# blue-yonder/tsfresh

Measured on AMD Instinct MI355X. Metric: series/sec (ComprehensiveFCParameters, len=1024), higher is better.
Workload: dtype f64

## Files before the change

tsfresh_amd/csrc/fam_ar.h:

```cpp
#ifndef TSFA_FAM_AR_H
#define TSFA_FAM_AR_H

#include "tsfa_common.h"

TSFA_DEV int adf_maxlag_for(int n) {
    int maxlag = (int)ceil(12.0 * pow((double)n / 100.0, 0.25));
    const int cap = n / 2 - 1 - 1;
    if (cap < maxlag) maxlag = cap;
    return maxlag;
}

TSFA_DEV bool chol_factor(double *G, int p, int ld) {
    for (int j = 0; j < p; ++j) {
        double d = G[j + j * ld];
        for (int k = 0; k < j; ++k) d -= G[j + k * ld] * G[j + k * ld];
        if (!(d > 0.0)) return false;
        d = sqrt(d);
        G[j + j * ld] = d;
        for (int i = j + 1; i < p; ++i) {
            double s = G[i + j * ld];
            for (int k = 0; k < j; ++k) s -= G[i + k * ld] * G[j + k * ld];
            G[i + j * ld] = s / d;
        }
    }
    return true;
}
TSFA_DEV void chol_solve(const double *L, int p, int ld, const double *rhs, double *x) {
    for (int i = 0; i < p; ++i) {
        double s = rhs[i];
        for (int k = 0; k < i; ++k) s -= L[i + k * ld] * x[k];
        x[i] = s * (1.0 / L[i + i * ld]);
    }
    for (int i = p - 1; i >= 0; --i) {
        double s = x[i];
        for (int k = i + 1; k < p; ++k) s -= L[k + i * ld] * x[k];
        x[i] = s * (1.0 / L[i + i * ld]);
    }
}

TSFA_DEV void blk_chol_solve(const Blk &b, const double *L, int p, int ld, const double *rhs, double *x) {
#if TSFA_GPU
    const int lane = b.tid & 63;
    const bool live = lane < p;
    double s = live ? rhs[lane] : 0.0;
    const double dg = live ? 1.0 / L[lane + lane * ld] : 1.0;
    for (int k = 0; k < p; ++k) {
        const double wk = readlane_f64(s, k) * readlane_f64(dg, k);
        if (lane == k) s = wk;
        else if (live && lane > k) s -= L[lane + k * ld] * wk;
    }
    for (int k = p - 1; k >= 0; --k) {
        const double xk = readlane_f64(s, k) * readlane_f64(dg, k);
        if (lane == k) s = xk;
        else if (live && lane < k) s -= L[k + lane * ld] * xk;
    }
    if (b.tid < p) x[b.tid] = s;
#else
    if (b.tid == 0) chol_solve(L, p, ld, rhs, x);
#endif
}

#define TSFA_AR_PIVOT_TOL 1e-6
TSFA_DEV bool blk_chol_factor(const Blk &b, double *G, int p, int ld, double *diag0, double *dmin = nullptr) {
    for (int a = b.tid; a < p; a += b.nt) diag0[a] = G[a + a * ld];
    double dm = TSFA_INF;
    for (int j = 0; j < p; ++j) {
        blk_sync();
        const double d = G[j + j * ld];
        if (!(d > TSFA_AR_PIVOT_TOL * diag0[j])) return false;
        dm = fmin(dm, d);
        if (dmin) *dmin = dm;
        const double sd = sqrt(d);
        blk_sync();
        const double rsd = 1.0 / sd;
        for (int i = j + b.tid; i < p; i += b.nt) G[i + j * ld] = (i == j) ? sd : G[i + j * ld] * rsd;
        blk_sync();
        const int rsh = (b.nt >= 32) ? 5 : 0;
        for (int i = j + 1 + (b.tid & ((1 << rsh) - 1)); i < p; i += (1 << rsh)) {
            const double lij = G[i + j * ld];
            for (int k = j + 1 + (b.tid >> rsh); k <= i; k += (b.nt >> rsh))
                G[i + k * ld] = G[i + k * ld] - lij * G[k + j * ld];
        }
    }
    blk_sync();
    return true;
}
TSFA_DEV void blk_chol_forward(const Blk &b, const double *L, int p, int ld, double *w) {
#if TSFA_GPU
    if (p <= 64) {
        const int lane = b.tid & 63;
        const bool live = lane < p;
        double s = live ? w[lane] : 0.0;
        const double dg = live ? 1.0 / L[lane + lane * ld] : 1.0;
        for (int k = 0; k < p; ++k) {
            const double wk = readlane_f64(s, k) * readlane_f64(dg, k);
            if (lane == k) s = wk;
            else if (live && lane > k) s = s - L[lane + k * ld] * wk;
        }
        blk_sync();
        if (b.tid < p) w[b.tid] = s;
        blk_sync();
        return;
    }
#endif
    for (int i = 0; i < p; ++i) {
        blk_sync();
        const double wi = w[i] * (1.0 / L[i + i * ld]);
        blk_sync();
        if (b.tid == 0) w[i] = wi;
        for (int k = i + 1 + b.tid; k < p; k += b.nt) w[k] = w[k] - L[k + i * ld] * wi;
    }
    blk_sync();
}


#define TSFA_AR_PADL 64
#define TSFA_AR_PADR 16

template <class ST>
TSFA_DEV void ar_load8(const ST *p, double (&r)[8]) {
#if TSFA_GPU
    p = (const ST *)__builtin_assume_aligned(p, 16);
#endif
#pragma unroll
    for (int q = 0; q < 8; ++q) r[q] = (double)p[q];
}

template <class ST>
struct ArBlocks {
    const ST *xs;
    double mean;
    TSFA_MEM void y8(int i0, double (&r)[8]) const {
        ar_load8(xs + i0, r);
#pragma unroll
        for (int q = 0; q < 8; ++q) r[q] -= mean;
    }
    TSFA_MEM void d8(int i0, double (&r)[8]) const {
        double v[8];
        ar_load8(xs + i0, v);
        const double nx = (double)xs[i0 + 8];
#pragma unroll
        for (int q = 0; q < 7; ++q) r[q] = v[q + 1] - v[q];
        r[7] = nx - v[7];
    }
};

TSFA_DEV void tile_mask_rows(double (&A)[8], int tb, int r0, int r1) {
#pragma unroll
    for (int u = 0; u < 8; ++u) A[u] = (tb + u >= r0 && tb + u < r1) ? A[u] : 0.0;
}

TSFA_DEV void tile_dots8(const double (&A)[8], const double (&lo)[8], const double (&hi)[8], double (&s)[8]) {
#pragma unroll
    for (int j = 0; j < 8; ++j) {
#pragma unroll
        for (int u = 0; u < 8; ++u) s[j] = fma(A[u], (u >= j) ? hi[u - j] : lo[u - j + 8], s[j]);
    }
}
TSFA_DEV void tile_axpy8(const double (&cf)[8], const double (&lo)[8], const double (&hi)[8], double (&r)[8]) {
#pragma unroll
    for (int j = 0; j < 8; ++j) {
#pragma unroll
        for (int u = 0; u < 8; ++u) r[u] = fma(-cf[j], (u >= j) ? hi[u - j] : lo[u - j + 8], r[u]);
    }
}

#define TSFA_AR_PART_STRIDE 72
template <class LA, class LB, class SF>
TSFA_DEV void blk_tile_lagdots(const Blk &b, int nrows, int nlags, LA loadA, LB loadB, SF store, double *sums = nullptr,
                               double *part = nullptr, int part_doubles = 0) {
    const int ntiles = (nrows + 7) >> 3;
    const bool single = ntiles <= b.nt;
#if TSFA_GPU
    const int nwv = (b.nt + 63) >> 6, wv = b.tid >> 6, lane = b.tid & 63;
#else
    const int nwv = 1, wv = 0;
#endif
    const bool deferred = (part != nullptr) && (nwv * TSFA_AR_PART_STRIDE <= part_doubles) && (nlags <= 64);
    if (deferred) blk_sync();
    double A[8], lo[8], hi[8];
    for (int j0 = 0; j0 < nlags; j0 += 8) {
        double s[8], sa[2] = {0.0, 0.0};
#pragma unroll
        for (int j = 0; j < 8; ++j) s[j] = 0.0;
        for (int tile = b.tid; tile < ntiles; tile += b.nt) {
            const int tb = tile << 3;
            if (single && j0 > 0) {
#pragma unroll
                for (int q = 0; q < 8; ++q) hi[q] = lo[q];
            } else {
                loadA(tb, A);
                loadB(tb - j0, hi);
            }
            loadB(tb - j0 - 8, lo);
            tile_dots8(A, lo, hi, s);
            if (sums != nullptr && j0 == 0) {
#pragma unroll
                for (int u = 0; u < 8; ++u) { sa[0] += A[u]; sa[1] = fma(A[u], A[u], sa[1]); }
            }
        }
        if (deferred) {
            double *slot = part + wv * TSFA_AR_PART_STRIDE;
#if TSFA_GPU
            const double held = wave_reduce_scatter<8>(s);
            if (lane < 8) slot[j0 + wave_reduce_scatter_index<8>(lane)] = held;
            if (sums != nullptr && j0 == 0) {
                sa[0] = wave_sum(sa[0]);
                sa[1] = wave_sum(sa[1]);
                if (lane == 0) { slot[64] = sa[0]; slot[65] = sa[1]; }
            }
#else
#pragma unroll
            for (int j = 0; j < 8; ++j) slot[j0 + j] = s[j];
            if (sums != nullptr && j0 == 0) { slot[64] = sa[0]; slot[65] = sa[1]; }
#endif
            continue;
        }
        blk_sum_multi<8>(b, s);
        if (b.tid == 0) {
#pragma unroll
            for (int j = 0; j < 8; ++j)
                if (j0 + j < nlags) store(j0 + j, s[j]);
        }
        if (sums != nullptr && j0 == 0) {
            blk_sum_multi<2>(b, sa);
            sums[0] = sa[0];
            sums[1] = sa[1];
        }
    }
    if (deferred) {
        blk_sync();
        for (int j = b.tid; j < nlags; j += b.nt) {
            double v = part[j];
            for (int w = 1; w < nwv; ++w) v += part[w * TSFA_AR_PART_STRIDE + j];
            store(j, v);
        }
        if (sums != nullptr) {
            double v0 = part[64], v1 = part[65];
            for (int w = 1; w < nwv; ++w) { v0 += part[w * TSFA_AR_PART_STRIDE + 64]; v1 += part[w * TSFA_AR_PART_STRIDE + 65]; }
            sums[0] = v0;
            sums[1] = v1;
        }
    }
}

template <class S>
TSFA_DEV void blk_lag_products_rest(const Blk &b, S s, int Lg, int t0, int t1, double *T, int ld, double *C) {
    if (b.tid == 0) {
        for (int j = 0; j < Lg; ++j) C[j + 1] = C[j] + s(t0 - 1 - j) - s(t1 - 1 - j);
    }
    blk_sync();
    for (int dg = b.tid; dg <= Lg; dg += b.nt) {
        double v = T[dg];
        for (int j = 0; dg + j + 1 <= Lg; ++j) {
            const int i = dg + j;
            v = v + s(t0 - 1 - i) * s(t0 - 1 - j) - s(t1 - 1 - i) * s(t1 - 1 - j);
            T[(i + 1) + (j + 1) * ld] = v;
        }
    }
    blk_sync();
}

TSFA_DEV double mackinnon_p_c1(double t) {
    if (t > 2.74) return 1.0;
    if (t < -18.83) return 0.0;
    double z;
    if (t <= -1.61) z = 2.1659 + t * (1.4412 + t * (3.8269 * 1e-2));
    else z = 1.7339 + t * (9.3202 * 1e-1 + t * (-1.2745 * 1e-1 + t * (-1.0368 * 1e-2)));
    return tsfa_norm_cdf(z);
}

TSFA_DEV int ar_scratch_doubles(int P) { return 2 * P * P + 7 * P + 64 + 16 + 48 + 40 + 128; }

#define TSFA_AR_REFINE_TOL 1e-8
TSFA_DEV bool ar_refinement_suspect(const Blk &b, const double *beta, const double *corr, const double *diag0, int p) {
    double mb = 0.0, mc = 0.0;
#if TSFA_GPU
    for (int a = b.tid & 63; a < p; a += 64) {
        const double w = sqrt(diag0[a]);
        mb = fmax(mb, fabs(beta[a]) * w);
        mc = fmax(mc, fabs(corr[a]) * w);
    }
    mb = wave_max(mb);
    mc = wave_max(mc);
#else
    (void)b;
    for (int a = 0; a < p; ++a) {
        const double w = sqrt(diag0[a]);
        mb = fmax(mb, fabs(beta[a]) * w);
        mc = fmax(mc, fabs(corr[a]) * w);
    }
#endif
    return mc > TSFA_AR_REFINE_TOL * mb;
}

#define TSFA_AR_COND_CHECK_K 10
#define TSFA_AR_RAW_RATIO 1e-12
TSFA_DEV bool ar_raw_design_suspect(double dmin, double mu_norm, double trace_raw) {
    return sqrt(dmin) < TSFA_AR_RAW_RATIO * (1.0 + mu_norm) * sqrt(trace_raw);
}

template <class ST>
struct ArCentred {
    const ST *p;
    double mean;
    TSFA_MEM double operator[](int i) const { return (double)p[i] - mean; }
};
template <class ST, class X>
TSFA_DEV int fam_ar_series(const Blk &b, X xv, int n, const TsfaSpec *specs, int nspecs, double *out_row, void *xc_raw,
                            double *aw, int P, int hint_acf, int hint_pacf, int hint_adf, int n_loop = -1,
                            const double *stats = nullptr) {
    const int nloop = (n_loop >= 0) ? n_loop : nspecs;
    const double dn = (double)n;
    TSFA_TICKER(tk, 0);
    const double mean = stats ? stats[TSFA_STATS_MEAN] : np_sum(b, n, [=](int i) { return xv(i); }) / dn;
    blk_sync();
    ST *xs_lds = (ST *)xc_raw + TSFA_AR_PADL;
    for (int i = b.tid; i < n + TSFA_AR_PADL + TSFA_AR_PADR; i += b.nt) {
        const int j = i - TSFA_AR_PADL;
        ((ST *)xc_raw)[i] = (j >= 0 && j < n) ? (ST)xv(j) : (ST)0;
    }
    const ArCentred<ST> xc{xs_lds, mean};
    const ArBlocks<ST> blk{xs_lds, mean};
    blk_sync();
    double v0 = 0.0;
    for (int i = b.tid; i < n; i += b.nt) v0 += xc[i] * xc[i];
    const double var = blk_sum(b, v0) / dn;

    double *T = aw;
    double *G = T + P * P;
    double *g = G + P * P;
    double *beta = g + P;
    double *tmp1 = beta + P;
    double *tmp2 = tmp1 + P;
    double *C = tmp2 + P;
    double *V = C + P;
    double *diag0 = V + P;
    double *acv = diag0 + P;
    double *res = acv + 64;
    double *pac = res + 16;
    double *arres = pac + 48;
    double *pacw = arres + 40;
    const ArCentred<ST> xcc = xc;
    int degenerate = 0;

    TSFA_TICK(tk, b, 120);
    int max_acf_lag = hint_acf, max_pacf_lag = hint_pacf;
    const bool need_adf = (hint_adf != 0);
    const int adf_mode = (hint_adf >> 1) & 3;
    if (max_acf_lag > 60) max_acf_lag = 60;
    if (max_pacf_lag > 40) max_pacf_lag = 40;

    int pacf_maxlag = 0;
    if (max_pacf_lag >= 0 && n > 1) pacf_maxlag = (max_pacf_lag >= n / 2) ? (n / 2 - 1) : max_pacf_lag;
    int nacv = -1;
    if (max_acf_lag >= 0) nacv = (max_acf_lag < n - 1) ? max_acf_lag : (n - 1);
    if (pacf_maxlag > nacv) nacv = pacf_maxlag;
    if (nacv >= 0) {
        blk_tile_lagdots(b, n, nacv + 1,
                         [=](int tb, double (&A)[8]) { blk.y8(tb, A); tile_mask_rows(A, tb, 0, n); },
                         [=](int i0, double (&B)[8]) {
                             blk.y8(i0, B);
#pragma unroll
                             for (int q = 0; q < 8; ++q) B[q] = (i0 >= 0) ? B[q] : 0.0;
                         },
                         [=](int k, double v) { acv[k] = v / (double)(n - k); }, nullptr, G, P * P);
    }
    blk_sync();

    TSFA_TICK(tk, b, 121);
    if (max_pacf_lag >= 0) {
#if TSFA_GPU
        {
            const int lane = b.tid & 63;
            for (int k = b.tid; k <= max_pacf_lag; k += b.nt) pac[k] = TSFA_NAN;
            blk_sync();
            if (n > 1 && pacf_maxlag > 0) {
                const int ord = pacf_maxlag;
                const double a0 = acv[0], a1 = acv[1];
                const double p1v = a1 / a0;
                double phi = (lane == 1) ? p1v : 0.0;
                double sig = a0 - p1v * a1;
                if (b.tid == 0) pac[1] = p1v;
                for (int k = 2; k <= ord; ++k) {
                    const int back = k - lane;
                    const double ak = acv[(back >= 0 && back <= ord) ? back : 0];
                    const double prod = phi * ak;
                    double dot = 0.0;
                    for (int j = 1; j < k; ++j) dot += readlane_f64(prod, j);
                    const double pkk = (acv[k] - dot) / sig;
                    const double rev = __shfl(phi, (back >= 0 && back < 64) ? back : 0);
                    phi = (lane >= 1 && lane < k) ? phi - pkk * rev : ((lane == k) ? pkk : phi);
                    sig = sig * (1.0 - pkk * pkk);
                    if (b.tid == 0) pac[k] = pkk;
                }
                if (b.tid == 0) pac[0] = 1.0;
            }
        }
#else
        if (b.tid == 0) {
            for (int k = 0; k <= max_pacf_lag; ++k) pac[k] = TSFA_NAN;
            if (n > 1 && pacf_maxlag > 0) {
                const int ord = pacf_maxlag;
                double *prev = pacw, *cur = pacw + 42, *sig = pacw + 84;
                prev[1] = acv[1] / acv[0];
                pac[1] = prev[1];
                sig[1] = acv[0] - prev[1] * acv[1];
                for (int k = 2; k <= ord; ++k) {
                    double dot = 0.0;
                    for (int j = 1; j < k; ++j) dot += prev[j] * acv[k - j];
                    const double pkk = (acv[k] - dot) / sig[k - 1];
                    for (int j = 1; j < k; ++j) cur[j] = prev[j] - pkk * prev[k - j];
                    cur[k] = pkk;
                    sig[k] = sig[k - 1] * (1.0 - pkk * pkk);
                    pac[k] = pkk;
                    for (int j = 1; j <= k; ++j) prev[j] = cur[j];
                }
                pac[0] = 1.0;
            }
        }
#endif
        blk_sync();
    }

    TSFA_TICK(tk, b, 122);
    double adf_stat = TSFA_NAN, adf_p = TSFA_NAN, adf_lag = TSFA_NAN;
    if (need_adf) {
        const int maxlag = adf_maxlag_for(n);
        if (maxlag + 2 > 64) degenerate |= 2;
        else if (maxlag >= 0 && maxlag + 3 <= P) {
            auto dif = [=](int t) { return (double)xs_lds[t + 1] - (double)xs_lds[t]; };
            const int t0 = maxlag, t1 = n - 1;
            const double nobs = (double)(t1 - t0);
            auto d_blocks = [=](int i0, double (&B)[8]) { blk.d8(i0, B); };
            double sd[2], sl[2];
            blk_tile_lagdots(b, n, maxlag + 1,
                             [=](int tb, double (&A)[8]) { blk.d8(tb, A); tile_mask_rows(A, tb, t0, t1); }, d_blocks,
                             [=](int j, double v) { T[j] = v; }, sd, G, P * P);
            blk_tile_lagdots(b, n, maxlag + 1,
                             [=](int tb, double (&A)[8]) { blk.y8(tb, A); tile_mask_rows(A, tb, t0, t1); }, d_blocks,
                             [=](int j, double v) { V[j] = v; }, sl, G, P * P);
            if (b.tid == 0) C[0] = sd[0];
            blk_lag_products_rest(b, dif, maxlag, t0, t1, T, P, C);
            const double sx = sl[0], sxx = sl[1];
            const int p1 = maxlag + 2;
            for (int e = b.tid; e < 64 * p1; e += b.nt) {
                const int a = e & 63, c = e >> 6;
                if (a >= p1 || c > a) continue;
                double v;
                if (a == 0) v = nobs;
                else if (a == 1) v = (c == 0) ? sx : sxx;
                else {
                    const int la = a - 1;
                    if (c == 0) v = C[la];
                    else if (c == 1) v = V[la];
                    else v = T[la + (c - 1) * P];
                }
                G[a + c * P] = v;
            }
            for (int a = b.tid; a < p1; a += b.nt) g[a] = (a == 0) ? C[0] : (a == 1 ? V[0] : T[a - 1]);
            blk_sync();
            const double yy = T[0];
            TSFA_TICK(tk, b, 123);
            {
                double dmin1 = 0.0;
                const bool okf = blk_chol_factor(b, G, p1, P, diag0, &dmin1);
                if (!okf) degenerate |= 2;
                else {
                    const double mu = xcc.mean;
                    const double tr = nobs + (sxx + 2.0 * mu * sx + nobs * mu * mu) + (double)maxlag * yy;
                    if (ar_raw_design_suspect(dmin1, fabs(mu), tr)) degenerate |= 2;
                }
                if (okf) {
                    for (int a = b.tid; a < p1; a += b.nt) tmp1[a] = g[a];
                    blk_chol_forward(b, G, p1, P, tmp1);
                    if (b.tid == 0) {
                        double acc = 0.0;
                        for (int i = 0; i < p1; ++i) { acc += tmp1[i] * tmp1[i]; tmp2[i] = acc; }
                    }
                    blk_sync();
                    for (int i = b.tid; i < p1; i += b.nt) {
                        const int pcols = i + 1;
                        const double ssr = yy - tmp2[i];
                        const double llf = -0.5 * nobs * log(2.0 * M_PI) - 0.5 * nobs * log(ssr / nobs) - 0.5 * nobs;
                        const double wi = tmp1[i];
                        double ic = -2.0 * llf + ((adf_mode == TSFA_AUTOLAG_BIC) ? log(nobs) : 2.0) * (double)pcols;
                        if (adf_mode == TSFA_AUTOLAG_TSTAT) ic = fabs(wi / sqrt(ssr / (nobs - (double)pcols)));
                        tmp1[i] = ic;
                    }
                    blk_sync();
                }
                if (b.tid == 0) {
                    int best = -1;
                    double best_aic = 0.0;
                    if (okf && adf_mode == TSFA_AUTOLAG_TSTAT) {
                        for (int i = p1 - 1; i >= 1; --i) {
                            best = i + 1;
                            if (tmp1[i] >= TSFA_AUTOLAG_TSTAT_STOP) break;
                        }
                    } else if (okf && adf_mode == TSFA_AUTOLAG_NONE) {
                        best = p1;
                    } else if (okf)
                        for (int i = 1; i < p1; ++i) {
                            const double aic = tmp1[i];
                            if (best < 0 || aic < best_aic) { best = i + 1; best_aic = aic; }
                        }
                    res[0] = (double)best;
                }
            }
            blk_sync();
            const int bestcols = (int)res[0];
            blk_sync();
            TSFA_TICK(tk, b, 124);
            if (bestcols >= 2) {
                const int usedlag = bestcols - 2;
                const int p2 = usedlag + 2;
                const int u0 = usedlag;
                const double nobs2 = (double)(t1 - u0);
                auto reg2 = [=](int a, int t) { return a == 0 ? xcc[t] : (a == p2 - 1 ? 1.0 : dif(t - a)); };
                for (int e = b.tid; e < p2 * p2 + p2; e += b.nt) {
                    const bool is_rhs = e >= p2 * p2;
                    const int a = is_rhs ? e - p2 * p2 : e % p2;
                    const int c = is_rhs ? 0 : e / p2;
                    if (!is_rhs && c > a) continue;
                    double v;
                    auto lagidx = [=](int q) { return q == 0 ? -2 : (q == p2 - 1 ? -1 : q); };
                    const int A = lagidx(a), Cc = is_rhs ? 0 : lagidx(c);
                    if (is_rhs) {
                        v = (A == -2) ? V[0] : (A == -1 ? C[0] : T[A]);
                    } else {
                        const int hi = a, lo = c;
                        (void)hi; (void)lo;
                        if (A == -1 && Cc == -1) v = nobs;
                        else if ((A == -1 && Cc == -2) || (A == -2 && Cc == -1)) v = sx;
                        else if (A == -2 && Cc == -2) v = sxx;
                        else if (A == -1) v = C[Cc];
                        else if (Cc == -1) v = C[A];
                        else if (A == -2) v = V[Cc];
                        else if (Cc == -2) v = V[A];
                        else v = (A >= Cc) ? T[A + Cc * P] : T[Cc + A * P];
                    }
                    for (int t = u0; t < t0; ++t) v += reg2(a, t) * (is_rhs ? dif(t) : reg2(c, t));
                    if (is_rhs) g[a] = v; else G[a + c * P] = v;
                }
                blk_sync();
                const bool ok2 = blk_chol_factor(b, G, p2, P, diag0);
                if (!ok2) degenerate |= 2;
                if (ok2) blk_chol_solve(b, G, p2, P, g, beta);
                blk_sync();
                if (ok2) {
                    auto resid2 = [=](int t) {
                        double r = dif(t);
                        for (int c = 0; c < p2; ++c) r -= reg2(c, t) * beta[c];
                        return r;
                    };
                    for (int a0 = 0; a0 < p2; a0 += 8) {
                        double s8[8];
#pragma unroll
                        for (int j = 0; j < 8; ++j) s8[j] = 0.0;
                        for (int t = u0 + b.tid; t < t1; t += b.nt) {
                            const double rt = resid2(t);
#pragma unroll
                            for (int j = 0; j < 8; ++j)
                                if (a0 + j < p2) s8[j] += reg2(a0 + j, t) * rt;
                        }
                        blk_sum_multi<8>(b, s8);
                        if (b.tid == 0) {
#pragma unroll
                            for (int j = 0; j < 8; ++j)
                                if (a0 + j < p2) tmp1[a0 + j] = s8[j];
                        }
                    }
                    blk_sync();
                    blk_chol_solve(b, G, p2, P, tmp1, tmp2);
                    blk_sync();
                    if (ar_refinement_suspect(b, beta, tmp2, diag0, p2)) degenerate |= 2;
                    blk_sync();
                    for (int a = b.tid; a < p2; a += b.nt) beta[a] += tmp2[a];
                    blk_sync();
                    double ssr = 0.0;
                    for (int t = u0 + b.tid; t < t1; t += b.nt) {
                        double r = dif(t);
                        for (int c = 0; c < p2; ++c) r -= reg2(c, t) * beta[c];
                        ssr += r * r;
                    }
                    ssr = blk_sum(b, ssr);
                    for (int i = b.tid; i < p2; i += b.nt) tmp1[i] = (i == 0) ? 1.0 : 0.0;
                    blk_sync();
                    blk_chol_solve(b, G, p2, P, tmp1, tmp2);
                    blk_sync();
                    if (b.tid == 0) {
                        const double sigma2 = ssr / (nobs2 - (double)p2);
                        const double tstat = beta[0] / sqrt(sigma2 * tmp2[0]);
                        res[2] = tstat;
                        res[3] = mackinnon_p_c1(tstat);
                        res[4] = (double)usedlag;
                    }
                    blk_sync();
                    adf_stat = res[2];
                    adf_p = res[3];
                    adf_lag = res[4];
                    if (adf_stat != adf_stat) adf_p = TSFA_NAN;
                    blk_sync();
                }
            }
        }
    }

    int ar_cached_k = -1;
    bool ar_ok = false;
    TSFA_TICK(tk, b, 125);
    for (int s = 0; s < nloop; ++s) {
        const TsfaSpec sp = specs[s];
        double v = TSFA_NAN;
        switch (sp.calc) {
        case TSFA_C_AGG_AUTOCORRELATION: {
            const int agg = (int)sp.p[0];
            const int ml = (int)sp.p[1];
            double r = TSFA_NAN;
#if TSFA_GPU
            {
                int len = (ml < n - 1) ? ml : (n - 1);
                if (len > 60) len = 60;
                const int lane = b.tid & 63;
                const bool live = lane < len;
                if (fabs(var) < 1e-10 || n == 1) {
                    r = 0.0;
                } else if (len > 0) {
                    const double a0 = acv[0];
                    const double ak = live ? acv[lane + 1] / a0 : 0.0;
                    if (agg == TSFA_AGG_MEAN) {
                        r = wave_sum(ak) / (double)len;
                    } else if (agg == TSFA_AGG_VAR) {
                        const double m = wave_sum(ak) / (double)len;
                        const double d = live ? ak - m : 0.0;
                        r = wave_sum(d * d) / (double)len;
                    } else {
                        int rank = 0;
                        for (int j = 0; j < len; ++j) {
                            const double aj = readlane_f64(ak, j);
                            rank += (aj < ak || (aj == ak && j < lane)) ? 1 : 0;
                        }
                        const unsigned long long mlo = __ballot(live && rank == (len - 1) / 2);
                        const unsigned long long mhi = __ballot(live && rank == len / 2);
                        const double lo = readlane_f64(ak, __ffsll((long long)mlo) - 1);
                        const double hi = readlane_f64(ak, __ffsll((long long)mhi) - 1);
                        r = (len & 1) ? lo : (0.0 + lo + hi) / 2.0;
                    }
                }
            }
            v = r;
            break;
#endif
            if (b.tid == 0) {
                if (fabs(var) < 1e-10 || n == 1) {
                    r = 0.0;
                } else {
                    int len = (ml < n - 1) ? ml : (n - 1);
                    if (len > 60) len = 60;
                    double abuf[64];
                    double *a = abuf;
                    for (int k = 0; k < len; ++k) a[k] = acv[k + 1] / acv[0];
                    if (len <= 0) {
                        r = TSFA_NAN;
                    } else if (agg == TSFA_AGG_MEAN) {
                        r = np_leaf_sum(0, len, [=](int i) { return a[i]; }) / (double)len;
                    } else if (agg == TSFA_AGG_VAR) {
                        const double m = np_leaf_sum(0, len, [=](int i) { return a[i]; }) / (double)len;
                        r = np_leaf_sum(0, len, [=](int i) { const double d = a[i] - m; return d * d; }) / (double)len;
                    } else {
                        for (int i = 1; i < len; ++i) {
                            const double key = a[i];
                            int j = i - 1;
                            while (j >= 0 && a[j] > key) { a[j + 1] = a[j]; --j; }
                            a[j + 1] = key;
                        }
                        r = (len & 1) ? a[(len - 1) / 2] : (0.0 + a[len / 2 - 1] + a[len / 2]) / 2.0;
                    }
                }
            }
            v = blk_bcast0(b, r);
        } break;
        case TSFA_C_PARTIAL_AUTOCORRELATION: {
            const int l = (int)sp.p[0];
            v = (l >= 0 && l <= max_pacf_lag) ? pac[l] : TSFA_NAN;
        } break;
        case TSFA_C_AUGMENTED_DICKEY_FULLER: {
            const int attr = (int)sp.p[0];
            v = (attr == TSFA_ADF_TESTSTAT) ? adf_stat : (attr == TSFA_ADF_PVALUE ? adf_p : (attr == TSFA_ADF_USEDLAG ? adf_lag : TSFA_NAN));
        } break;
        case TSFA_C_AR_COEFFICIENT: {
            const int coeff = (int)sp.p[0], k = (int)sp.p[1];
            if (coeff > k) { v = TSFA_NAN; break; }
            if (n < 2 * k + 2 || k < 1) {
                v = (coeff < k) ? TSFA_NAN : 0.0;
                break;
            }
            if (k > TSFA_AR_TABLE_K || k + 2 > P) {
                degenerate |= 1;
                v = TSFA_NAN;
                break;
            }
            if (ar_cached_k != k) {
                auto sx = [=](int u) { return xcc[u]; };
                auto y_blocks = [=](int i0, double (&B)[8]) { blk.y8(i0, B); };
                double sy[2];
                blk_tile_lagdots(b, n, k + 1,
                                 [=](int tb, double (&A)[8]) { blk.y8(tb, A); tile_mask_rows(A, tb, k, n); }, y_blocks,
                                 [=](int j, double v) { T[j] = v; }, sy, G, P * P);
                if (b.tid == 0) C[0] = sy[0];
                blk_lag_products_rest(b, sx, k, k, n, T, P, C);
                const int p = k + 1;
                for (int e = b.tid; e < p * p; e += b.nt) {
                    const int a = e % p, c = e / p;
                    if (c > a) continue;
                    G[a + c * P] = (a == 0) ? (double)(n - k) : (c == 0 ? C[a] : T[a + c * P]);
                }
                for (int a = b.tid; a < p; a += b.nt) g[a] = (a == 0) ? C[0] : T[a];
                blk_sync();
                double dmin_ar = 0.0;
                ar_ok = blk_chol_factor(b, G, p, P, diag0, &dmin_ar);
                if (!ar_ok) degenerate |= 1;
                else {
                    const double mu = xcc.mean, rows = (double)(n - k);
                    double tr = rows;
                    for (int a = 1; a < p; ++a) tr += diag0[a] + 2.0 * mu * C[a] + rows * mu * mu;
                    if (ar_raw_design_suspect(dmin_ar, sqrt((double)k) * fabs(mu), tr)) degenerate |= 1;
                }
                if (ar_ok && k > TSFA_AR_COND_CHECK_K) {
                    double tr0 = 0.0, s0 = 0.0;
                    for (int a = 0; a < p; ++a) { tr0 += diag0[a]; s0 += 1.0 / diag0[a]; }
                    for (int a = b.tid; a < p; a += b.nt) tmp1[a] = 1.0 / sqrt(diag0[a] * s0);
                    blk_sync();
                    double lmin = tr0;
                    for (int it = 0; it < 2; ++it) {
                        blk_chol_solve(b, G, p, P, tmp1, tmp2);
                        blk_sync();
                        double nrm2 = 0.0;
                        for (int a = 0; a < p; ++a) nrm2 += tmp2[a] * tmp2[a];
                        const double nrm = sqrt(nrm2);
                        if (!(nrm > 0.0) || isinf(nrm) || nrm != nrm) { lmin = 0.0; break; }
                        lmin = 1.0 / nrm;
                        blk_sync();
                        for (int a = b.tid; a < p; a += b.nt) tmp1[a] = tmp2[a] / nrm;
                        blk_sync();
                    }
                    if (!(lmin >= 1e-12 * tr0)) degenerate |= 1;
                }
                if (ar_ok) blk_chol_solve(b, G, p, P, g, beta);
                blk_sync();
                if (ar_ok) {
                    double sr[2];
                    blk_tile_lagdots(b, n, k + 1,
                                     [=](int tb, double (&A)[8]) {
                                         blk.y8(tb, A);
                                         const double b0 = beta[0];
#pragma unroll
                                         for (int u = 0; u < 8; ++u) A[u] -= b0;
                                         double lo[8], hi[8], cf[8];
                                         blk.y8(tb, hi);
                                         for (int c0 = 0; c0 <= k; c0 += 8) {
                                             blk.y8(tb - c0 - 8, lo);
#pragma unroll
                                             for (int j = 0; j < 8; ++j) {
                                                 const int c = c0 + j;
                                                 cf[j] = (c >= 1 && c <= k) ? beta[(c <= k) ? c : 0] : 0.0;
                                             }
                                             tile_axpy8(cf, lo, hi, A);
#pragma unroll
                                             for (int q = 0; q < 8; ++q) hi[q] = lo[q];
                                         }
                                         tile_mask_rows(A, tb, k, n);
                                     },
                                     y_blocks, [=](int a, double v) { if (a > 0) tmp1[a] = v; }, sr, T, P * P);
                    if (b.tid == 0) tmp1[0] = sr[0];
                    blk_sync();
                    blk_chol_solve(b, G, p, P, tmp1, tmp2);
                    blk_sync();
                    if (ar_refinement_suspect(b, beta, tmp2, diag0, p)) degenerate |= 1;
                    blk_sync();
                    if (b.tid == 0) {
                        double sphi = 0.0;
                        for (int a = 0; a < p; ++a) {
                            beta[a] += tmp2[a];
                            if (a > 0) sphi += beta[a];
                        }
                        arres[0] = beta[0] + mean * (1.0 - sphi);
                        for (int a = 1; a < p; ++a) arres[a] = beta[a];
                    }
                    blk_sync();
                }
                ar_cached_k = k;
            }
            v = ar_ok ? arres[coeff] : TSFA_NAN;
        } break;
        default: break;
        }
        if (b.tid == 0) out_row[sp.col] = v;
        TSFA_TICK(tk, b, sp.calc);
    }
    if (nloop < nspecs) {
        blk_sync();
        for (int s = nloop + b.tid; s < nspecs; s += b.nt) {
            const TsfaSpec sp = specs[s];
            double v = TSFA_NAN;
            if (sp.calc == TSFA_C_PARTIAL_AUTOCORRELATION) {
                const int l = (int)sp.p[0];
                v = (l >= 0 && l <= max_pacf_lag) ? pac[l] : TSFA_NAN;
            } else if (sp.calc == TSFA_C_AUGMENTED_DICKEY_FULLER) {
                const int attr = (int)sp.p[0];
                v = (attr == TSFA_ADF_TESTSTAT) ? adf_stat : (attr == TSFA_ADF_PVALUE ? adf_p : (attr == TSFA_ADF_USEDLAG ? adf_lag : TSFA_NAN));
            } else if (sp.calc == TSFA_C_AR_COEFFICIENT) {
                const int coeff = (int)sp.p[0], k = (int)sp.p[1];
                if (coeff > k) v = TSFA_NAN;
                else if (n < 2 * k + 2 || k < 1) v = (coeff < k) ? TSFA_NAN : 0.0;
                else v = (ar_cached_k == k && ar_ok && k <= TSFA_AR_TABLE_K) ? arres[coeff] : TSFA_NAN;
            }
            out_row[sp.col] = v;
        }
    }
    return degenerate;
}

#endif
```

tsfresh_amd/csrc/tsfa_api.cpp:

```cpp
#include <hip/hip_runtime.h>

#include <stdio.h>
#include <stdlib.h>

#include <algorithm>
#include <string>
#include <vector>

#include "../../include/tsfresh_amd.h"
#include "tsfa_host_tables.h"
#include "tsfa_launch.h"
#include "fam_seq.h"
#include "tsfa_layout.h"

static thread_local std::string g_last_error;

static int fail(int code, const std::string &msg) {
    g_last_error = msg;
    return code;
}

int tsfa_fail(int code, const char *msg) { return fail(code, std::string(msg ? msg : "")); }
#define HIP_TRY(expr)                                                                                    \
    do {                                                                                                 \
        hipError_t e_ = (expr);                                                                          \
        if (e_ != hipSuccess) return fail(TSFA_ERR_HIP, std::string(#expr) + ": " + hipGetErrorString(e_)); \
    } while (0)

struct DevBuf {
    void *p = nullptr;
    size_t cap = 0;
    int ensure(size_t bytes) {
        if (bytes <= cap) return 0;
        size_t want = bytes + bytes / 8 + 4096;
        void *q = nullptr;
        if (hipMalloc(&q, want) != hipSuccess) {
            (void)hipGetLastError();
            if (p) { (void)hipFree(p); p = nullptr; cap = 0; }
            if (hipMalloc(&q, want) != hipSuccess) {
                (void)hipGetLastError();
                return -1;
            }
        }
        if (p) (void)hipFree(p);
        p = q;
        cap = want;
        return 0;
    }
    void release() {
        if (p) (void)hipFree(p);
        p = nullptr;
        cap = 0;
    }
};

#define TSFA_MAX_AUX 3
#define TSFA_MAX_CHUNKS 16
#define TSFA_DEFAULT_STREAMS 1

struct Timing {
    std::string name;
    hipEvent_t e0 = nullptr, e1 = nullptr;
    float ms = 0.f;
};

struct PlanOptions {
    bool length_classes = true;
    bool stats_share = true;
    bool perm_share = true;
    bool select = true;
    bool bluestein = true;
    bool cwt_mfma = false;
    bool force_long = false;
    int entropy_route = 0;
    int bluestein_min = 0;
    int gscratch_slots = 0;
    int host_chunks = 0;
    int nt[TSFA_N_FAMILIES] = {0};
    bool trace = false;
    bool row_form = true;
    int seq_rows = -1;
};

#if defined(TSFA_LAB)
#define TSFA_LAB_ONLY(x) (x)
#else
#define TSFA_LAB_ONLY(x) (0)
#endif

static int64_t g_relevance_batch = 0;
int64_t tsfa_relevance_batch_override() { return g_relevance_batch; }

struct tsfa_plan {
    int device = 0;
    PlanOptions opt;
    hipStream_t stream = nullptr;
    int n_cols = 0;
    std::vector<TsfaSpec> fam_specs[TSFA_N_FAMILIES];
    TsfaSpec *d_specs[TSFA_N_FAMILIES] = {nullptr};
    TsfaFamHints hints[TSFA_N_FAMILIES];
    TsfaCwtBank bank;
    double *d_W = nullptr;
    int *d_cols = nullptr, *d_coeff = nullptr;
    double *d_dectab = nullptr, *d_twc = nullptr, *d_tws = nullptr, *d_consts = nullptr;
    long long *d_stats = nullptr;
    DevBuf values, offsets, out, gscratch, times, deg_list, sel, long_scratch, pf_buf, perm_buf, stats_buf, dd_scratch, gen_scratch, seq_rows;
    std::vector<TsfaSpec> gen_specs;
    TsfaSpec *d_gen_specs = nullptr;
    TsfaGenPlan gen_plan;
    double *d_pool = nullptr;
    int *d_deg_count = nullptr;
    int *d_cursor = nullptr;
    hipStream_t s_in = nullptr, s_out = nullptr;
    hipEvent_t ev_in[TSFA_MAX_CHUNKS] = {nullptr}, ev_k[TSFA_MAX_CHUNKS] = {nullptr};
    std::vector<int64_t> h_rel;
    bool needs_times = false;
    bool sort_only_order_stats = false;
    bool stream_ok = false;
    int n_streams = 1;
    hipStream_t aux[TSFA_MAX_AUX] = {nullptr};
    hipEvent_t ev_fork = nullptr, ev_join[TSFA_MAX_AUX] = {nullptr};
    bool profiling = false;
    std::vector<Timing> timings;
    long long hint_min_len = 0, hint_max_len = 0;
    bool fill_all = false;
    int *d_fill_cols = nullptr;
    int n_fill_cols = 0;
    int debug_skip_fam = -1;
    hipStream_t side = nullptr;
    hipEvent_t ev_side_fork = nullptr, ev_side_join = nullptr;
    unsigned side_mask = 0;
    double fill_value = __builtin_nan("");
};

static const char *fam_names[TSFA_N_FAMILIES] = {"k_basic", "k_sort", "k_spectral", "k_ar", "k_entropy", "k_cwtpeaks", "k_seq", "k_trend"};

template <class T>
static int upload(const std::vector<T> &h, T **d) {
    *d = nullptr;
    if (h.empty()) return 0;
    if (hipMalloc((void **)d, h.size() * sizeof(T)) != hipSuccess) return -1;
    if (hipMemcpy(*d, h.data(), h.size() * sizeof(T), hipMemcpyHostToDevice) != hipSuccess) return -1;
    return 0;
}

static int record(tsfa_plan *plan, hipStream_t st, size_t slot, const char *name, bool begin) {
    if (!plan->profiling) return 0;
    if (plan->timings.size() <= slot) plan->timings.resize(slot + 1);
    Timing &t = plan->timings[slot];
    if (!t.e0) {
        if (hipEventCreate(&t.e0) != hipSuccess || hipEventCreate(&t.e1) != hipSuccess) return -1;
    }
    t.name = name;
    return hipEventRecord(begin ? t.e0 : t.e1, st) == hipSuccess ? 0 : -1;
}

extern "C" {

int tsfa_version(void) { return TSFA_VERSION; }

int tsfa_device_count(void) {
    int n = 0;
    if (hipGetDeviceCount(&n) != hipSuccess) return 0;
    return n;
}

const char *tsfa_last_error(void) { return g_last_error.c_str(); }

int tsfa_calc_id(const char *name) {
    if (!name) return -1;
    for (int i = 0; i < TSFA_N_CALCS; ++i)
        if (strcmp(tsfa_calc_table[i].name, name) == 0) return i;
    return -1;
}
const char *tsfa_calc_name(int calc) { return (calc >= 0 && calc < TSFA_N_CALCS) ? tsfa_calc_table[calc].name : nullptr; }
int tsfa_calc_count(void) { return TSFA_N_CALCS; }

void tsfa_plan_destroy(tsfa_plan *plan) {
    if (!plan) return;
    (void)hipSetDevice(plan->device);
    for (int f = 0; f < TSFA_N_FAMILIES; ++f)
        if (plan->d_specs[f]) (void)hipFree(plan->d_specs[f]);
    if (plan->d_W) (void)hipFree(plan->d_W);
    if (plan->d_cols) (void)hipFree(plan->d_cols);
    if (plan->d_coeff) (void)hipFree(plan->d_coeff);
    if (plan->d_dectab) (void)hipFree(plan->d_dectab);
    if (plan->d_twc) (void)hipFree(plan->d_twc);
    if (plan->d_tws) (void)hipFree(plan->d_tws);
    if (plan->d_consts) (void)hipFree(plan->d_consts);
    if (plan->d_stats) (void)hipFree(plan->d_stats);
    if (plan->d_deg_count) (void)hipFree(plan->d_deg_count);
    if (plan->d_cursor) (void)hipFree(plan->d_cursor);
    plan->deg_list.release();
    plan->pf_buf.release();
    plan->stats_buf.release();
    plan->perm_buf.release();
    plan->sel.release();
    plan->long_scratch.release();
    for (int i = 0; i < TSFA_MAX_CHUNKS; ++i) {
        if (plan->ev_in[i]) (void)hipEventDestroy(plan->ev_in[i]);
        if (plan->ev_k[i]) (void)hipEventDestroy(plan->ev_k[i]);
    }
    if (plan->s_in) (void)hipStreamDestroy(plan->s_in);
    if (plan->s_out) (void)hipStreamDestroy(plan->s_out);
    plan->times.release();
    plan->values.release();
    plan->offsets.release();
    plan->out.release();
    plan->gscratch.release();
    plan->dd_scratch.release();
    plan->gen_scratch.release();
    if (plan->d_gen_specs) (void)hipFree(plan->d_gen_specs);
    if (plan->d_pool) (void)hipFree(plan->d_pool);
    for (auto &t : plan->timings) {
        if (t.e0) (void)hipEventDestroy(t.e0);
        if (t.e1) (void)hipEventDestroy(t.e1);
    }
    for (int i = 0; i < TSFA_MAX_AUX; ++i) {
        if (plan->aux[i]) (void)hipStreamDestroy(plan->aux[i]);
        if (plan->ev_join[i]) (void)hipEventDestroy(plan->ev_join[i]);
    }
    if (plan->ev_fork) (void)hipEventDestroy(plan->ev_fork);
    if (plan->side) (void)hipStreamDestroy(plan->side);
    if (plan->ev_side_fork) (void)hipEventDestroy(plan->ev_side_fork);
    if (plan->ev_side_join) (void)hipEventDestroy(plan->ev_side_join);
    if (plan->stream) (void)hipStreamDestroy(plan->stream);
    delete plan;
}

int tsfa_plan_create(const tsfa_feature_spec *specs, int32_t n_specs, int32_t device, tsfa_plan **out_plan) {
    return tsfa_plan_create_with_data(specs, n_specs, nullptr, 0, device, out_plan);
}

int tsfa_plan_create_with_data(const tsfa_feature_spec *specs, int32_t n_specs, const double *data, int64_t n_data, int32_t device,
                               tsfa_plan **out_plan) {
    if (!out_plan) return fail(TSFA_ERR_INVALID, "out_plan is NULL");
    *out_plan = nullptr;
    if (n_specs < 0 || (n_specs > 0 && !specs)) return fail(TSFA_ERR_INVALID, "bad specs");
    if (n_data < 0 || (n_data > 0 && !data)) return fail(TSFA_ERR_INVALID, "bad data pool");
    const int ndev = tsfa_device_count();
    if (ndev <= 0) return fail(TSFA_ERR_NO_DEVICE, "no HIP device visible: tsfresh_amd has no CPU fallback");
    if (device < 0 || device >= ndev) return fail(TSFA_ERR_INVALID, "device ordinal out of range");

    tsfa_plan *plan = new tsfa_plan();
    plan->device = device;
    plan->n_cols = n_specs;
    std::vector<TsfaSpec> cwt_coef;
    bool general[TSFA_N_CALCS];
    tsfa_general_calcs(specs, n_specs, general);
    for (int i = 0; i < n_specs; ++i) {
        TsfaSpec s;
        s.calc = specs[i].calc;
        s.col = i;
        for (int k = 0; k < 4; ++k) s.p[k] = specs[i].p[k];
        if (s.calc < 0 || s.calc >= TSFA_N_CALCS) {
            delete plan;
            return fail(TSFA_ERR_UNSUPPORTED, "spec " + std::to_string(i) + ": unknown calculator id " + std::to_string(s.calc));
        }
        const std::string why = tsfa_validate_spec(s);
        if (!why.empty()) {
            delete plan;
            return fail(TSFA_ERR_UNSUPPORTED, std::string("spec ") + std::to_string(i) + " (" + tsfa_calc_table[s.calc].name + "): " + why);
        }
        if (s.calc == TSFA_C_QUERY_SIMILARITY_COUNT && s.p[3] > 0 && !(s.p[2] + s.p[3] <= (double)n_data)) {
            delete plan;
            return fail(TSFA_ERR_INVALID, "spec " + std::to_string(i) + " (query_similarity_count): the query lies outside the data pool");
        }
        if (s.calc == TSFA_C_LINEAR_TREND_TIMEWISE) plan->needs_times = true;
        if (s.calc == TSFA_C_CWT_COEFFICIENTS) cwt_coef.push_back(s);
        else if (general[s.calc]) plan->gen_specs.push_back(s);
        else plan->fam_specs[tsfa_calc_table[s.calc].family].push_back(s);
    }
    plan->gen_plan = tsfa_prepare_general(plan->gen_specs);
    if (cwt_coef.size() > 128) {
        delete plan;
        return fail(TSFA_ERR_UNSUPPORTED, "more than 128 cwt_coefficients columns in one plan");
    }
    {
        std::vector<TsfaSpec> all;
        for (int f = 0; f < TSFA_N_FAMILIES; ++f) all.insert(all.end(), plan->fam_specs[f].begin(), plan->fam_specs[f].end());
        const std::string why = tsfa_validate_plan(all.data(), (int)all.size());
        if (!why.empty()) {
            delete plan;
            return fail(TSFA_ERR_UNSUPPORTED, why);
        }
    }
    if (!cwt_coef.empty()) {
        const std::string why = plan->bank.build(cwt_coef);
        if (!why.empty()) {
            delete plan;
            return fail(TSFA_ERR_UNSUPPORTED, why);
        }
    }
    if (hipSetDevice(device) != hipSuccess) {
        delete plan;
        return fail(TSFA_ERR_HIP, "hipSetDevice failed");
    }
    for (int f = 0; f < TSFA_N_FAMILIES; ++f) tsfa_prepare_family(f, plan->fam_specs[f], plan->hints[f]);
    plan->sort_only_order_stats = !plan->fam_specs[TSFA_FAM_SORT].empty();
    for (const auto &sp : plan->fam_specs[TSFA_FAM_SORT])
        if (sp.calc != TSFA_C_MEDIAN && sp.calc != TSFA_C_QUANTILE) plan->sort_only_order_stats = false;
    plan->stream_ok = !plan->fam_specs[TSFA_FAM_BASIC].empty() && plan->hints[TSFA_FAM_BASIC].c == 0;
    for (const auto &sp : plan->fam_specs[TSFA_FAM_BASIC])
        if (!tsfa_stream_calc_ok(sp.calc) || sp.calc == TSFA_C_MEDIAN) plan->stream_ok = false;
    for (const auto &sp : plan->fam_specs[TSFA_FAM_SORT])
        if (sp.calc != TSFA_C_MEDIAN) plan->stream_ok = false;
    bool ok = hipStreamCreateWithFlags(&plan->stream, hipStreamNonBlocking) == hipSuccess;
    for (int f = 0; ok && f < TSFA_N_FAMILIES; ++f) ok = upload(plan->fam_specs[f], &plan->d_specs[f]) == 0;
    if (ok) ok = upload(plan->gen_specs, &plan->d_gen_specs) == 0;
    if (ok && n_data > 0) ok = upload(std::vector<double>(data, data + n_data), &plan->d_pool) == 0;
    if (ok && !cwt_coef.empty()) {
        ok = upload(plan->bank.W, &plan->d_W) == 0 && upload(plan->bank.cols, &plan->d_cols) == 0 &&
             upload(plan->bank.coeff_idx, &plan->d_coeff) == 0;
    }
    if (ok) {
        std::vector<double> dt, twc, tws;
        tsfa_build_dectab(dt);
        tsfa_build_twiddles(twc, tws);
        ok = upload(dt, &plan->d_dectab) == 0 && upload(twc, &plan->d_twc) == 0 && upload(tws, &plan->d_tws) == 0;
        std::vector<double> consts;
        tsfa_build_consts(consts);
        ok = ok && upload(consts, &plan->d_consts) == 0;
    }
    if (ok) ok = hipMalloc((void **)&plan->d_stats, TSFA_LEN_STATS * sizeof(long long)) == hipSuccess;
    if (ok) ok = hipMalloc((void **)&plan->d_deg_count, 2 * sizeof(int)) == hipSuccess;
    if (ok) ok = hipMalloc((void **)&plan->d_cursor, TSFA_N_LEN_CLASSES * sizeof(int)) == hipSuccess;
    if (ok) ok = hipStreamCreateWithFlags(&plan->s_in, hipStreamNonBlocking) == hipSuccess &&
                 hipStreamCreateWithFlags(&plan->s_out, hipStreamNonBlocking) == hipSuccess;
    for (int i = 0; ok && i < TSFA_MAX_CHUNKS; ++i)
        ok = hipEventCreateWithFlags(&plan->ev_in[i], hipEventDisableTiming) == hipSuccess &&
             hipEventCreateWithFlags(&plan->ev_k[i], hipEventDisableTiming) == hipSuccess;
    {
        const char *e = getenv("TSFA_STREAMS");
        plan->n_streams = e ? std::min(std::max(atoi(e), 1), TSFA_MAX_AUX + 1) : TSFA_DEFAULT_STREAMS;
        for (int i = 0; ok && i + 1 < plan->n_streams; ++i)
            ok = hipStreamCreateWithFlags(&plan->aux[i], hipStreamNonBlocking) == hipSuccess &&
                 hipEventCreateWithFlags(&plan->ev_join[i], hipEventDisableTiming) == hipSuccess;
        if (ok && plan->n_streams > 1) ok = hipEventCreateWithFlags(&plan->ev_fork, hipEventDisableTiming) == hipSuccess;
    }
    if (const char *e = getenv("TSFA_PAIR")) {
        static const char *nm[TSFA_N_FAMILIES] = {"basic", "sort", "spectral", "ar", "entropy", "cwt", "seq", "trend"};
        for (int f = 0; f < TSFA_N_FAMILIES; ++f)
            if (f != TSFA_FAM_BASIC && f != TSFA_FAM_SORT && f != TSFA_FAM_ENTROPY && strstr(e, nm[f])) plan->side_mask |= 1u << f;
        if (plan->side_mask) {
            int least = 0, greatest = 0;
            (void)hipDeviceGetStreamPriorityRange(&least, &greatest);
            ok = ok && hipStreamCreateWithPriority(&plan->side, hipStreamNonBlocking, least) == hipSuccess &&
                 hipEventCreateWithFlags(&plan->ev_side_fork, hipEventDisableTiming) == hipSuccess &&
                 hipEventCreateWithFlags(&plan->ev_side_join, hipEventDisableTiming) == hipSuccess;
        }
    }
    if (const char *e = getenv("TSFA_HOST_CHUNKS")) plan->opt.host_chunks = std::max(atoi(e), 0);
    if (!ok) {
        tsfa_plan_destroy(plan);
        return fail(TSFA_ERR_HIP, "device allocation/upload failed while creating the plan");
    }
    *out_plan = plan;
    return TSFA_OK;
}

int32_t tsfa_plan_n_cols(const tsfa_plan *plan) { return plan ? plan->n_cols : -1; }

int tsfa_plan_set_length_hint(tsfa_plan *plan, int64_t min_len, int64_t max_len) {
    if (!plan) return fail(TSFA_ERR_INVALID, "null plan");
    if (max_len == 0 && min_len == 0) { plan->hint_min_len = plan->hint_max_len = 0; return TSFA_OK; }
    if (min_len < 1 || max_len < min_len || max_len > 2147483647LL / 64) return fail(TSFA_ERR_INVALID, "length hint must satisfy 1 <= min <= max <= 33554431");
    plan->hint_min_len = min_len;
    plan->hint_max_len = max_len;
    return TSFA_OK;
}

int tsfa_plan_set_option(tsfa_plan *plan, const char *name, double value) {
    if (!name) return fail(TSFA_ERR_INVALID, "option name is NULL");
    const std::string n(name);
    const bool on = value != 0.0;
    if (!plan) {
        if (n == "relevance_batch") { g_relevance_batch = value > 0.0 ? (int64_t)value : 0; return TSFA_OK; }
        return fail(TSFA_ERR_INVALID, "unknown library option '" + n + "'");
    }
    PlanOptions &o = plan->opt;
    if (n == "length_classes") o.length_classes = on;
    else if (n == "stats_share") o.stats_share = on;
    else if (n == "perm_share") o.perm_share = on;
    else if (n == "select") o.select = on;
    else if (n == "bluestein") o.bluestein = on;
    else if (n == "cwt_mfma") o.cwt_mfma = on;
    else if (n == "force_long") o.force_long = on;
    else if (n == "row_form") o.row_form = on;
    else if (n == "seq_rows") o.seq_rows = (value < 0.0) ? -1 : (on ? 1 : 0);
    else if (n == "entropy_route") { if (value != 0.0 && value != 1.0 && value != 2.0) return fail(TSFA_ERR_INVALID, "entropy_route: 0, 1 or 2"); o.entropy_route = (int)value; }
    else if (n == "bluestein_min") o.bluestein_min = value > 0.0 ? (int)std::min(value, 32767.0) : 0;
    else if (n == "gscratch_slots") o.gscratch_slots = value > 0.0 ? (int)std::min(value, 2147483647.0) : 0;
    else if (n == "host_chunks") o.host_chunks = value > 0.0 ? (int)std::min(value, (double)TSFA_MAX_CHUNKS) : 0;
    else if (n == "fused_minimal") { if (!on) plan->stream_ok = false; }
    else if (n == "perm_fused") { if (!on) plan->hints[TSFA_FAM_SORT].d = 0; }
    else if (n == "fill") { plan->fill_value = value; plan->fill_all = true; }
    else if (n == "fill_off") { plan->fill_all = false; }
#if defined(TSFA_LAB)
    else if (n == "skip_family") plan->debug_skip_fam = (int)value;
    else if (n == "trace") o.trace = on;
    else if (n.rfind("nt_", 0) == 0 && n.size() == 4 && n[3] >= '0' && n[3] < '0' + TSFA_N_FAMILIES) o.nt[n[3] - '0'] = (int)value;
#endif
    else return fail(TSFA_ERR_INVALID, "unknown plan option '" + n + "'");
    return TSFA_OK;
}

int tsfa_plan_set_profiling(tsfa_plan *plan, int32_t enable) {
    if (!plan) return fail(TSFA_ERR_INVALID, "plan is NULL");
    plan->profiling = enable != 0;
    return TSFA_OK;
}

int32_t tsfa_plan_last_timings(const tsfa_plan *plan, const char **names, float *ms, int32_t cap) {
    if (!plan) return 0;
    int32_t n = 0;
    for (const auto &t : plan->timings) {
        if (n >= cap) break;
        if (names) names[n] = t.name.c_str();
        if (ms) ms[n] = t.ms;
        ++n;
    }
    return n;
}

int tsfa_extract(tsfa_plan *plan, const void *values, int32_t dtype, const int64_t *offsets, int64_t n_series,
                 double *out, int64_t ld_out, int32_t space, void *stream) {
    return tsfa_extract_timed(plan, values, dtype, nullptr, offsets, n_series, out, ld_out, space, stream);
}

int tsfa_extract_timed(tsfa_plan *plan, const void *values, int32_t dtype, const double *times, const int64_t *offsets,
                       int64_t n_series, double *out, int64_t ld_out, int32_t space, void *stream) {
    return tsfa_extract_windows(plan, values, dtype, times, offsets, offsets ? offsets + 1 : nullptr, n_series, out,
                                ld_out, space, stream);
}

struct BatchShape {
    long long max_len = 0, min_len = 0, max_np2 = 0;
    int n_groups = 1;
    int g_maxn[TSFA_N_LEN_CLASSES] = {0};
    long long g_np2[TSFA_N_LEN_CLASSES] = {0};
    int64_t g_count[TSFA_N_LEN_CLASSES] = {0};
    bool g_has_short[TSFA_N_LEN_CLASSES] = {false};
    TsfaClassMap map;
};

static void shape_from_stats(const long long *st, int64_t n_series, BatchShape &sh, bool length_classes) {
    sh.max_len = st[0];
    sh.min_len = st[1];
    sh.max_np2 = st[2];
    memset(&sh.map, 0, sizeof sh.map);
    sh.n_groups = 1;
    sh.g_maxn[0] = (int)st[0];
    sh.g_np2[0] = st[2];
    sh.g_count[0] = n_series;
    sh.g_has_short[0] = st[1] <= TSFA_ROW_MAXN;
    if (!length_classes || n_series < 2048 || st[0] <= 2 * st[1] || st[0] <= 128) return;
    const int64_t min_group = 512;
    int ng = 0;
    int64_t pend_count = 0;
    long long pend_np2 = 0;
    int first_of_group = 0;
    for (int c = 0; c < TSFA_N_LEN_CLASSES; ++c) {
        const int64_t cnt = st[3 + c];
        pend_count += cnt;
        pend_np2 = std::max(pend_np2, st[3 + 2 * TSFA_N_LEN_CLASSES + c]);
        bool last = true;
        for (int d = c + 1; d < TSFA_N_LEN_CLASSES; ++d)
            if (st[3 + d] > 0) last = false;
        if (cnt > 0 && (pend_count >= min_group || last)) {
            sh.g_maxn[ng] = (int)st[3 + TSFA_N_LEN_CLASSES + c];
            sh.g_np2[ng] = pend_np2;
            sh.g_count[ng] = pend_count;
            sh.g_has_short[ng] = false;
            for (int d = first_of_group; d <= c; ++d) {
                sh.map.group_of[d] = ng;
                if ((64LL << d) <= TSFA_ROW_MAXN && st[3 + d] > 0) sh.g_has_short[ng] = true;
            }
            first_of_group = c + 1;
            pend_count = 0;
            pend_np2 = 0;
            ++ng;
        }
        if (last) {
            for (int d = first_of_group; d < TSFA_N_LEN_CLASSES; ++d) sh.map.group_of[d] = ng > 0 ? ng - 1 : 0;
            break;
        }
    }
    sh.n_groups = std::max(ng, 1);
    int b = 0;
    for (int g = 0; g < sh.n_groups; ++g) {
        sh.map.base[g] = b;
        b += (int)sh.g_count[g];
    }
}

static int host_len_stats(const int64_t *starts, const int64_t *ends, int64_t n, long long *st) {
    for (int i = 0; i < TSFA_LEN_STATS; ++i) st[i] = 0;
    st[1] = (1LL << 62);
    for (int64_t s = 0; s < n; ++s) {
        const long long l = ends[s] - starts[s];
        if (l < 0) return -1;
        const bool np2 = l > 0 && (l & (l - 1)) != 0;
        const int c = tsfa_len_class(l);
        st[0] = std::max(st[0], l);
        st[1] = std::min(st[1], l);
        if (np2) st[2] = std::max(st[2], l);
        st[3 + c] += 1;
        st[3 + TSFA_N_LEN_CLASSES + c] = std::max(st[3 + TSFA_N_LEN_CLASSES + c], l);
        if (np2) st[3 + 2 * TSFA_N_LEN_CLASSES + c] = std::max(st[3 + 2 * TSFA_N_LEN_CLASSES + c], l);
    }
    return 0;
}

static int run_batch(tsfa_plan *plan, const void *d_values, int dtype, const double *d_times, const int64_t *d_starts,
                     const int64_t *d_ends, int64_t n_series, double *d_out, int64_t ld, const BatchShape &sh,
                     const int *d_sel, hipStream_t st, bool with_overlap) {
    if ((plan->fill_all || plan->n_fill_cols > 0) &&
        tsfa_launch_fill_nan(d_out, n_series, plan->n_cols, ld, st, plan->fill_value, plan->fill_all ? nullptr : plan->d_fill_cols,
                             plan->n_fill_cols))
        return fail(TSFA_ERR_HIP, "fill launch failed");

    static const int order_long_first[TSFA_N_FAMILIES] = {TSFA_FAM_ENTROPY, TSFA_FAM_AR, TSFA_FAM_SORT, TSFA_FAM_CWT, TSFA_FAM_BASIC,
                                                          TSFA_FAM_SEQ, TSFA_FAM_SPECTRAL, TSFA_FAM_TREND};
    static const int order_basic_first[TSFA_N_FAMILIES] = {TSFA_FAM_BASIC, TSFA_FAM_ENTROPY, TSFA_FAM_AR, TSFA_FAM_SORT, TSFA_FAM_CWT,
                                                           TSFA_FAM_SEQ, TSFA_FAM_SPECTRAL, TSFA_FAM_TREND};
    const bool overlap = with_overlap && plan->n_streams > 1 && !plan->profiling;
    const bool share_stats = plan->stats_buf.p != nullptr && !overlap && !plan->stream_ok && plan->opt.stats_share;
    const int *order = share_stats ? order_basic_first : order_long_first;
    bool stats_valid[TSFA_N_LEN_CLASSES + 1];
    for (int g = 0; g <= TSFA_N_LEN_CLASSES; ++g) stats_valid[g] = false;
    if (overlap) {
        HIP_TRY(hipEventRecord(plan->ev_fork, st));
        for (int i = 0; i + 1 < plan->n_streams; ++i) HIP_TRY(hipStreamWaitEvent(plan->aux[i], plan->ev_fork, 0));
    }
    bool pair = plan->side != nullptr && plan->side_mask != 0 && !overlap && !plan->profiling && with_overlap;
    for (int g = 0; g < sh.n_groups; ++g) pair = pair && sh.g_maxn[g] <= 4096;
    bool side_forked = false, side_used = false;
    size_t slot = 0;
    int dealt = 0;
    bool perm_valid[TSFA_N_LEN_CLASSES + 1];
    for (int g = 0; g <= TSFA_N_LEN_CLASSES; ++g) perm_valid[g] = false;
    const bool perm_share = plan->perm_buf.p != nullptr && !overlap && plan->opt.perm_share;
    bool stream_done[TSFA_N_LEN_CLASSES + 1];
    for (int g = 0; g <= TSFA_N_LEN_CLASSES; ++g) stream_done[g] = false;
    for (int fi = 0; fi < TSFA_N_FAMILIES; ++fi) {
        const int f = order[fi];
        if (plan->fam_specs[f].empty()) continue;
        if (TSFA_LAB_ONLY(plan->debug_skip_fam == f)) continue;
        if (f == TSFA_FAM_BASIC && plan->stream_ok) {
            bool all = true;
            for (int g = 0; g < sh.n_groups; ++g) all = all && stream_done[g];
            if (all) continue;
        }
        hipStream_t fst = st;
        if (overlap) {
            const int k = dealt++ % plan->n_streams;
            if (k > 0) fst = plan->aux[k - 1];
        }
        if (pair && fi > 0 && ((plan->side_mask >> f) & 1u)) {
            if (!side_forked) {
                HIP_TRY(hipEventRecord(plan->ev_side_fork, st));
                HIP_TRY(hipStreamWaitEvent(plan->side, plan->ev_side_fork, 0));
                side_forked = true;
            }
            fst = plan->side;
            side_used = true;
        }
        const char *slot_name = (plan->stream_ok && (f == TSFA_FAM_SORT || (f == TSFA_FAM_BASIC && plan->fam_specs[TSFA_FAM_SORT].empty())))
                                    ? "k_stream" : fam_names[f];
        if (record(plan, fst, slot, slot_name, true)) return fail(TSFA_ERR_HIP, "event record failed");
        std::vector<TsfaLaunch> perm_launches;
        for (int g = sh.n_groups - 1; g >= 0; --g) {
            const int maxn = sh.g_maxn[g];
            const long long max_np2 = sh.g_np2[g];
            TsfaLaunch a;
            memset(&a, 0, sizeof a);
            a.fam = f;
            a.dtype = dtype;
            a.values = d_values;
            a.starts = d_starts;
            a.ends = d_ends;
            a.n_series = sh.g_count[g];
            a.sel = (sh.n_groups > 1) ? d_sel + sh.map.base[g] : nullptr;
            a.specs = plan->d_specs[f];
            a.nspecs = (int)plan->fam_specs[f].size();
            a.out = d_out;
            a.ld = ld;
            a.maxn = maxn;
            a.nt = (maxn <= 2048) ? 64 : 256;
            if (maxn > 2048) {
                static const int nt_8k[TSFA_N_FAMILIES] = {512, 512, 512, 512, 256, 1024, 256, 256};
                static const int nt_4k[TSFA_N_FAMILIES] = {256, 256, 256, 256, 256, 512, 256, 256};
                a.nt = (maxn > 4096) ? nt_8k[f] : nt_4k[f];
            }
            if (maxn <= 2048) {
                static const int pref[TSFA_N_FAMILIES] = {64, 128, 128, 128, 256, 256, 128, 64};
                const int cap = std::max(64, ((maxn / 4 + 63) / 64) * 64);
                a.nt = std::min(pref[f], cap);
            }
            if (TSFA_LAB_ONLY(plan->opt.nt[f] >= 64)) a.nt = plan->opt.nt[f];
            a.stream = fst;
            a.dectab = plan->d_dectab;
            a.times = d_times;
            a.twc = plan->d_twc;
            a.consts = plan->d_consts;
            a.tws = plan->d_tws;
            a.hint_a = plan->hints[f].a;
            a.hint_b = plan->hints[f].b;
            a.hint_c = plan->hints[f].c;
            a.hint_d = plan->hints[f].d;
            a.hint_e = plan->hints[f].e;
            a.alt = plan->hints[f].alt;
            a.cq = plan->hints[f].cq;
            if (f == TSFA_FAM_SPECTRAL && maxn > 2048 && !TSFA_LAB_ONLY(plan->opt.nt[f] >= 64)) a.nt = 512;
            int aux = 0;
            if (f == TSFA_FAM_TREND) aux = a.alt.small_w;
            if (f == TSFA_FAM_SPECTRAL) {
                a.dft_n = (int)std::min<long long>(max_np2, 256);
                aux = a.dft_n;
                int bl_odd = TSFA_BLUESTEIN_MIN, bl_even = TSFA_BLUESTEIN_MIN_EVEN;
                if (plan->opt.bluestein_min > 0) bl_odd = bl_even = std::min(std::max(plan->opt.bluestein_min, 17), 32767);
                a.bluestein_min = TSFA_BLUESTEIN_PACK(bl_odd, bl_even);
                if (max_np2 >= std::min(bl_odd, bl_even) && max_np2 <= 32768 && plan->opt.bluestein) {
                    long long M = 1;
                    while (M < 2 * max_np2 - 1) M <<= 1;
                    const size_t slot_bytes = (size_t)(4 * M) * sizeof(double);
                    int64_t slots = std::min<int64_t>(a.n_series, std::max<int64_t>((int64_t)((1ull << 30) / slot_bytes), 2048));
                    if (plan->opt.gscratch_slots > 0) slots = std::min<int64_t>(slots, plan->opt.gscratch_slots);
                    const size_t bytes = (size_t)slots * slot_bytes;
                    if (plan->gscratch.ensure(bytes) == 0) {
                        a.gscratch = (double *)plan->gscratch.p;
                        a.gscratch_n = (int)(4 * M);
                        a.gscratch_slots = slots;
                    }
                }
            } else if (f == TSFA_FAM_CWT) {
                a.cwt_rowv = tsfa_family_lds_bytes(f, maxn, a.nt, 1) <= 96 * 1024 ? 1 : 0;
                aux = a.cwt_rowv;
                if (plan->opt.cwt_mfma) a.cwt_rowv |= 2;
            } else if (f == TSFA_FAM_AR) {
                int P = 8, Pdd = 8;
                for (const auto &s : plan->fam_specs[f]) {
                    if (s.calc == TSFA_C_AUGMENTED_DICKEY_FULLER) {
                        int ml = (int)ceil(12.0 * pow((double)maxn / 100.0, 0.25));
                        if (maxn / 2 - 2 < ml) ml = maxn / 2 - 2;
                        P = std::max(P, ml + 3);
                    } else if (s.calc == TSFA_C_AR_COEFFICIENT) {
                        const int k = std::min((int)s.p[1], std::max(1, (maxn - 2) / 2));
                        if ((int)s.p[1] <= TSFA_AR_TABLE_K) P = std::max(P, (int)s.p[1] + 2);
                        Pdd = std::max(Pdd, k + 2);
                        a.ar_has_coef = 1;
                    }
                }
                Pdd = std::max(Pdd, P);
                a.ar_P = P;
                a.ar_P_dd = Pdd;
                aux = P;
                {
                    ArDdLds D;
                    if (D.carve(nullptr, Pdd) > TSFA_LDS_LIMIT - 2048) {
                        const size_t slot_bytes = (size_t)ArDdLds::scratch_doubles(Pdd) * sizeof(double);
                        const int slots = (int)std::min<int64_t>(a.n_series, std::min<int64_t>(256, std::max<int64_t>(8, (int64_t)(((size_t)2 << 30) / slot_bytes))));
                        if (plan->dd_scratch.ensure((size_t)slots * slot_bytes))
                            return fail(TSFA_ERR_HIP, "hipMalloc failed for the second AR pass");
                        a.dd_scratch = (double *)plan->dd_scratch.p;
                        a.dd_slots = slots;
                    }
                }
                a.deg_list = (long long *)plan->deg_list.p;
                a.deg_count = plan->d_deg_count;
                HIP_TRY(hipMemsetAsync(plan->d_deg_count, 0, sizeof(int), fst));
            } else if (f == TSFA_FAM_SORT && plan->hints[f].b > 0) {
                a.pf_slot = tsfa_pf_slot_doubles(plan->hints[f].b);
                a.pf_buf = (double *)plan->pf_buf.p;
                a.pf_count = plan->d_deg_count + 1;
                a.pf_cap = (int)std::min<long long>((long long)n_series * std::max(1, plan->hints[f].e), 2147483647LL);
                HIP_TRY(hipMemsetAsync(a.pf_count, 0, sizeof(int), fst));
            } else if (f == TSFA_FAM_ENTROPY) {
                const int waves = std::min(4, std::max(1, (maxn - 1 + 63) / 64));
                a.nt = std::max(a.nt, 64 * waves);
                a.ent_cnt = tsfa_entropy_lds_bytes(maxn, 1) <= TSFA_LDS_LIMIT ? 1 : 0;
                a.ent_fast = a.ent_cnt;
                for (const auto &s : plan->fam_specs[f])
                    if (s.calc == TSFA_C_APPROXIMATE_ENTROPY && (int)s.p[0] != 2) a.ent_fast = 0;
                if (plan->opt.entropy_route == 2) a.ent_fast = 0;
                const bool entb_wide = maxn > TSFA_ENTB_MAXN && maxn <= TSFA_ENTB_MAXN_WIDE &&
                                       tsfa_entropy_lds_bytes(maxn, 2) <= TSFA_LDS_LIMIT &&
                                       entb_kround(maxn, std::min(a.nspecs, TSFA_ENTB_MAXK), TSFA_ENTB_MAXWAVES) >= std::min(a.nspecs, TSFA_ENTB_MAXK);
                if (a.ent_fast && a.nspecs >= 2 && maxn >= 3 && plan->opt.entropy_route == 0 &&
                    ((maxn <= TSFA_ENTB_MAXN && tsfa_entropy_lds_bytes(maxn, 2) <= TSFA_LDS_LIMIT / 2) || entb_wide)) {
                    a.ent_cnt = 2;
                    a.nt = 64 * std::min(TSFA_ENTB_MAXWAVES, entb_waves_for(maxn, a.nspecs));
                    if (TSFA_LAB_ONLY(plan->opt.nt[f] >= 64)) a.nt = plan->opt.nt[f];
                } else if (a.ent_fast && a.nspecs >= 2 && maxn > TSFA_ENTB_MAXN && maxn <= TSFA_ENTB_MAXN_LONG &&
                           plan->opt.entropy_route == 0 &&
                           tsfa_entropy_lds_bytes(maxn, 3) <= TSFA_LDS_LIMIT) {
                    a.ent_cnt = 3;
                    a.nt = 64 * TSFA_ENTB_MAXWAVES;
                } else if (a.nspecs >= 2 && maxn > TSFA_ENTB_MAXN_LONG && maxn <= TSFA_ENTH_MAXN && plan->opt.entropy_route == 0) {
                    bool all_m2 = true;
                    for (const auto &s : plan->fam_specs[f])
                        if (s.calc == TSFA_C_APPROXIMATE_ENTROPY && (int)s.p[0] != 2) all_m2 = false;
                    if (all_m2) {
                        a.ent_cnt = 4;
                        a.ent_fast = 0;
                        a.nt = 64 * TSFA_ENTB_MAXWAVES;
                    }
                }
            }
            int seq_group = 0;
            if (f == TSFA_FAM_SEQ) {
                for (seq_group = std::min(a.nspecs, TSFA_LZ_MAX_GROUP); seq_group > 1; --seq_group) {
                    bool fits = true;
                    for (int s0 = 0; fits && s0 < a.nspecs; s0 += seq_group) {
                        lz_build_group(plan->fam_specs[f].data() + s0, std::min(seq_group, a.nspecs - s0), maxn, &a.seq);
                        fits = tsfa_seq_lds_bytes(a.seq) <= TSFA_LDS_LIMIT;
                    }
                    if (fits) break;
                }
                lz_build_group(plan->fam_specs[f].data(), std::min(seq_group, a.nspecs), maxn, &a.seq);
            }
            size_t seq_lds = 0;
            int seq_grows = 0;
            if (f == TSFA_FAM_SEQ) {
                TsfaSeqGroup g;
                for (int s0 = 0; s0 < a.nspecs; s0 += seq_group) {
                    lz_build_group(plan->fam_specs[f].data() + s0, std::min(seq_group, a.nspecs - s0), maxn, &g);
                    seq_lds = std::max(seq_lds, tsfa_seq_lds_bytes(g));
                }
                if (plan->opt.seq_rows != 0 && !plan->opt.force_long) {
                    const int group_g = std::min(a.nspecs, TSFA_LZ_MAX_GROUP);
                    size_t lds_g = 0, stride_g = 0;
                    for (int s0 = 0; s0 < a.nspecs; s0 += group_g) {
                        lz_build_group(plan->fam_specs[f].data() + s0, std::min(group_g, a.nspecs - s0), maxn, &g, 1);
                        lds_g = std::max(lds_g, tsfa_seq_lds_bytes(g));
                        stride_g = std::max(stride_g, (size_t)g.stride);
                    }
                    auto resident = [&](size_t lds) {
                        if (lds > TSFA_LDS_LIMIT) return (size_t)0;
                        return std::min<size_t>((size_t)(163840 / std::max<size_t>(lds, 1)), (size_t)(32 * 64 / a.nt));
                    };
                    const bool more = resident(lds_g) > resident(seq_lds);
                    if (lds_g <= TSFA_LDS_LIMIT && (plan->opt.seq_rows == 1 || more) &&
                        (size_t)a.n_series * stride_g <= ((size_t)2 << 30) &&
                        plan->seq_rows.ensure((size_t)a.n_series * stride_g) == 0) {
                        seq_grows = 1;
                        seq_group = group_g;
                        seq_lds = lds_g;
                        a.seq_rows = (unsigned char *)plan->seq_rows.p;
                    }
                }
            }
            size_t lds = (f == TSFA_FAM_SEQ) ? seq_lds
                         : (f == TSFA_FAM_ENTROPY) ? tsfa_entropy_lds_bytes(maxn, a.ent_cnt)
                                                   : tsfa_family_lds_bytes(f, maxn, a.nt, aux);
            const bool use_long = lds > TSFA_LDS_LIMIT || plan->opt.force_long || (f == TSFA_FAM_ENTROPY && a.ent_cnt == 4);
            if (TSFA_LAB_ONLY(f == TSFA_FAM_SPECTRAL && plan->opt.trace))
                fprintf(stderr, "[tsfa] spectral group %d: n_series %lld maxn %d max_np2 %lld lds %zu long %d chirp-z %d slots %lld nt %d\n", g,
                        (long long)a.n_series, maxn, max_np2, lds, (int)use_long, (int)(a.gscratch != nullptr), (long long)a.gscratch_slots, a.nt);
            if (use_long) {
                if (!(f == TSFA_FAM_ENTROPY && a.ent_cnt == 4)) a.nt = 256;
                if (a.gscratch != nullptr && a.gscratch_slots < std::min<int64_t>(a.n_series, 2048)) a.gscratch = nullptr;
                if (f == TSFA_FAM_ENTROPY && a.ent_cnt != 4) { a.ent_cnt = 0; a.ent_fast = 0; lds = tsfa_entropy_lds_bytes(maxn, 5); }
                if (f == TSFA_FAM_CWT) { a.cwt_rowv &= 2; lds = tsfa_family_lds_bytes(f, maxn, a.nt, 0); }
                if (f == TSFA_FAM_SEQ) {
                    seq_group = std::min(a.nspecs, TSFA_LZ_MAX_GROUP);
                    seq_grows = 0;
                    lds = 0;
                    for (int s0 = 0; s0 < a.nspecs; s0 += seq_group) {
                        lz_build_group(plan->fam_specs[f].data() + s0, std::min(seq_group, a.nspecs - s0), maxn, &a.seq);
                        lds = std::max(lds, tsfa_seq_lds_bytes(a.seq));
                    }
                } else if (f != TSFA_FAM_ENTROPY && f != TSFA_FAM_CWT) {
                    lds = tsfa_family_lds_bytes(f, maxn, a.nt, aux);
                }
                const size_t slot_bytes = (lds + 255) & ~(size_t)255;
                const int64_t n_slots = std::max<int64_t>(1, std::min<int64_t>(std::min<int64_t>(a.n_series, 512),
                                                                               (int64_t)((4ull << 30) / slot_bytes)));
                if (plan->long_scratch.ensure((size_t)n_slots * slot_bytes))
                    return fail(TSFA_ERR_HIP, "hipMalloc failed for the long-series scratch");
                a.long_scratch = (unsigned char *)plan->long_scratch.p;
                a.long_bytes = (size_t)n_slots * slot_bytes;
            }
            if (share_stats && g <= TSFA_N_LEN_CLASSES) {
                if (f == TSFA_FAM_BASIC && !(plan->hints[f].c == 0 && a.nt <= 256)) {
                    a.stats_out = (double *)plan->stats_buf.p;
                    stats_valid[g] = true;
                } else if ((f == TSFA_FAM_ENTROPY || f == TSFA_FAM_AR || f == TSFA_FAM_SEQ || f == TSFA_FAM_SORT) && stats_valid[g]) {
                    a.stats_in = (const double *)plan->stats_buf.p;
                }
            }
            if (perm_share && !use_long && g <= TSFA_N_LEN_CLASSES) {
                if (f == TSFA_FAM_ENTROPY && a.ent_cnt == 2 && maxn <= TSFA_ENTB_MAXN) {
                    a.perm_buf = (unsigned short *)plan->perm_buf.p;
                    a.perm_stride = TSFA_ENTB_MAXN;
                    perm_valid[g] = true;
                } else if (f == TSFA_FAM_SORT && perm_valid[g]) {
                    a.perm_buf = (unsigned short *)plan->perm_buf.p;
                    a.perm_stride = TSFA_ENTB_MAXN;
                }
            }
            if (f == TSFA_FAM_SORT) {
                a.hint_d = 0;
                if (plan->hints[f].d != 0) {
                    const int pnt = (maxn <= 2048) ? std::min(256, std::max(64, ((maxn / 4 + 63) / 64) * 64))
                                                   : std::min(1024, ((maxn / 8 + 63) / 64) * 64);
                    if (maxn <= 65535 && tsfa_perm_lds_bytes(maxn, pnt, dtype == TSFA_F32 ? 4 : 8) <= TSFA_LDS_LIMIT) {
                        a.hint_d = plan->hints[f].d;
                        TsfaLaunch pa = a;
                        pa.nt = pnt;
                        pa.long_scratch = nullptr;
                        perm_launches.push_back(pa);
                    }
                }
            }
            int rc = 0;
            if (plan->stream_ok && (f == TSFA_FAM_SORT || f == TSFA_FAM_BASIC) && maxn <= 2048 && g <= TSFA_N_LEN_CLASSES) {
                if (stream_done[g]) continue;
                TsfaLaunch sa = a;
                sa.specs = plan->d_specs[TSFA_FAM_SORT];
                sa.nspecs = (int)plan->fam_specs[TSFA_FAM_SORT].size();
                sa.bspecs = plan->d_specs[TSFA_FAM_BASIC];
                sa.nbspecs = (int)plan->fam_specs[TSFA_FAM_BASIC].size();
                rc = tsfa_launch_stream(sa);
                stream_done[g] = true;
            } else
            if (f == TSFA_FAM_SORT && plan->sort_only_order_stats && maxn <= 2048 && !use_long &&
                plan->opt.select) {
                rc = tsfa_launch_order_stats(a);
            } else if (f == TSFA_FAM_SEQ) {
                for (int s0 = 0; rc == 0 && s0 < a.nspecs; s0 += seq_group) {
                    lz_build_group(plan->fam_specs[f].data() + s0, std::min(seq_group, a.nspecs - s0), maxn, &a.seq, seq_grows);
                    if (!use_long && tsfa_seq_lds_bytes(a.seq) > TSFA_LDS_LIMIT)
                        return fail(TSFA_ERR_TOO_LONG, "k_seq: a series of " + std::to_string(maxn) + " samples does not fit LDS");
                    rc = use_long ? tsfa_launch_family_long(a) : tsfa_launch_family(a);
                }
            } else {
                bool rows_any = false, rows_all = false;
                const bool lite = (f == TSFA_FAM_BASIC && plan->hints[f].c == 0 && a.nt <= 256);
                if ((f == TSFA_FAM_BASIC || f == TSFA_FAM_TREND) && plan->opt.row_form && !lite && g <= TSFA_N_LEN_CLASSES) {
                    rows_any = sh.g_has_short[g];
                    rows_all = maxn <= TSFA_ROW_MAXN;
                }
                if (rows_any) {
                    a.skip_le = TSFA_ROW_MAXN;
                    rc = tsfa_launch_rows(a);
                }
                if (rc == 0 && !rows_all) rc = use_long ? tsfa_launch_family_long(a) : tsfa_launch_family(a);
            }
            if (rc == 0 && f == TSFA_FAM_AR) rc = tsfa_launch_ar_degenerate(a);
            if (rc == 0 && f == TSFA_FAM_SORT && a.pf_buf) rc = tsfa_launch_langevin_dd(a);
            if (rc) return fail(TSFA_ERR_HIP, std::string(fam_names[f]) + " launch failed: " +
                                                  (rc == -2 ? "no scratch slot" : hipGetErrorString((hipError_t)rc)));
        }
        if (record(plan, fst, slot, slot_name, false)) return fail(TSFA_ERR_HIP, "event record failed");
        ++slot;
        if (!perm_launches.empty()) {
            if (record(plan, fst, slot, "k_perm", true)) return fail(TSFA_ERR_HIP, "event record failed");
            for (const auto &pa : perm_launches) {
                const int rc = tsfa_launch_perm(pa);
                if (rc) return fail(TSFA_ERR_HIP, std::string("k_perm launch failed: ") + hipGetErrorString((hipError_t)rc));
            }
            if (record(plan, fst, slot, "k_perm", false)) return fail(TSFA_ERR_HIP, "event record failed");
            ++slot;
        }
    }
    if (overlap) {
        for (int i = 0; i + 1 < plan->n_streams; ++i) {
            HIP_TRY(hipEventRecord(plan->ev_join[i], plan->aux[i]));
            HIP_TRY(hipStreamWaitEvent(st, plan->ev_join[i], 0));
        }
    }
    if (side_used) {
        HIP_TRY(hipEventRecord(plan->ev_side_join, plan->side));
        HIP_TRY(hipStreamWaitEvent(st, plan->ev_side_join, 0));
    }
    if (plan->bank.C > 0) {
        TsfaCwtLaunch c;
        memset(&c, 0, sizeof c);
        c.dtype = dtype;
        c.values = d_values;
        c.starts = d_starts;
        c.ends = d_ends;
        c.n_series = n_series;
        c.W = plan->d_W;
        c.S4 = plan->bank.S4;
        c.C = plan->bank.C;
        c.cols = plan->d_cols;
        c.coeff_idx = plan->d_coeff;
        c.out = d_out;
        c.ld = ld;
        c.stream = st;
        if (record(plan, st, slot, "k_cwt_gemm", true)) return fail(TSFA_ERR_HIP, "event record failed");
        const int rc = tsfa_launch_cwt(c);
        if (rc) return fail(TSFA_ERR_HIP, "k_cwt_gemm launch failed");
        if (record(plan, st, slot, "k_cwt_gemm", false)) return fail(TSFA_ERR_HIP, "event record failed");
        ++slot;
    }
    if (!plan->gen_specs.empty()) {
        const int maxn = (int)sh.max_len;
        const size_t slot_doubles = tsfa_general_slot_doubles(maxn, plan->gen_plan) + 8;
        int slots = (int)std::min<int64_t>(n_series, 2048);
        const size_t budget = (size_t)1 << 30;
        if ((size_t)slots * slot_doubles * sizeof(double) > budget)
            slots = (int)std::max<size_t>(16, budget / (slot_doubles * sizeof(double)));
        slots = (int)std::min<int64_t>(slots, n_series);
        if (plan->gen_scratch.ensure((size_t)slots * slot_doubles * sizeof(double)))
            return fail(TSFA_ERR_HIP, "hipMalloc failed for the scratch of k_general");
        TsfaLaunch a;
        memset(&a, 0, sizeof a);
        a.dtype = dtype;
        a.values = d_values;
        a.starts = d_starts;
        a.ends = d_ends;
        a.n_series = n_series;
        a.specs = plan->d_gen_specs;
        a.nspecs = (int)plan->gen_specs.size();
        a.out = d_out;
        a.ld = ld;
        a.maxn = maxn;
        a.stream = st;
        if (record(plan, st, slot, "k_general", true)) return fail(TSFA_ERR_HIP, "event record failed");
        if (tsfa_launch_general(a, plan->gen_plan, (double *)plan->gen_scratch.p, slot_doubles, slots, plan->d_pool))
            return fail(TSFA_ERR_HIP, "k_general launch failed");
        if (record(plan, st, slot, "k_general", false)) return fail(TSFA_ERR_HIP, "event record failed");
        ++slot;
    }
    if (plan->profiling) plan->timings.resize(slot);
    return TSFA_OK;
}

static int check_shape(const tsfa_plan *plan, const BatchShape &sh) {
    if (sh.min_len < 1) return fail(TSFA_ERR_INVALID, "every series must hold at least one sample");
    if (sh.max_len > 2147483647LL / 64) return fail(TSFA_ERR_TOO_LONG, "series longer than 33 554 431 samples are not supported");
    return TSFA_OK;
}

static int build_sel(tsfa_plan *plan, const int64_t *d_starts, const int64_t *d_ends, int64_t n_series, const BatchShape &sh,
                     int *d_sel, hipStream_t st) {
    if (sh.n_groups <= 1) return TSFA_OK;
    HIP_TRY(hipMemsetAsync(plan->d_cursor, 0, TSFA_N_LEN_CLASSES * sizeof(int), st));
    if (tsfa_launch_class_fill(d_starts, d_ends, n_series, sh.map, plan->d_cursor, d_sel, st))
        return fail(TSFA_ERR_HIP, "class_fill launch failed");
    return TSFA_OK;
}

int tsfa_extract_windows(tsfa_plan *plan, const void *values, int32_t dtype, const double *times, const int64_t *starts,
                         const int64_t *ends, int64_t n_series, double *out, int64_t ld_out, int32_t space,
                         void *stream) {
    if (!plan) return fail(TSFA_ERR_INVALID, "plan is NULL");
    if (plan->needs_times && !times)
        return fail(TSFA_ERR_INVALID, "the plan holds linear_trend_timewise columns: call tsfa_extract_timed with the "
                                      "per-sample times (the reference skips the calculator without a DatetimeIndex)");
    if (dtype != TSFA_F32 && dtype != TSFA_F64) return fail(TSFA_ERR_INVALID, "dtype must be TSFA_F32 or TSFA_F64");
    if (space != TSFA_HOST && space != TSFA_DEVICE) return fail(TSFA_ERR_INVALID, "space must be TSFA_HOST or TSFA_DEVICE");
    if (n_series < 0) return fail(TSFA_ERR_INVALID, "n_series < 0");
    if (n_series == 0 || plan->n_cols == 0) return TSFA_OK;
    if (!values || !starts || !ends || !out) return fail(TSFA_ERR_INVALID, "NULL buffer");
    if (ld_out < plan->n_cols) return fail(TSFA_ERR_INVALID, "ld_out < n_cols");
    if (n_series > 2147483647LL) return fail(TSFA_ERR_INVALID, "n_series exceeds the grid limit (2^31 - 1)");
    HIP_TRY(hipSetDevice(plan->device));
    const size_t esz = (dtype == TSFA_F32) ? 4 : 8;
    if (plan->deg_list.ensure((size_t)n_series * sizeof(long long)))
        return fail(TSFA_ERR_HIP, "hipMalloc failed for the k_ar_degenerate list");
    if (!plan->fam_specs[TSFA_FAM_SORT].empty() && !plan->fam_specs[TSFA_FAM_ENTROPY].empty() && !plan->sort_only_order_stats &&
        plan->perm_buf.ensure((size_t)n_series * (size_t)TSFA_ENTB_MAXN * sizeof(unsigned short)))
        return fail(TSFA_ERR_HIP, "hipMalloc failed for the shared sample order");
    if (!plan->fam_specs[TSFA_FAM_BASIC].empty() && !plan->stream_ok &&
        (!plan->fam_specs[TSFA_FAM_ENTROPY].empty() || !plan->fam_specs[TSFA_FAM_AR].empty() || !plan->fam_specs[TSFA_FAM_SEQ].empty() ||
         !plan->fam_specs[TSFA_FAM_SORT].empty()) &&
        plan->stats_buf.ensure((size_t)n_series * TSFA_STATS_N * sizeof(double)))
        return fail(TSFA_ERR_HIP, "hipMalloc failed for the shared per-series statistics");
    if (plan->hints[TSFA_FAM_SORT].b > 0 &&
        plan->pf_buf.ensure((size_t)n_series * (size_t)std::max(1, plan->hints[TSFA_FAM_SORT].e) *
                            (size_t)tsfa_pf_slot_doubles(plan->hints[TSFA_FAM_SORT].b) * sizeof(double)))
        return fail(TSFA_ERR_HIP, "hipMalloc failed for the records of the Langevin second pass");

    if (space == TSFA_DEVICE) {
        hipStream_t st = stream ? (hipStream_t)stream : plan->stream;
        long long h_stats[TSFA_LEN_STATS];
        for (int i = 0; i < TSFA_LEN_STATS; ++i) h_stats[i] = 0;
        h_stats[1] = (1LL << 62);
        BatchShape sh;
        if (plan->hint_max_len > 0) {
            h_stats[0] = plan->hint_max_len;
            h_stats[1] = plan->hint_min_len;
            h_stats[2] = (plan->hint_min_len == plan->hint_max_len && (plan->hint_max_len & (plan->hint_max_len - 1)) == 0)
                             ? 0 : plan->hint_max_len;
            sh.max_len = h_stats[0];
            sh.min_len = h_stats[1];
            sh.max_np2 = h_stats[2];
            sh.g_maxn[0] = (int)h_stats[0];
            sh.g_np2[0] = h_stats[2];
            sh.g_count[0] = n_series;
            sh.g_has_short[0] = plan->hint_min_len <= TSFA_ROW_MAXN;
            memset(&sh.map, 0, sizeof sh.map);
        } else {
            HIP_TRY(hipMemcpyAsync(plan->d_stats, h_stats, sizeof h_stats, hipMemcpyHostToDevice, st));
            if (tsfa_launch_len_stats(starts, ends, n_series, plan->d_stats, st)) return fail(TSFA_ERR_HIP, "len_stats launch failed");
            HIP_TRY(hipMemcpyAsync(h_stats, plan->d_stats, sizeof h_stats, hipMemcpyDeviceToHost, st));
            HIP_TRY(hipStreamSynchronize(st));
            shape_from_stats(h_stats, n_series, sh, plan->opt.length_classes);
        }
        int rc = check_shape(plan, sh);
        if (rc) return rc;
        int *d_sel = nullptr;
        if (sh.n_groups > 1) {
            if (plan->sel.ensure((size_t)n_series * sizeof(int))) return fail(TSFA_ERR_HIP, "hipMalloc failed for the length-class lists");
            d_sel = (int *)plan->sel.p;
            if ((rc = build_sel(plan, starts, ends, n_series, sh, d_sel, st))) return rc;
        }
        if ((rc = run_batch(plan, values, dtype, plan->needs_times ? times : nullptr, starts, ends, n_series, out, ld_out, sh,
                            d_sel, st, true)))
            return rc;
        const bool async = (stream != nullptr);
        if (!async || plan->profiling) {
            HIP_TRY(hipStreamSynchronize(st));
            if (plan->profiling)
                for (auto &t : plan->timings) (void)hipEventElapsedTime(&t.ms, t.e0, t.e1);
        }
        return TSFA_OK;
    }

    hipStream_t st = plan->stream;
    const bool ragged = (ends == starts + 1);
    long long h_stats[TSFA_LEN_STATS];
    if (host_len_stats(starts, ends, n_series, h_stats))
        return fail(TSFA_ERR_INVALID, "a series ends before it starts (offsets must be non-decreasing)");
    {
        BatchShape whole;
        shape_from_stats(h_stats, n_series, whole, plan->opt.length_classes);
        const int rc = check_shape(plan, whole);
        if (rc) return rc;
    }
    int64_t base = starts[0], top = ends[0];
    if (ragged) {
        base = starts[0];
        top = starts[n_series];
    } else {
        for (int64_t i = 0; i < n_series; ++i) {
            base = std::min(base, starts[i]);
            top = std::max(top, ends[i]);
        }
    }
    const int64_t total = top - base;
    std::vector<int64_t> &rel = plan->h_rel;
    if (ragged) {
        rel.resize((size_t)n_series + 1);
        for (int64_t i = 0; i <= n_series; ++i) rel[(size_t)i] = starts[i] - base;
    } else {
        rel.resize(2 * (size_t)n_series);
        for (int64_t i = 0; i < n_series; ++i) {
            rel[(size_t)i] = starts[i] - base;
            rel[(size_t)(n_series + i)] = ends[i] - base;
        }
    }
    if (plan->values.ensure((size_t)total * esz + 16) || plan->offsets.ensure(rel.size() * sizeof(int64_t)) ||
        plan->out.ensure((size_t)n_series * plan->n_cols * sizeof(double)) ||
        plan->sel.ensure((size_t)n_series * sizeof(int)))
        return fail(TSFA_ERR_HIP, "hipMalloc failed for the staging buffers");
    const double *d_times = nullptr;
    if (plan->needs_times) {
        if (plan->times.ensure((size_t)total * sizeof(double) + 16)) return fail(TSFA_ERR_HIP, "hipMalloc failed for the times buffer");
        d_times = (const double *)plan->times.p;
    }
    const int64_t *d_starts = (const int64_t *)plan->offsets.p;
    const int64_t *d_ends = d_starts + (ragged ? 1 : n_series);
    double *d_out = (double *)plan->out.p;
    const int64_t ld = plan->n_cols;

    int n_chunks = (int)std::min<int64_t>(TSFA_MAX_CHUNKS, std::max<int64_t>(1, n_series / 4096));
    if (plan->opt.host_chunks >= 1) n_chunks = std::min(plan->opt.host_chunks, TSFA_MAX_CHUNKS);
    if (plan->profiling) n_chunks = 1;
    n_chunks = (int)std::min<int64_t>(n_chunks, n_series);

    HIP_TRY(hipMemcpyAsync(plan->offsets.p, rel.data(), rel.size() * sizeof(int64_t), hipMemcpyHostToDevice, plan->s_in));
    if (!ragged || n_chunks == 1) {
        HIP_TRY(hipMemcpyAsync(plan->values.p, (const char *)values + (size_t)base * esz, (size_t)total * esz,
                               hipMemcpyHostToDevice, plan->s_in));
        if (d_times)
            HIP_TRY(hipMemcpyAsync(plan->times.p, times + base, (size_t)total * sizeof(double), hipMemcpyHostToDevice, plan->s_in));
    }
    int rc = TSFA_OK;
    for (int c = 0; c < n_chunks && rc == TSFA_OK; ++c) {
        const int64_t c0 = n_series * c / n_chunks, c1 = n_series * (c + 1) / n_chunks;
        if (ragged && n_chunks > 1) {
            const int64_t v0 = rel[(size_t)c0], v1 = rel[(size_t)c1];
            HIP_TRY(hipMemcpyAsync((char *)plan->values.p + (size_t)v0 * esz, (const char *)values + (size_t)(base + v0) * esz,
                                   (size_t)(v1 - v0) * esz, hipMemcpyHostToDevice, plan->s_in));
            if (d_times)
                HIP_TRY(hipMemcpyAsync((char *)plan->times.p + (size_t)v0 * 8, times + base + v0, (size_t)(v1 - v0) * 8,
                                       hipMemcpyHostToDevice, plan->s_in));
        }
        HIP_TRY(hipEventRecord(plan->ev_in[c], plan->s_in));
        HIP_TRY(hipStreamWaitEvent(st, plan->ev_in[c], 0));
        long long cs[TSFA_LEN_STATS];
        host_len_stats(starts + c0, ends + c0, c1 - c0, cs);
        BatchShape sh;
        shape_from_stats(cs, c1 - c0, sh, plan->opt.length_classes);
        int *d_sel = (int *)plan->sel.p + c0;
        if ((rc = build_sel(plan, d_starts + c0, d_ends + c0, c1 - c0, sh, d_sel, st))) break;
        if ((rc = run_batch(plan, plan->values.p, dtype, d_times, d_starts + c0, d_ends + c0, c1 - c0, d_out + c0 * ld, ld,
                            sh, d_sel, st, n_chunks == 1)))
            break;
        HIP_TRY(hipEventRecord(plan->ev_k[c], st));
        HIP_TRY(hipStreamWaitEvent(plan->s_out, plan->ev_k[c], 0));
        HIP_TRY(hipMemcpy2DAsync(out + c0 * ld_out, (size_t)ld_out * sizeof(double), d_out + c0 * ld, (size_t)ld * sizeof(double),
                                 (size_t)plan->n_cols * sizeof(double), (size_t)(c1 - c0), hipMemcpyDeviceToHost, plan->s_out));
    }
    const hipError_t e1 = hipStreamSynchronize(plan->s_in), e2 = hipStreamSynchronize(st), e3 = hipStreamSynchronize(plan->s_out);
    if (rc) return rc;
    if (e1 != hipSuccess || e2 != hipSuccess || e3 != hipSuccess)
        return fail(TSFA_ERR_HIP, std::string("stream synchronize: ") + hipGetErrorString(e1 != hipSuccess ? e1 : (e2 != hipSuccess ? e2 : e3)));
    if (plan->profiling)
        for (auto &t : plan->timings) (void)hipEventElapsedTime(&t.ms, t.e0, t.e1);
    return TSFA_OK;
}

int tsfa_host_alloc(void **ptr, size_t bytes) {
    if (!ptr) return fail(TSFA_ERR_INVALID, "ptr is NULL");
    *ptr = nullptr;
    if (tsfa_device_count() <= 0) return fail(TSFA_ERR_NO_DEVICE, "no HIP device visible");
    HIP_TRY(hipHostMalloc(ptr, bytes ? bytes : 1, hipHostMallocDefault));
    return TSFA_OK;
}

int tsfa_host_free(void *ptr) {
    if (!ptr) return TSFA_OK;
    HIP_TRY(hipHostFree(ptr));
    return TSFA_OK;
}

}
```

tsfresh_amd/csrc/tsfa_kernels.hip:

```cpp
#include <hip/hip_runtime.h>

#include "fam_ar.h"
#include "fam_ar_dd.h"
#include "fam_basic.h"
#include "fam_cwt.h"
#include "fam_entropy.h"
#include "fam_seq.h"
#include "fam_perm.h"
#include "fam_sort.h"
#include "fam_spectral.h"
#include "fam_general.h"
#include "tsfa_launch.h"
#include "tsfa_layout.h"

#include <algorithm>

#if defined(TSFA_LONG)
#define TSFA_GS_PARAMS , unsigned char *__restrict__ gsc, size_t gslot
#define TSFA_GS_ARGS , gsc, gslot
#define TSFA_SERIES_BEGIN                                                           \
    unsigned char *const tsfa_base = gsc + (size_t)blockIdx.x * gslot;             \
    for (int64_t wi_ = blockIdx.x; wi_ < n_series; wi_ += gridDim.x) {             \
        const int64_t sidx = sel ? (int64_t)sel[wi_] : wi_;
#define TSFA_SERIES_END \
        __syncthreads(); \
    }
#define TSFA_SERIES_SKIP continue
#else
extern __shared__ __attribute__((aligned(16))) unsigned char tsfa_smem[];
#define TSFA_GS_PARAMS
#define TSFA_GS_ARGS
#define TSFA_SERIES_BEGIN                                                                                                   \
    if ((int64_t)blockIdx.x >= n_series) return;                                                                            \
    unsigned char *const tsfa_base = tsfa_smem;                                                                             \
    {                                                                                                                       \
        const int64_t sidx = sel ? (int64_t)sel[blockIdx.x] : (int64_t)blockIdx.x;
#define TSFA_SERIES_END }
#define TSFA_SERIES_SKIP return
#endif

template <typename T>
__device__ __forceinline__ void stage_series(const Blk &b, const T *__restrict__ g, int n, double *xs) {
    for (int i = b.tid; i < n; i += b.nt) xs[i] = (double)g[i];
    blk_sync();
}

template <typename T, int PART>
__device__ __forceinline__ void basic_body(const T *__restrict__ values, const int64_t *__restrict__ starts, const int64_t *__restrict__ ends, int64_t n_series, const int *__restrict__ sel,
                        const TsfaSpec *__restrict__ specs, int nspecs, double *__restrict__ out, int64_t ld,
                        const double *__restrict__ dectab, int maxn, int hint_a, int hint_b,
                        const double *__restrict__ times, const TsfaAltPlan &alt, int n_loop, int n_count, int n_sum,
                        double *__restrict__ stats_out, int skip_le TSFA_GS_PARAMS) {
    TSFA_SERIES_BEGIN
    const int64_t off = starts[sidx];
    const int n = (int)(ends[sidx] - off);
    if (n <= skip_le) TSFA_SERIES_SKIP;
    BasicLds L;
    L.carve(tsfa_base, maxn, blockDim.x, (int)sizeof(T), PART, (PART == 2) ? alt.small_w : 0);
    TSFA_TICKS_BEGIN();
    Blk b{(int)threadIdx.x, (int)blockDim.x, L.red, L.np};
    T *xs = (T *)L.xs;
    {
        const T *__restrict__ g = values + off;
        for (int i = b.tid; i < n; i += b.nt) xs[i] = g[i];
        blk_sync();
    }
    fam_basic_series<PART>(b, XsView<T>{xs}, n, specs, nspecs, out + sidx * ld, L.w, L.cum, L.altc, L.iw, dectab, hint_a,
                           hint_b, alt, L.stage, times ? times + off : nullptr, n_loop, L.ctx, n_count, n_sum,
                           stats_out ? stats_out + sidx * TSFA_STATS_N : nullptr);
    TSFA_TICKS_END();
    TSFA_SERIES_END
}

template <typename T>
__global__ void __launch_bounds__(1024) k_basic(const T *__restrict__ values, const int64_t *__restrict__ starts, const int64_t *__restrict__ ends, int64_t n_series, const int *__restrict__ sel,
                        const TsfaSpec *__restrict__ specs, int nspecs, double *__restrict__ out, int64_t ld,
                        const double *__restrict__ dectab, int maxn, int hint_a, int n_loop, int n_count, int n_sum,
                        double *__restrict__ stats_out, int skip_le TSFA_GS_PARAMS) {
    TsfaAltPlan alt;
    alt.nkeys = 0; alt.want_p = 0; alt.nq = 0; alt.small_w = 0;
    basic_body<T, 1>(values, starts, ends, n_series, sel, specs, nspecs, out, ld, dectab, maxn, hint_a, 0, nullptr, alt, n_loop,
                     n_count, n_sum, stats_out, skip_le TSFA_GS_ARGS);
}

template <typename T>
__global__ void __launch_bounds__(256, 4) k_basic_lite(const T *__restrict__ values, const int64_t *__restrict__ starts, const int64_t *__restrict__ ends, int64_t n_series, const int *__restrict__ sel,
                        const TsfaSpec *__restrict__ specs, int nspecs, double *__restrict__ out, int64_t ld,
                        const double *__restrict__ dectab, int maxn, int hint_a TSFA_GS_PARAMS) {
    TsfaAltPlan alt;
    alt.nkeys = 0; alt.want_p = 0; alt.nq = 0; alt.small_w = 0;
#if defined(TSFA_LONG)
    basic_body<T, 5>(values, starts, ends, n_series, sel, specs, nspecs, out, ld, dectab, maxn, hint_a, 0, nullptr, alt, 0, 0, 0, nullptr, 0 TSFA_GS_ARGS);
#else
    unsigned char *const tsfa_base = tsfa_smem;
    BasicLds L;
    L.carve(tsfa_base, maxn, blockDim.x, (int)sizeof(T), 1);
    const bool prefetch = (maxn <= 16 * (int)blockDim.x);
    Blk b{(int)threadIdx.x, (int)blockDim.x, L.red, L.np};
    T *xs = (T *)L.xs;
    T pre[16];
    int64_t sidx_n = 0;
    int n_n = 0;
    if ((int64_t)blockIdx.x < n_series) {
        sidx_n = sel ? (int64_t)sel[blockIdx.x] : (int64_t)blockIdx.x;
        const int64_t off = starts[sidx_n];
        n_n = (int)(ends[sidx_n] - off);
        if (prefetch) {
#pragma unroll
            for (int u = 0; u < 16; ++u) {
                const int i = b.tid + u * b.nt;
                pre[u] = (i < n_n) ? values[off + i] : (T)0;
            }
        }
    }
    for (int64_t wi = blockIdx.x; wi < n_series; wi += gridDim.x) {
        const int64_t sidx = sidx_n;
        const int n = n_n;
        if (prefetch) {
#pragma unroll
            for (int u = 0; u < 16; ++u) {
                const int i = b.tid + u * b.nt;
                if (i < n) xs[i] = pre[u];
            }
        } else {
            const T *__restrict__ g = values + starts[sidx];
            for (int i = b.tid; i < n; i += b.nt) xs[i] = g[i];
        }
        blk_sync();
        const int64_t wn = wi + gridDim.x;
        if (wn < n_series) {
            sidx_n = sel ? (int64_t)sel[wn] : wn;
            const int64_t off = starts[sidx_n];
            n_n = (int)(ends[sidx_n] - off);
            if (prefetch) {
#pragma unroll
                for (int u = 0; u < 16; ++u) {
                    const int i = b.tid + u * b.nt;
                    pre[u] = (i < n_n) ? values[off + i] : (T)0;
                }
            }
        }
        fam_basic_series<5>(b, XsView<T>{xs}, n, specs, nspecs, out + sidx * ld, L.w, L.cum, L.altc, L.iw, dectab, hint_a, 0,
                            alt, L.stage, nullptr, 0, L.ctx, 0, 0);
        blk_sync();
    }
#endif
}

template <typename T>
__global__ void __launch_bounds__(512) __attribute__((amdgpu_waves_per_eu(4))) k_trend(const T *__restrict__ values, const int64_t *__restrict__ starts, const int64_t *__restrict__ ends, int64_t n_series, const int *__restrict__ sel,
                        const TsfaSpec *__restrict__ specs, int nspecs, double *__restrict__ out, int64_t ld, int maxn,
                        int hint_b, const double *__restrict__ times, const TsfaAltPlan alt, int n_loop, int skip_le TSFA_GS_PARAMS) {
    basic_body<T, 2>(values, starts, ends, n_series, sel, specs, nspecs, out, ld, nullptr, maxn, 0, hint_b, times, alt, n_loop, 0, 0, nullptr, skip_le TSFA_GS_ARGS);
}

#if !defined(TSFA_LONG)
template <typename T, int PART>
__device__ __forceinline__ void basic_rows_body(const T *__restrict__ values, const int64_t *__restrict__ starts, const int64_t *__restrict__ ends, int64_t n_series, const int *__restrict__ sel,
                        const TsfaSpec *__restrict__ specs, int nspecs, double *__restrict__ out, int64_t ld,
                        const double *__restrict__ dectab, int maxn, int hint_a, int hint_b,
                        const double *__restrict__ times, const TsfaAltPlan &alt, int n_loop, int n_count, int n_sum,
                        double *__restrict__ stats_out, int row_bytes) {
    const int row = (int)(threadIdx.x >> 4);
    const int64_t wi = (int64_t)blockIdx.x * (64 / TSFA_ROW_LANES) + row;
    if (wi >= n_series) return;
    const int64_t sidx = sel ? (int64_t)sel[wi] : wi;
    const int64_t off = starts[sidx];
    const int n = (int)(ends[sidx] - off);
    if (n > TSFA_ROW_MAXN) return;
    BasicRowLds L;
    L.carve(tsfa_smem + (size_t)row * (size_t)row_bytes, maxn, (int)sizeof(T), PART, (PART == 2) ? alt.small_w : 0);
    BlkRow b;
    b.tid = (int)(threadIdx.x & (TSFA_ROW_LANES - 1));
    b.nt = TSFA_ROW_LANES;
    b.red = L.red;
    b.np = nullptr;
    T *xs = (T *)L.xs;
    {
        const T *__restrict__ g = values + off;
        for (int i = b.tid; i < n; i += TSFA_ROW_LANES) xs[i] = g[i];
        blk_sync();
    }
    fam_basic_series<PART>(b, XsView<T>{xs}, n, specs, nspecs, out + sidx * ld, L.w, L.cum, L.altc, L.iw, dectab, hint_a,
                           hint_b, alt, (TsfaSpec *)nullptr, times ? times + off : nullptr, n_loop, L.ctx, n_count, n_sum,
                           stats_out ? stats_out + sidx * TSFA_STATS_N : nullptr);
}

#if !defined(TSFA_ROWS_WPE)
#define TSFA_ROWS_WPE 4
#endif
template <typename T>
__global__ void __launch_bounds__(64) __attribute__((amdgpu_waves_per_eu(TSFA_ROWS_WPE))) k_basic_rows(const T *__restrict__ values, const int64_t *__restrict__ starts, const int64_t *__restrict__ ends, int64_t n_series, const int *__restrict__ sel,
                        const TsfaSpec *__restrict__ specs, int nspecs, double *__restrict__ out, int64_t ld,
                        const double *__restrict__ dectab, int maxn, int hint_a, int n_loop, int n_count, int n_sum,
                        double *__restrict__ stats_out, int row_bytes) {
    TsfaAltPlan alt;
    alt.nkeys = 0; alt.want_p = 0; alt.nq = 0; alt.small_w = 0;
    basic_rows_body<T, 1>(values, starts, ends, n_series, sel, specs, nspecs, out, ld, dectab, maxn, hint_a, 0, nullptr, alt, n_loop,
                          n_count, n_sum, stats_out, row_bytes);
}

template <typename T>
__global__ void __launch_bounds__(64) __attribute__((amdgpu_waves_per_eu(TSFA_ROWS_WPE))) k_trend_rows(const T *__restrict__ values, const int64_t *__restrict__ starts, const int64_t *__restrict__ ends, int64_t n_series, const int *__restrict__ sel,
                        const TsfaSpec *__restrict__ specs, int nspecs, double *__restrict__ out, int64_t ld, int maxn,
                        int hint_b, const double *__restrict__ times, const TsfaAltPlan alt, int n_loop, int row_bytes) {
    basic_rows_body<T, 2>(values, starts, ends, n_series, sel, specs, nspecs, out, ld, nullptr, maxn, 0, hint_b, times, alt, n_loop, 0, 0,
                          nullptr, row_bytes);
}
#endif

template <typename T>
__global__ void __launch_bounds__(1024) k_sort(const T *__restrict__ values, const int64_t *__restrict__ starts, const int64_t *__restrict__ ends, int64_t n_series, const int *__restrict__ sel,
                       const TsfaSpec *__restrict__ specs, int nspecs, double *__restrict__ out, int64_t ld, int maxn,
                       const TsfaCqPlan cqplan, int n_loop, int w_doubles, double *__restrict__ pf_buf,
                       int *__restrict__ pf_count, int pf_slot, int pf_cap, const unsigned short *__restrict__ perm_buf, int perm_stride,
                       const double *__restrict__ stats_in, int pe_hint TSFA_GS_PARAMS) {
    TSFA_SERIES_BEGIN
    const int64_t off = starts[sidx];
    const int n = (int)(ends[sidx] - off);
    SortLds L;
    L.carve(tsfa_base, maxn, blockDim.x, (int)sizeof(T), w_doubles);
    TSFA_TICKS_BEGIN();
    Blk b{(int)threadIdx.x, (int)blockDim.x, L.red, L.np};
    T *xs = (T *)L.xs;
    {
        const T *__restrict__ g = values + off;
        for (int i = b.tid; i < n; i += b.nt) xs[i] = g[i];
        blk_sync();
    }
    fam_sort_series<T>(b, xs, n, specs, nspecs, out + sidx * ld, (T *)L.srt, L.w, L.iw, cqplan, L.cq, L.stage,
                       n_loop, L.ctx, w_doubles, FrDefer{pf_buf, pf_count, pf_slot, (long long)sidx, 0, pf_cap},
                       perm_buf ? perm_buf + (size_t)sidx * (size_t)perm_stride : nullptr,
                       stats_in ? stats_in + sidx * TSFA_STATS_N : nullptr, pe_hint);
    TSFA_TICKS_END();
    TSFA_SERIES_END
}

#if !defined(TSFA_LONG)
template <typename T>
__global__ void __launch_bounds__(1024) k_perm(const T *__restrict__ values, const int64_t *__restrict__ starts, const int64_t *__restrict__ ends, int64_t n_series, const int *__restrict__ sel,
                       const TsfaSpec *__restrict__ specs, int nspecs, double *__restrict__ out, int64_t ld, int maxn, int tau) {
    TSFA_SERIES_BEGIN
    const int64_t off = starts[sidx];
    const int n = (int)(ends[sidx] - off);
    PermLds L;
    L.carve(tsfa_base, maxn, blockDim.x, (int)sizeof(T), TSFA_PE_HIST_WORDS, TSFA_PE_LOGS + TSFA_PE_MAXD + 1);
    TSFA_TICKS_BEGIN();
    Blk b{(int)threadIdx.x, (int)blockDim.x, L.red, nullptr};
    T *xs = (T *)L.xs;
    {
        const T *__restrict__ g = values + off;
        for (int i = b.tid; i < n; i += b.nt) xs[i] = g[i];
        blk_sync();
    }
    fam_perm_series<T>(b, xs, n, specs, nspecs, out + sidx * ld, tau, L.iw, L.ltab);
    TSFA_TICKS_END();
    TSFA_SERIES_END
}
#endif

template <typename T, bool BL>
__global__ void __launch_bounds__(1024) k_spectral(const T *__restrict__ values, const int64_t *__restrict__ starts, const int64_t *__restrict__ ends, int64_t n_series, const int *__restrict__ sel,
                           const TsfaSpec *__restrict__ specs, int nspecs, double *__restrict__ out, int64_t ld,
                           int maxn, int dft_n, double *__restrict__ gscratch, int gscratch_n, int bl_min,
                           const double *__restrict__ twc, const double *__restrict__ tws, int hint_a, int hint_b,
                           const double *__restrict__ consts TSFA_GS_PARAMS) {
    TSFA_SERIES_BEGIN
    const int64_t off = starts[sidx];
    const int n = (int)(ends[sidx] - off);
    SpectralLds L;
    L.carve(tsfa_base, maxn, dft_n, (int)sizeof(T));
    TSFA_TICKS_BEGIN();
    Blk b{(int)threadIdx.x, (int)blockDim.x, L.red, nullptr};
    T *xs = (T *)L.xs;
    {
        const T *__restrict__ g = values + off;
        for (int i = b.tid; i < n; i += b.nt) xs[i] = g[i];
        blk_sync();
    }
    double *gs = gscratch ? gscratch + (size_t)blockIdx.x * (size_t)gscratch_n : nullptr;
    fam_spectral_series<T, BL>(b, xs, n, specs, nspecs, out + sidx * ld, L.Xr, L.Xi, L.tc, L.ts, L.win, L.pxx, L.iw, twc, tws,
                        hint_a, hint_b, gs, consts ? consts + TSFA_CONSTS_HANN : nullptr, L.chirp_tab(), bl_min);
    TSFA_TICKS_END();
    TSFA_SERIES_END
}

template <typename T>
__global__ void __launch_bounds__(1024) k_ar(const T *__restrict__ values, const int64_t *__restrict__ starts, const int64_t *__restrict__ ends, int64_t n_series, const int *__restrict__ sel,
                     const TsfaSpec *__restrict__ specs, int nspecs, double *__restrict__ out, int64_t ld, int maxn,
                     int P, int hint_acf, int hint_pacf, int hint_adf, int n_loop, long long *__restrict__ deg_list,
                     int *__restrict__ deg_count, const double *__restrict__ stats_in TSFA_GS_PARAMS) {
    TSFA_SERIES_BEGIN
    const int64_t off = starts[sidx];
    const int n = (int)(ends[sidx] - off);
    ArLds L;
    L.carve(tsfa_base, maxn, P, (int)sizeof(T));
    TSFA_TICKS_BEGIN();
    Blk b{(int)threadIdx.x, (int)blockDim.x, L.red, L.np};
    const T *g = values + off;
    const int flags = fam_ar_series<T>(b, [=](int i) { return (double)g[i]; }, n, specs, nspecs, out + sidx * ld,
                                       (void *)L.xc, L.aw, P, hint_acf, hint_pacf, hint_adf, n_loop,
                                       stats_in ? stats_in + sidx * TSFA_STATS_N : nullptr);
    if (flags && threadIdx.x == 0) deg_list[atomicAdd(deg_count, 1)] = ((long long)sidx << 2) | flags;
    TSFA_TICKS_END();
    TSFA_SERIES_END
}

#if !defined(TSFA_LONG)
__global__ void __launch_bounds__(64) k_langevin_dd(const double *__restrict__ pf_buf, const int *__restrict__ pf_count, int pf_slot, int pf_cap,
                     const TsfaSpec *__restrict__ specs, int nspecs, double *__restrict__ out, int64_t ld) {
    const int cnt = min(*pf_count, pf_cap);
    const int rmax = (pf_slot - TSFA_PF_HDR) / 2;
    for (int i = blockIdx.x * 64 + threadIdx.x; i < cnt; i += gridDim.x * 64) {
        const double *rec = pf_buf + (size_t)i * (size_t)pf_slot;
        const int64_t sidx = (int64_t)rec[0];
        const int sp0 = (int)rec[1], k = (int)rec[2];
        const TsfaSpec s0 = specs[sp0];
        int m, r;
        if (s0.calc == TSFA_C_FRIEDRICH_COEFFICIENTS) { m = (int)s0.p[1]; r = (int)s0.p[2]; }
        else { m = (int)s0.p[0]; r = (int)s0.p[1]; }
        double coef[TSFA_PF_MAXC];
        const double *xm = rec + TSFA_PF_HDR, *ym = rec + TSFA_PF_HDR + rmax;
        polyfit_svd_dd([=](int j) { return xm[j]; }, [=](int j) { return ym[j]; }, k, m, coef);
        double *row = out + sidx * ld;
        for (int s = 0; s < nspecs; ++s) {
            const TsfaSpec sp = specs[s];
            if (sp.calc == TSFA_C_FRIEDRICH_COEFFICIENTS && (int)sp.p[1] == m && (int)sp.p[2] == r) {
                const int c = (int)sp.p[0];
                row[sp.col] = (c >= 0 && c <= m) ? coef[c] : TSFA_NAN;
            } else if (sp.calc == TSFA_C_MAX_LANGEVIN_FIXED_POINT && (int)sp.p[0] == m && (int)sp.p[1] == r) {
                row[sp.col] = max_real_root_deg3(coef, m + 1);
            }
        }
    }
}

template <typename T>
__global__ void __launch_bounds__(64) k_ar_degenerate(const T *__restrict__ values, const int64_t *__restrict__ starts, const int64_t *__restrict__ ends,
                     const TsfaSpec *__restrict__ specs, int nspecs, double *__restrict__ out, int64_t ld, int P,
                     const long long *__restrict__ deg_list, const int *__restrict__ deg_count, int adf_mode,
                     double *__restrict__ gscratch) {
    ArDdLds L;
    L.carve(tsfa_smem, P);
    if (gscratch != nullptr) L.scratch = gscratch + (size_t)blockIdx.x * (size_t)ArDdLds::scratch_doubles(P);
    Blk b{(int)threadIdx.x, (int)blockDim.x, L.red, nullptr};
    const int cnt = *deg_count;
    for (int i = blockIdx.x; i < cnt; i += gridDim.x) {
        const long long e = deg_list[i];
        const int64_t sidx = e >> 2;
        const int64_t off = starts[sidx];
        const int n = (int)(ends[sidx] - off);
        const T *g = values + off;
        fam_ar_degenerate_series(b, [=](int k) { return (double)g[k]; }, n, specs, nspecs, out + sidx * ld, L.scratch, P,
                                 (int)(e & 3), adf_mode);
        blk_sync();
    }
}

#endif

template <typename T, bool FAST>
__global__ void __launch_bounds__(1024) k_entropy(const T *__restrict__ values, const int64_t *__restrict__ starts, const int64_t *__restrict__ ends, int64_t n_series, const int *__restrict__ sel,
                          const TsfaSpec *__restrict__ specs, int nspecs, double *__restrict__ out, int64_t ld,
                          int maxn, int with_cnt, const double *__restrict__ stats_in TSFA_GS_PARAMS) {
    TSFA_SERIES_BEGIN
    const int64_t off = starts[sidx];
    const int n = (int)(ends[sidx] - off);
    EntropyLds L;
#if defined(TSFA_LONG)
    typedef unsigned int ent_idx;
#else
    typedef unsigned short ent_idx;
#endif
    L.carve(tsfa_base, maxn, with_cnt, (int)sizeof(ent_idx));
    TSFA_TICKS_BEGIN();
    Blk b{(int)threadIdx.x, (int)blockDim.x, L.red, L.np};
    stage_series(b, values + off, n, L.xs);
    fam_entropy_series<double, FAST, sizeof(T) == 4, ent_idx>(b, L.xs, n, specs, nspecs, out + sidx * ld, L.thr, (ent_idx *)(void *)L.perm,
                                                               L.refs, L.cnt, 1, stats_in ? stats_in + sidx * TSFA_STATS_N : nullptr);
    TSFA_TICKS_END();
    TSFA_SERIES_END
}

#if defined(TSFA_LONG)
extern __shared__ __attribute__((aligned(16))) unsigned char tsfa_hsmem[];
template <typename T>
__global__ void __launch_bounds__(1024) kl_entropy_hbits(const T *__restrict__ values, const int64_t *__restrict__ starts, const int64_t *__restrict__ ends, int64_t n_series, const int *__restrict__ sel,
                          const TsfaSpec *__restrict__ specs, int nspecs, double *__restrict__ out, int64_t ld, int maxn,
                          const double *__restrict__ stats_in, unsigned char *__restrict__ gsc, size_t gslot) {
    EntropyHugeSlot H;
    H.carve(gsc + (size_t)blockIdx.x * gslot, maxn);
    double *red = (double *)(void *)tsfa_hsmem;
    unsigned int *table = (unsigned int *)(void *)(tsfa_hsmem + TSFA_RED_DOUBLES * sizeof(double));
    unsigned int *wtot = (unsigned int *)(void *)(tsfa_hsmem + entropy_huge_lds_bytes(maxn) - 64 - (size_t)2 * TSFA_ENTB_MAXWAVES * TSFA_ENTH_S * sizeof(unsigned int));
    Blk b{(int)threadIdx.x, (int)blockDim.x, red, (NpScratch *)(void *)table};
    for (int64_t wi = blockIdx.x; wi < n_series; wi += gridDim.x) {
        const int64_t sidx = sel ? (int64_t)sel[wi] : wi;
        const int64_t off = starts[sidx];
        const int n = (int)(ends[sidx] - off);
        fam_entropy_series_hbits<T>(b, values + off, n, specs, nspecs, out + sidx * ld, H, table, wtot,
                                    stats_in ? stats_in + sidx * TSFA_STATS_N : nullptr);
        __syncthreads();
    }
}
#endif

#if !defined(TSFA_LONG)
template <typename T, int QW_>
__global__ void __launch_bounds__(1024) k_entropy_bits(const T *__restrict__ values, const int64_t *__restrict__ starts, const int64_t *__restrict__ ends, int64_t n_series, const int *__restrict__ sel,
                          const TsfaSpec *__restrict__ specs, int nspecs, double *__restrict__ out, int64_t ld, int maxn,
                          unsigned short *__restrict__ perm_buf, int perm_stride, const double *__restrict__ stats_in) {
    TSFA_SERIES_BEGIN
    const int64_t off = starts[sidx];
    const int n = (int)(ends[sidx] - off);
    EntropyLds L;
    L.carve(tsfa_base, maxn, QW_ == TSFA_ENTB_QW ? 2 : 3);
    TSFA_TICKS_BEGIN();
    Blk b{(int)threadIdx.x, (int)blockDim.x, L.red, L.np};
    stage_series(b, values + off, n, L.xs);
    const int kcap = (QW_ == TSFA_ENTB_QW) ? TSFA_ENTB_MAXK : entb_kround(maxn, TSFA_ENTB_MAXK, TSFA_ENTB_MAXWAVES);
    fam_entropy_series_bits<sizeof(T) == 4, QW_>(b, L.xs, n, specs, nspecs, out + sidx * ld, L.thr, L.perm, L.cnt,
                                            perm_buf ? perm_buf + (size_t)sidx * (size_t)perm_stride : nullptr, kcap,
                                            stats_in ? stats_in + sidx * TSFA_STATS_N : nullptr);
    TSFA_TICKS_END();
    TSFA_SERIES_END
}
#endif

template <typename T, bool GROWS>
__global__ void __launch_bounds__(256) k_seq(const T *__restrict__ values, const int64_t *__restrict__ starts, const int64_t *__restrict__ ends, int64_t n_series, const int *__restrict__ sel,
                      double *__restrict__ out, int64_t ld, const TsfaSeqGroup g, const double *__restrict__ stats_in,
                      unsigned char *__restrict__ rows TSFA_GS_PARAMS) {
    TSFA_SERIES_BEGIN
    const int64_t off = starts[sidx];
    const int n = (int)(ends[sidx] - off);
    SeqLds L;
    L.carve(tsfa_base, GROWS ? 0 : 1, g.stride, g.ttotal, g.etotal, (int)(blockDim.x + 63) >> 6);
    TSFA_TICKS_BEGIN();
    Blk b{(int)threadIdx.x, (int)blockDim.x, L.red, nullptr};
    const T *gv = values + off;
    fam_seq_series<GROWS>(b, [=](int i) { return (double)gv[i]; }, n, g, out + sidx * ld,
                          GROWS ? rows + (size_t)blockIdx.x * (size_t)g.stride : L.seq, L.tab, L.edges,
                          stats_in ? stats_in + sidx * TSFA_STATS_N : nullptr);
    TSFA_TICKS_END();
    TSFA_SERIES_END
}

template <typename T, int MAXT, bool MFMA>
__global__ void __launch_bounds__(MAXT, (MAXT == 256) ? 6 : 4) k_cwtpeaks(const T *__restrict__ values, const int64_t *__restrict__ starts, const int64_t *__restrict__ ends, int64_t n_series, const int *__restrict__ sel,
                           const TsfaSpec *__restrict__ specs, int nspecs, double *__restrict__ out, int64_t ld,
                           int maxn, int with_rowv, const double *__restrict__ consts TSFA_GS_PARAMS) {
    TSFA_SERIES_BEGIN
    const int64_t off = starts[sidx];
    const int n = (int)(ends[sidx] - off);
    CwtPeaksLayout L;
    L.carve(tsfa_base, maxn, with_rowv & 1, (int)sizeof(T));
    L.p.rk = consts ? consts + TSFA_CONSTS_RICKER : nullptr;
    TSFA_TICKS_BEGIN();
    Blk b{(int)threadIdx.x, (int)blockDim.x, L.p.red, nullptr};
    const T *g = values + off;
    fam_cwtpeaks_series<T, MFMA>(b, [=](int i) { return (double)g[i]; }, n, specs, nspecs, out + sidx * ld, L.p);
    TSFA_TICKS_END();
    TSFA_SERIES_END
}

#if !defined(TSFA_LONG)
template <typename T> struct OsKey;
template <> struct OsKey<float> {
    typedef unsigned int key_t;
    static constexpr int BITS = 32;
    static __device__ __forceinline__ key_t enc(float v) {
        const unsigned int u = __float_as_uint(v);
        return (u & 0x80000000u) ? ~u : (u | 0x80000000u);
    }
    static __device__ __forceinline__ double dec(key_t k) {
        const unsigned int u = (k & 0x80000000u) ? (k & 0x7FFFFFFFu) : ~k;
        return (double)__uint_as_float(u);
    }
    static __device__ __forceinline__ key_t maxkey() { return 0xFFFFFFFFu; }
};
template <> struct OsKey<double> {
    typedef unsigned long long key_t;
    static constexpr int BITS = 64;
    static __device__ __forceinline__ key_t enc(double v) {
        const unsigned long long u = (unsigned long long)__double_as_longlong(v);
        return (u >> 63) ? ~u : (u | 0x8000000000000000ull);
    }
    static __device__ __forceinline__ double dec(key_t k) {
        const unsigned long long u = (k >> 63) ? (k & 0x7FFFFFFFFFFFFFFFull) : ~k;
        return __longlong_as_double((long long)u);
    }
    static __device__ __forceinline__ key_t maxkey() { return ~0ull; }
};

__device__ __forceinline__ int wave_sum_i32(int v) {
    v += __builtin_amdgcn_update_dpp(0, v, TSFA_DPP_QUAD_XOR1, 0xf, 0xf, false);
    v += __builtin_amdgcn_update_dpp(0, v, TSFA_DPP_QUAD_XOR2, 0xf, 0xf, false);
    v += __builtin_amdgcn_update_dpp(0, v, TSFA_DPP_ROW_HALF_MIRROR, 0xf, 0xf, false);
    v += __builtin_amdgcn_update_dpp(0, v, TSFA_DPP_ROW_MIRROR, 0xf, 0xf, false);
    return (__builtin_amdgcn_readlane(v, 0) + __builtin_amdgcn_readlane(v, 16)) +
           (__builtin_amdgcn_readlane(v, 32) + __builtin_amdgcn_readlane(v, 48));
}

template <typename K, int E, int BITS>
__device__ __forceinline__ K os_select(const K (&key)[E], int k) {
    K prefix = 0;
#pragma unroll 1
    for (int bit = BITS - 1; bit >= 0; --bit) {
        const K cand = prefix | ((K)1 << bit);
        int c = 0;
#pragma unroll
        for (int e = 0; e < E; ++e) c += __popcll(__ballot(key[e] < cand));
        if (c <= k) prefix = cand;
    }
    return prefix;
}

template <typename T, int E>
__global__ void __launch_bounds__(256) k_order_stats(const T *__restrict__ values, const int64_t *__restrict__ starts, const int64_t *__restrict__ ends, int64_t n_series,
                                                     const int *__restrict__ sel, const TsfaSpec *__restrict__ specs, int nspecs,
                                                     double *__restrict__ out, int64_t ld) {
    typedef OsKey<T> KC;
    typedef typename KC::key_t K;
    const int lane = threadIdx.x & 63;
    const int64_t wi = (int64_t)blockIdx.x * (blockDim.x >> 6) + (threadIdx.x >> 6);
    if (wi >= n_series) return;
    const int64_t sidx = sel ? (int64_t)sel[wi] : wi;
    const int64_t off = starts[sidx];
    const int n = (int)(ends[sidx] - off);
    const T *__restrict__ g = values + off;
    K key[E];
#pragma unroll
    for (int e = 0; e < E; ++e) {
        const int i = e * 64 + lane;
        key[e] = (i < n) ? KC::enc(g[i]) : KC::maxkey();
    }
    double *row = out + sidx * ld;
    int have_k = -1;
    double v_k = 0.0, v_k1 = 0.0;
    auto os = [&](int i) -> double {
        if (i == have_k) return v_k;
        if (i == have_k + 1 && have_k >= 0) return v_k1;
        const K kk = os_select<K, E, KC::BITS>(key, i);
        v_k = KC::dec(kk);
        int cle = 0;
        K nxt = KC::maxkey();
#pragma unroll
        for (int e = 0; e < E; ++e) {
            cle += __popcll(__ballot(key[e] <= kk));
            if (key[e] > kk && key[e] < nxt) nxt = key[e];
        }
#pragma unroll
        for (int o = 32; o > 0; o >>= 1) {
            const K t = (K)__shfl_xor(nxt, o);
            nxt = (t < nxt) ? t : nxt;
        }
        v_k1 = (cle >= i + 2 || i + 1 >= n) ? v_k : KC::dec(nxt);
        have_k = i;
        return v_k;
    };
    for (int s = 0; s < nspecs; ++s) {
        const TsfaSpec sp = specs[s];
        double res;
        if (sp.calc == TSFA_C_MEDIAN) {
            if (n & 1) res = os((n - 1) / 2);
            else { const double a0 = os(n / 2 - 1), a1 = os(n / 2); res = (0.0 + a0 + a1) / 2.0; }
        } else {
            res = np_quantile_sorted(os, n, sp.p[0]);
        }
        if (lane == 0) row[sp.col] = res;
    }
}

template <typename T, int E, bool FULL>
__device__ __forceinline__ void stream_body(const T (&v)[E], int n, int lane, typename OsKey<T>::key_t *w,
                                            const TsfaSpec *__restrict__ bspecs, int nb, const TsfaSpec *__restrict__ sspecs, int ns,
                                            int want_median, double *__restrict__ row) {
#pragma clang fp contract(fast)
    typedef OsKey<T> KC;
    typedef typename KC::key_t K;
    const double dn = (double)n;
    double s = 0.0;
    T tmn = (T)TSFA_INF, tmx = (T)-TSFA_INF;
#pragma unroll
    for (int e = 0; e < E; ++e) {
        const bool in = FULL || (e * 64 + lane < n);
        s += in ? (double)v[e] : 0.0;
        tmn = in ? (v[e] < tmn ? v[e] : tmn) : tmn;
        tmx = in ? (v[e] > tmx ? v[e] : tmx) : tmx;
    }
    s = wave_sum(s);
    const double mean = s / dn;
    double ssd = 0.0, sq = 0.0;
#pragma unroll
    for (int e = 0; e < E; ++e) {
        const bool in = FULL || (e * 64 + lane < n);
        const double x = (double)v[e], d = x - mean;
        ssd += in ? d * d : 0.0;
        sq += in ? x * x : 0.0;
    }
    ssd = wave_sum(ssd);
    sq = wave_sum(sq);
    const double mn = wave_min((double)tmn), mx = wave_max((double)tmx);
    const double var = ssd / dn, sd = sqrt(var);

    double med = TSFA_NAN;
    if (want_median) {
        const int k = (n - 1) / 2, k1 = n / 2;
        T lo = (T)(mean - 0.06 * sd), hi = (T)(mean + 0.06 * sd);
        int c_lo = 0, c_hi = 0;
        bool ok = false;
        if (sd > 0.0 && sd < TSFA_INF) {
#pragma unroll 1
            for (int it = 0; it < 4; ++it) {
                if (!((double)hi < TSFA_INF) || !((double)lo > -TSFA_INF)) break;
                c_lo = 0; c_hi = 0;
#pragma unroll
                for (int e = 0; e < E; ++e) {
                    c_lo += __popcll(__ballot(v[e] < lo));
                    c_hi += __popcll(__ballot(v[e] <= hi));
                }
                if (k >= c_lo && k1 < c_hi) {
                    if (c_hi - c_lo <= 64) { ok = true; break; }
                    const T mid = (T)(0.5 * ((double)lo + (double)hi));
                    int c_mid = 0;
#pragma unroll
                    for (int e = 0; e < E; ++e) c_mid += __popcll(__ballot(v[e] <= mid));
                    if (k1 < c_mid) hi = mid;
                    else if (k >= c_mid)
                        lo = (sizeof(T) == 4) ? (T)nextafterf((float)mid, INFINITY) : (T)nextafter((double)mid, (double)INFINITY);
                    else break;
                } else {
                    const double wd = (double)hi - (double)lo;
                    if (k < c_lo) { hi = (T)((double)lo + 0.5 * wd); lo = (T)((double)hi - 2.0 * wd); }
                    else { lo = (T)((double)hi - 0.5 * wd); hi = (T)((double)lo + 2.0 * wd); }
                }
            }
        }
        if (ok) {
            int base = 0;
#pragma unroll
            for (int e = 0; e < E; ++e) {
                const unsigned long long m = __ballot(v[e] >= lo && v[e] <= hi);
                const bool in = (m >> lane) & 1ull;
                const int pos = base + __popcll(m & ((1ull << lane) - 1ull));
                if (in) w[pos] = KC::enc(v[e]);
                base += __popcll(m);
            }
            __builtin_amdgcn_wave_barrier();
            K key = (lane < c_hi - c_lo) ? w[lane] : KC::maxkey();
#pragma unroll
            for (int kk = 2; kk <= 64; kk <<= 1) {
#pragma unroll
                for (int j = kk >> 1; j > 0; j >>= 1) {
                    const K o = (K)__shfl_xor(key, j);
                    const bool up = ((lane & kk) == 0), lower = ((lane & j) == 0);
                    const K a = key < o ? key : o, c = key < o ? o : key;
                    key = (lower == up) ? a : c;
                }
            }
            const K q0 = (K)__shfl(key, k - c_lo), q1 = (K)__shfl(key, k1 - c_lo);
            med = (n & 1) ? KC::dec(q0) : (0.0 + KC::dec(q0) + KC::dec(q1)) / 2.0;
        } else {
            K key[E];
#pragma unroll
            for (int e = 0; e < E; ++e) key[e] = (FULL || e * 64 + lane < n) ? KC::enc(v[e]) : KC::maxkey();
            const K q0 = os_select<K, E, KC::BITS>(key, k);
            double a0 = KC::dec(q0), a1 = a0;
            if (k1 != k) {
                int cle = 0;
                K nxt = KC::maxkey();
#pragma unroll
                for (int e = 0; e < E; ++e) {
                    cle += __popcll(__ballot(key[e] <= q0));
                    if (key[e] > q0 && key[e] < nxt) nxt = key[e];
                }
#pragma unroll
                for (int o = 32; o > 0; o >>= 1) {
                    const K t = (K)__shfl_xor(nxt, o);
                    nxt = (t < nxt) ? t : nxt;
                }
                a1 = (cle >= k1 + 1) ? a0 : KC::dec(nxt);
            }
            med = (n & 1) ? a0 : (0.0 + a0 + a1) / 2.0;
        }
    }
    for (int c = lane; c < nb + ns; c += 64) {
        const TsfaSpec sp = (c < nb) ? bspecs[c] : sspecs[c - nb];
        double r = TSFA_NAN;
        switch (sp.calc) {
        case TSFA_C_SUM_VALUES: r = s; break;
        case TSFA_C_MEAN: r = mean; break;
        case TSFA_C_LENGTH: r = dn; break;
        case TSFA_C_STANDARD_DEVIATION: r = sd; break;
        case TSFA_C_VARIANCE: r = var; break;
        case TSFA_C_ROOT_MEAN_SQUARE: r = sqrt(sq / dn); break;
        case TSFA_C_MAXIMUM: r = mx; break;
        case TSFA_C_ABSOLUTE_MAXIMUM: r = fmax(fabs(mx), fabs(mn)); break;
        case TSFA_C_MINIMUM: r = mn; break;
        case TSFA_C_ABS_ENERGY: r = sq; break;
        case TSFA_C_VARIATION_COEFFICIENT: r = (mean == 0.0) ? TSFA_NAN : sd / mean; break;
        case TSFA_C_MEDIAN: r = med; break;
        default: break;
        }
        row[sp.col] = r;
    }
}

template <typename T, int E>
__global__ void __launch_bounds__(256) k_stream(const T *__restrict__ values, const int64_t *__restrict__ starts, const int64_t *__restrict__ ends, int64_t n_series,
                                                const int *__restrict__ sel, const TsfaSpec *__restrict__ bspecs, int nb,
                                                const TsfaSpec *__restrict__ sspecs, int ns, int want_median,
                                                double *__restrict__ out, int64_t ld) {
    typedef OsKey<T> KC;
    typedef typename KC::key_t K;
    __shared__ K win[4][64];
    const int lane = threadIdx.x & 63;
    const int64_t wi = (int64_t)blockIdx.x * (blockDim.x >> 6) + (threadIdx.x >> 6);
    if (wi >= n_series) return;
    const int64_t sidx = sel ? (int64_t)sel[wi] : wi;
    const int64_t off = starts[sidx];
    const int n = (int)(ends[sidx] - off);
    const T *__restrict__ g = values + off;
    T v[E];
    K *w = win[threadIdx.x >> 6];
    double *row = out + sidx * ld;
    if (n == E * 64) {
#pragma unroll
        for (int e = 0; e < E; ++e) v[e] = g[e * 64 + lane];
        stream_body<T, E, true>(v, n, lane, w, bspecs, nb, sspecs, ns, want_median, row);
    } else {
#pragma unroll
        for (int e = 0; e < E; ++e) {
            const int i = e * 64 + lane;
            v[e] = (i < n) ? g[i] : (T)TSFA_INF;
        }
        stream_body<T, E, false>(v, n, lane, w, bspecs, nb, sspecs, ns, want_median, row);
    }
}

typedef double tsfa_d4 __attribute__((ext_vector_type(4)));

#define TSFA_CWT_KC 16
template <typename T, int CT>
__global__ void __launch_bounds__(256)
k_cwt_gemm(const T *__restrict__ values, const int64_t *__restrict__ starts, const int64_t *__restrict__ ends, int64_t n_series,
           const double *__restrict__ W, int S4, int C, const int *__restrict__ cols,
           const int *__restrict__ coeff_idx, double *__restrict__ out, int64_t ld) {
    constexpr int KC = TSFA_CWT_KC, NC = CT * 16;
    __shared__ double sA[2][64][KC + 1];
    __shared__ double sB[2][KC][NC + 2];
    __shared__ int lens[64];
    __shared__ long long offs[64];
    const int tid = threadIdx.x, lane = tid & 63, wave = tid >> 6;
    const int r = lane & 15, kq = lane >> 4;
    const int64_t base = (int64_t)blockIdx.x * 64;
    if (tid < 64) {
        const int64_t s = base + tid;
        long long off = 0;
        int len = 0;
        if (s < n_series) {
            off = starts[s];
            len = (int)(ends[s] - off);
        }
        lens[tid] = len;
        offs[tid] = off;
    }
    __syncthreads();
    double ra[4], rb[CT];
    auto fetch = [&](int k0) {
#pragma unroll
        for (int u = 0; u < 4; ++u) {
            const int i = tid + u * 256, m = i / KC, kk = i - m * KC, k = k0 + kk;
            ra[u] = (k < lens[m]) ? (double)values[offs[m] + k] : 0.0;
        }
#pragma unroll
        for (int u = 0; u < CT; ++u) {
            const int i = tid + u * 256, c = i / KC, kk = i - c * KC, k = k0 + kk;
            rb[u] = (k < S4) ? W[(size_t)c * S4 + k] : 0.0;
        }
    };
    auto put = [&](int buf) {
#pragma unroll
        for (int u = 0; u < 4; ++u) {
            const int i = tid + u * 256, m = i / KC, kk = i - m * KC;
            sA[buf][m][kk] = ra[u];
        }
#pragma unroll
        for (int u = 0; u < CT; ++u) {
            const int i = tid + u * 256, c = i / KC, kk = i - c * KC;
            sB[buf][kk][c] = rb[u];
        }
    };
    tsfa_d4 acc[CT];
#pragma unroll
    for (int ct = 0; ct < CT; ++ct) acc[ct] = (tsfa_d4){0.0, 0.0, 0.0, 0.0};
    const int nchunks = (S4 + KC - 1) / KC;
    fetch(0);
    put(0);
    __syncthreads();
    for (int ch = 0; ch < nchunks; ++ch) {
        const int buf = ch & 1;
        if (ch + 1 < nchunks) fetch((ch + 1) * KC);
#pragma unroll
        for (int ks = 0; ks < KC; ks += 4) {
            const double a = sA[buf][wave * 16 + r][ks + kq];
#pragma unroll
            for (int ct = 0; ct < CT; ++ct) {
                const double bv = sB[buf][ks + kq][ct * 16 + r];
                acc[ct] = __builtin_amdgcn_mfma_f64_16x16x4f64(a, bv, acc[ct], 0, 0, 0);
            }
        }
        if (ch + 1 < nchunks) put(buf ^ 1);
        __syncthreads();
    }
#pragma unroll
    for (int ct = 0; ct < CT; ++ct) {
        const int c = ct * 16 + r;
        if (c >= C) continue;
        const int col = cols[c], ci = coeff_idx[c];
#pragma unroll
        for (int v = 0; v < 4; ++v) {
            const int i = wave * 16 + 4 * v + kq;
            const int64_t srow = base + i;
            if (srow < n_series) out[srow * ld + col] = (ci < lens[i]) ? acc[ct][v] : TSFA_NAN;
        }
    }
}

__global__ void k_fill_nan(double *__restrict__ out, int64_t n_rows, int64_t n_cols, int64_t ld, double value) {
    const int64_t i = (int64_t)blockIdx.x * blockDim.x + threadIdx.x;
    const int64_t stride = (int64_t)gridDim.x * blockDim.x;
    if (ld == n_cols) {
        for (int64_t k = i; k < n_rows * n_cols; k += stride) out[k] = value;
    } else {
        for (int64_t k = i; k < n_rows * n_cols; k += stride) {
            const int64_t r = k / n_cols;
            out[r * ld + (k - r * n_cols)] = value;
        }
    }
}
__global__ void k_fill_cols(double *__restrict__ out, int64_t n_rows, const int *__restrict__ cols, int n_fill, int64_t ld, double value) {
    const int64_t total = n_rows * (int64_t)n_fill;
    for (int64_t k = (int64_t)blockIdx.x * blockDim.x + threadIdx.x; k < total; k += (int64_t)gridDim.x * blockDim.x) {
        const int64_t r = k / n_fill;
        out[r * ld + cols[k - r * n_fill]] = value;
    }
}

__device__ __forceinline__ int tsfa_len_class_dev(long long l) {
    int c = 0;
    while (c < TSFA_N_LEN_CLASSES - 1 && l > (64LL << c)) ++c;
    return c;
}
__global__ void __launch_bounds__(256) k_len_stats(const int64_t *__restrict__ starts, const int64_t *__restrict__ ends, int64_t n_series, long long *__restrict__ stats) {
    __shared__ long long acc[TSFA_LEN_STATS];
    for (int i = threadIdx.x; i < TSFA_LEN_STATS; i += blockDim.x) acc[i] = (i == 1) ? (1LL << 62) : 0;
    __syncthreads();
    for (int64_t s = (int64_t)blockIdx.x * blockDim.x + threadIdx.x; s < n_series;
         s += (int64_t)gridDim.x * blockDim.x) {
        const long long l = ends[s] - starts[s];
        const bool np2 = l > 0 && (l & (l - 1)) != 0;
        const int c = tsfa_len_class_dev(l);
        atomicMax(&acc[0], l);
        atomicMin(&acc[1], l);
        if (np2) atomicMax(&acc[2], l);
        atomicAdd((unsigned long long *)&acc[3 + c], 1ULL);
        atomicMax(&acc[3 + TSFA_N_LEN_CLASSES + c], l);
        if (np2) atomicMax(&acc[3 + 2 * TSFA_N_LEN_CLASSES + c], l);
    }
    __syncthreads();
    for (int i = threadIdx.x; i < TSFA_LEN_STATS; i += blockDim.x) {
        if (i == 1) atomicMin(&stats[1], acc[1]);
        else if (i >= 3 && i < 3 + TSFA_N_LEN_CLASSES) atomicAdd((unsigned long long *)&stats[i], (unsigned long long)acc[i]);
        else atomicMax(&stats[i], acc[i]);
    }
}

__global__ void __launch_bounds__(256) k_class_fill(const int64_t *__restrict__ starts, const int64_t *__restrict__ ends, int64_t n_series,
                                                    const TsfaClassMap g, int *__restrict__ cursor, int *__restrict__ sel) {
    for (int64_t s = (int64_t)blockIdx.x * blockDim.x + threadIdx.x; s < n_series;
         s += (int64_t)gridDim.x * blockDim.x) {
        const int grp = g.group_of[tsfa_len_class_dev(ends[s] - starts[s])];
        sel[g.base[grp] + atomicAdd(&cursor[grp], 1)] = (int)s;
    }
}

#endif

#define TSFA_LAUNCH_CHECK()                       \
    do {                                          \
        hipError_t e_ = hipGetLastError();        \
        if (e_ != hipSuccess) return (int)e_;     \
    } while (0)

template <typename K>
static int set_lds(K kern, size_t bytes) {
    if (bytes > 64 * 1024) {
        hipError_t e = hipFuncSetAttribute(reinterpret_cast<const void *>(kern),
                                           hipFuncAttributeMaxDynamicSharedMemorySize, (int)bytes);
        if (e != hipSuccess) return (int)e;
    }
    return 0;
}

#if defined(TSFA_LONG)
#define TSFA_KLAUNCH(kern, lds, ...)                                                                       \
    do {                                                                                                   \
        const size_t slot_ = ((size_t)(lds) + 255) & ~(size_t)255;                                          \
        const int64_t slots_ = (int64_t)(a.long_bytes / slot_);                                            \
        if (!a.long_scratch || slots_ < 1) return -2;                                                      \
        const dim3 lgrid_((unsigned)std::min<int64_t>(a.n_series, std::min<int64_t>(slots_, 2048)));       \
        kern<<<lgrid_, nt, 0, st>>>(__VA_ARGS__, a.long_scratch, slot_);                                   \
    } while (0)
#else
#define TSFA_KLAUNCH(kern, lds, ...)                           \
    do {                                                       \
        if ((rc = set_lds(kern, lds))) return rc;              \
        kern<<<grid, nt, lds, st>>>(__VA_ARGS__);              \
    } while (0)
#endif

template <typename T>
static int launch_all_t(const TsfaLaunch &a, const T *values) {
    hipStream_t st = (hipStream_t)a.stream;
    const dim3 grid((unsigned)a.n_series);
    const int nt = a.nt;
    int rc = 0;
    (void)grid; (void)rc;
    if (a.fam == TSFA_FAM_BASIC) {
        BasicLds L;
        const size_t lds = L.carve(nullptr, a.maxn, nt, (int)sizeof(T), 1);
        if (a.hint_c == 0 && nt <= 256) {
#if defined(TSFA_LONG)
            TSFA_KLAUNCH(k_basic_lite<T>, lds, values, a.starts, a.ends, a.n_series, a.sel, a.specs, a.nspecs, a.out, a.ld,
                         a.dectab, a.maxn, a.hint_a);
#else
            if ((rc = set_lds(k_basic_lite<T>, lds))) return rc;
            const int64_t resident = std::max<int64_t>(1, std::min<int64_t>(32, (int64_t)(TSFA_LDS_LIMIT / std::max<size_t>(lds, 1))));
            const dim3 pgrid((unsigned)std::min<int64_t>(a.n_series, 256 * resident));
            k_basic_lite<T><<<pgrid, nt, lds, st>>>(values, a.starts, a.ends, a.n_series, a.sel, a.specs, a.nspecs, a.out, a.ld,
                                                     a.dectab, a.maxn, a.hint_a);
#endif
        } else {
            TSFA_KLAUNCH(k_basic<T>, lds, values, a.starts, a.ends, a.n_series, a.sel, a.specs, a.nspecs, a.out, a.ld, a.dectab,
                         a.maxn, a.hint_a, a.hint_c, a.hint_d, a.hint_e, a.stats_out, a.skip_le);
        }
    } else if (a.fam == TSFA_FAM_TREND) {
        BasicLds L;
        const size_t lds = L.carve(nullptr, a.maxn, nt, (int)sizeof(T), 2, a.alt.small_w);
        TSFA_KLAUNCH(k_trend<T>, lds, values, a.starts, a.ends, a.n_series, a.sel, a.specs, a.nspecs, a.out, a.ld, a.maxn,
                     a.hint_b, a.times, a.alt, a.hint_c, a.skip_le);
    } else if (a.fam == TSFA_FAM_SORT) {
        SortLds L;
        const int wd = (a.hint_a >= 320) ? a.hint_a : 1280;
        const size_t lds = L.carve(nullptr, a.maxn, nt, (int)sizeof(T), wd);
        TSFA_KLAUNCH(k_sort<T>, lds, values, a.starts, a.ends, a.n_series, a.sel, a.specs, a.nspecs, a.out, a.ld, a.maxn, a.cq,
                     a.hint_c, wd, a.pf_buf, a.pf_count, a.pf_slot, a.pf_cap, a.perm_buf, a.perm_stride, a.stats_in, a.hint_d);
    } else if (a.fam == TSFA_FAM_SPECTRAL) {
        SpectralLds L;
        const size_t lds = L.carve(nullptr, a.maxn, a.dft_n, (int)sizeof(T));
        if (a.gscratch != nullptr) {
            auto kfn = k_spectral<T, true>;
#if defined(TSFA_LONG)
            TSFA_KLAUNCH(kfn, lds, values, a.starts, a.ends, a.n_series, a.sel, a.specs, a.nspecs, a.out, a.ld, a.maxn,
                         a.dft_n, a.gscratch, a.gscratch_n, a.bluestein_min, a.twc, a.tws, a.hint_a, a.hint_b, a.consts);
#else
            if ((rc = set_lds(kfn, lds))) return rc;
            const int64_t slots = std::max<int64_t>(a.gscratch_slots, 1);
            for (int64_t c0 = 0; c0 < a.n_series; c0 += slots) {
                const int64_t nc = std::min<int64_t>(slots, a.n_series - c0);
                const int64_t s0 = a.sel ? 0 : c0;
                kfn<<<dim3((unsigned)nc), nt, lds, st>>>(values, a.starts + s0, a.ends + s0, nc, a.sel ? a.sel + c0 : nullptr, a.specs,
                                                        a.nspecs, a.out + s0 * a.ld, a.ld, a.maxn, a.dft_n, a.gscratch,
                                                        a.gscratch_n, a.bluestein_min, a.twc, a.tws, a.hint_a, a.hint_b, a.consts);
            }
#endif
        } else {
            auto kfn = k_spectral<T, false>;
            TSFA_KLAUNCH(kfn, lds, values, a.starts, a.ends, a.n_series, a.sel, a.specs, a.nspecs, a.out, a.ld, a.maxn,
                         a.dft_n, a.gscratch, a.gscratch_n, a.bluestein_min, a.twc, a.tws, a.hint_a, a.hint_b, a.consts);
        }
    } else if (a.fam == TSFA_FAM_AR) {
        ArLds L;
        const size_t lds = L.carve(nullptr, a.maxn, a.ar_P, (int)sizeof(T));
        TSFA_KLAUNCH(k_ar<T>, lds, values, a.starts, a.ends, a.n_series, a.sel, a.specs, a.nspecs, a.out, a.ld, a.maxn, a.ar_P,
                     a.hint_a, a.hint_b, a.hint_c, a.hint_d, a.deg_list, a.deg_count, a.stats_in);
    } else if (a.fam == TSFA_FAM_ENTROPY) {
#if defined(TSFA_LONG)
        if (a.ent_cnt == 4) {
            EntropyHugeSlot H;
            const size_t slot_ = (H.carve(nullptr, a.maxn) + 255) & ~(size_t)255;
            const int64_t slots_ = (int64_t)(a.long_bytes / slot_);
            if (!a.long_scratch || slots_ < 1) return -2;
            const size_t hl = entropy_huge_lds_bytes(a.maxn);
            auto kfn = kl_entropy_hbits<T>;
            hipError_t e = hipFuncSetAttribute(reinterpret_cast<const void *>(kfn), hipFuncAttributeMaxDynamicSharedMemorySize, (int)hl);
            if (e != hipSuccess) return (int)e;
            const dim3 hgrid((unsigned)std::min<int64_t>(a.n_series, std::min<int64_t>(slots_, 512)));
            kfn<<<hgrid, 1024, hl, st>>>(values, a.starts, a.ends, a.n_series, a.sel, a.specs, a.nspecs, a.out, a.ld, a.maxn, a.stats_in,
                                         a.long_scratch, slot_);
            TSFA_LAUNCH_CHECK();
            return 0;
        }
#endif
        EntropyLds L;
#if defined(TSFA_LONG)
        const size_t lds = L.carve(nullptr, a.maxn, a.ent_cnt, 4);
#else
        const size_t lds = L.carve(nullptr, a.maxn, a.ent_cnt);
#endif
#if !defined(TSFA_LONG)
        if (a.ent_cnt == 3) {
            auto kfn = k_entropy_bits<T, TSFA_ENTB_QW_LONG>;
            TSFA_KLAUNCH(kfn, lds, values, a.starts, a.ends, a.n_series, a.sel, a.specs, a.nspecs, a.out, a.ld, a.maxn,
                         (unsigned short *)nullptr, 0, a.stats_in);
        } else if (a.ent_cnt == 2) {
            auto kfn = k_entropy_bits<T, TSFA_ENTB_QW>;
            TSFA_KLAUNCH(kfn, lds, values, a.starts, a.ends, a.n_series, a.sel, a.specs, a.nspecs, a.out, a.ld, a.maxn,
                         a.perm_buf, a.perm_stride, a.stats_in);
        } else
#endif
        if (a.ent_fast) {
            auto kfn = k_entropy<T, true>;
            TSFA_KLAUNCH(kfn, lds, values, a.starts, a.ends, a.n_series, a.sel, a.specs, a.nspecs, a.out, a.ld, a.maxn, a.ent_cnt, a.stats_in);
        } else {
            auto kfn = k_entropy<T, false>;
            TSFA_KLAUNCH(kfn, lds, values, a.starts, a.ends, a.n_series, a.sel, a.specs, a.nspecs, a.out, a.ld, a.maxn, a.ent_cnt, a.stats_in);
        }
    } else if (a.fam == TSFA_FAM_SEQ) {
        SeqLds L;
        const size_t lds = L.carve(nullptr, a.seq.grows ? 0 : 1, a.seq.stride, a.seq.ttotal, a.seq.etotal, (nt + 63) >> 6);
#if !defined(TSFA_LONG)
        if (a.seq.grows) {
            if (!a.seq_rows) return -2;
            auto kfn = k_seq<T, true>;
            TSFA_KLAUNCH(kfn, lds, values, a.starts, a.ends, a.n_series, a.sel, a.out, a.ld, a.seq, a.stats_in, a.seq_rows);
        } else
#endif
        {
            auto kfn = k_seq<T, false>;
            TSFA_KLAUNCH(kfn, lds, values, a.starts, a.ends, a.n_series, a.sel, a.out, a.ld, a.seq, a.stats_in, (unsigned char *)nullptr);
        }
    } else if (a.fam == TSFA_FAM_CWT) {
        CwtPeaksLayout L;
        const size_t lds = L.carve(nullptr, a.maxn, a.cwt_rowv & 1, (int)sizeof(T));
#if !defined(TSFA_LONG)
        if (a.cwt_rowv & 2) {
            if (nt <= 256) {
                auto kfn = k_cwtpeaks<T, 256, true>;
                TSFA_KLAUNCH(kfn, lds, values, a.starts, a.ends, a.n_series, a.sel, a.specs, a.nspecs, a.out, a.ld, a.maxn, a.cwt_rowv, a.consts);
            } else {
                auto kfn = k_cwtpeaks<T, 1024, true>;
                TSFA_KLAUNCH(kfn, lds, values, a.starts, a.ends, a.n_series, a.sel, a.specs, a.nspecs, a.out, a.ld, a.maxn, a.cwt_rowv, a.consts);
            }
        } else
#endif
        if (nt <= 256) {
            auto kfn = k_cwtpeaks<T, 256, false>;
            TSFA_KLAUNCH(kfn, lds, values, a.starts, a.ends, a.n_series, a.sel, a.specs, a.nspecs, a.out, a.ld, a.maxn, a.cwt_rowv, a.consts);
        } else {
            auto kfn = k_cwtpeaks<T, 1024, false>;
            TSFA_KLAUNCH(kfn, lds, values, a.starts, a.ends, a.n_series, a.sel, a.specs, a.nspecs, a.out, a.ld, a.maxn, a.cwt_rowv, a.consts);
        }
    } else {
        return -1;
    }
    TSFA_LAUNCH_CHECK();
    return 0;
}

#if !defined(TSFA_LONG)
template <typename T>
static int launch_rows_t(const TsfaLaunch &a, const T *values) {
    hipStream_t st = (hipStream_t)a.stream;
    const int per = 64 / TSFA_ROW_LANES;
    const dim3 grid((unsigned)((a.n_series + per - 1) / per));
    const int maxn = std::min(a.maxn, TSFA_ROW_MAXN);
    int rc = 0;
    if (a.fam == TSFA_FAM_BASIC) {
        const size_t rb = BasicRowLds::row_bytes(maxn, (int)sizeof(T), 1, 0);
        if ((rc = set_lds(k_basic_rows<T>, rb * per))) return rc;
        k_basic_rows<T><<<grid, 64, rb * per, st>>>(values, a.starts, a.ends, a.n_series, a.sel, a.specs, a.nspecs, a.out, a.ld, a.dectab,
                                                    maxn, a.hint_a, a.hint_c, a.hint_d, a.hint_e, a.stats_out, (int)rb);
    } else if (a.fam == TSFA_FAM_TREND) {
        const size_t rb = BasicRowLds::row_bytes(maxn, (int)sizeof(T), 2, a.alt.small_w);
        if ((rc = set_lds(k_trend_rows<T>, rb * per))) return rc;
        k_trend_rows<T><<<grid, 64, rb * per, st>>>(values, a.starts, a.ends, a.n_series, a.sel, a.specs, a.nspecs, a.out, a.ld, maxn,
                                                    a.hint_b, a.times, a.alt, a.hint_c, (int)rb);
    } else {
        return -1;
    }
    TSFA_LAUNCH_CHECK();
    return 0;
}
int tsfa_launch_rows(const TsfaLaunch &a) {
    if (a.dtype == 0) return launch_rows_t<float>(a, (const float *)a.values);
    return launch_rows_t<double>(a, (const double *)a.values);
}
#endif

#if defined(TSFA_LONG)
int tsfa_launch_family_long(const TsfaLaunch &a) {
    if (a.dtype == 0) return launch_all_t<float>(a, (const float *)a.values);
    return launch_all_t<double>(a, (const double *)a.values);
}

template <typename T>
__global__ void __launch_bounds__(64) k_general(const T *__restrict__ values, const int64_t *__restrict__ starts, const int64_t *__restrict__ ends,
                                               int64_t n_series, const TsfaSpec *__restrict__ specs, int nspecs, double *__restrict__ out, int64_t ld,
                                               int maxn, const TsfaGenPlan g, double *__restrict__ scratch, size_t slot_doubles,
                                               const double *__restrict__ pool) {
    __shared__ double red[TSFA_RED_DOUBLES];
    __shared__ NpScratch nps;
    Blk b{(int)threadIdx.x, (int)blockDim.x, red, &nps};
    GenSlot S;
    S.carve(scratch + (size_t)blockIdx.x * slot_doubles, maxn, g);
    for (int64_t sidx = blockIdx.x; sidx < n_series; sidx += gridDim.x) {
        const int64_t off = starts[sidx];
        const int n = (int)(ends[sidx] - off);
        const T *gv = values + off;
        fam_general_series(b, [=](int i) { return (double)gv[i]; }, n, specs, nspecs, out + sidx * ld, S, g, pool);
        __syncthreads();
    }
}

size_t tsfa_general_slot_doubles(int maxn, const TsfaGenPlan &g) {
    GenSlot S;
    return S.carve(nullptr, maxn, g);
}

int tsfa_launch_general(const TsfaLaunch &a, const TsfaGenPlan &g, double *scratch, size_t slot_doubles, int slots, const double *pool) {
    hipStream_t st = (hipStream_t)a.stream;
    const unsigned grid = (unsigned)std::max<int64_t>(1, std::min<int64_t>(a.n_series, slots));
    if (a.dtype == 0)
        k_general<float><<<grid, 64, 0, st>>>((const float *)a.values, a.starts, a.ends, a.n_series, a.specs, a.nspecs, a.out, a.ld, a.maxn, g,
                                              scratch, slot_doubles, pool);
    else
        k_general<double><<<grid, 64, 0, st>>>((const double *)a.values, a.starts, a.ends, a.n_series, a.specs, a.nspecs, a.out, a.ld, a.maxn, g,
                                               scratch, slot_doubles, pool);
    TSFA_LAUNCH_CHECK();
    return 0;
}
#else
template <typename T>
static int launch_ar_degenerate_t(const TsfaLaunch &a, const T *values) {
    hipStream_t st = (hipStream_t)a.stream;
    int rc;
    ArDdLds D;
    const int P = a.ar_P_dd > 0 ? a.ar_P_dd : a.ar_P;
    size_t dlds = D.carve(nullptr, P);
    unsigned dgrid = (unsigned)std::min<int64_t>(a.n_series, 4096);
    if (a.dd_scratch != nullptr) {
        dlds = (size_t)TSFA_RED_DOUBLES * sizeof(double) + 64;
        dgrid = (unsigned)std::max<int64_t>(1, std::min<int64_t>(a.n_series, a.dd_slots));
    }
    if ((rc = set_lds(k_ar_degenerate<T>, dlds))) return rc;
    k_ar_degenerate<T><<<dgrid, 64, dlds, st>>>(values, a.starts, a.ends, a.specs, a.nspecs, a.out, a.ld, P, a.deg_list,
                                                a.deg_count, (a.hint_c >> 1) & 3, a.dd_scratch);
    TSFA_LAUNCH_CHECK();
    return 0;
}
int tsfa_launch_ar_degenerate(const TsfaLaunch &a) {
    if (!(a.hint_c || a.ar_has_coef)) return 0;
    if (a.dtype == 0) return launch_ar_degenerate_t<float>(a, (const float *)a.values);
    return launch_ar_degenerate_t<double>(a, (const double *)a.values);
}

int tsfa_launch_langevin_dd(const TsfaLaunch &a) {
    if (!a.pf_buf) return 0;
    hipStream_t st = (hipStream_t)a.stream;
    const unsigned grid = (unsigned)std::min<int64_t>((a.n_series + 63) / 64, 4096);
    k_langevin_dd<<<grid, 64, 0, st>>>(a.pf_buf, a.pf_count, a.pf_slot, a.pf_cap, a.specs, a.nspecs, a.out, a.ld);
    TSFA_LAUNCH_CHECK();
    return 0;
}

size_t tsfa_entropy_lds_bytes(int maxn, int with_cnt) {
    if (with_cnt == 5) {
        EntropyLds L;
        return L.carve(nullptr, maxn, 0, 4);
    }
    if (with_cnt == 4) {
        EntropyHugeSlot H;
        return H.carve(nullptr, maxn);
    }
    EntropyLds L;
    return L.carve(nullptr, maxn, with_cnt);
}

size_t tsfa_seq_lds_bytes(const TsfaSeqGroup &g) {
    SeqLds L;
    return L.carve(nullptr, g.grows ? 0 : 1, g.stride, g.ttotal, g.etotal);
}

size_t tsfa_family_lds_bytes(int fam, int maxn, int nt, int aux) {
    switch (fam) {
    case TSFA_FAM_BASIC: { BasicLds L; return L.carve(nullptr, maxn, nt, 8, 1); }
    case TSFA_FAM_TREND: { BasicLds L; return L.carve(nullptr, maxn, nt, 8, 2, aux); }
    case TSFA_FAM_SORT: { SortLds L; return L.carve(nullptr, maxn, nt); }
    case TSFA_FAM_SPECTRAL: { SpectralLds L; return L.carve(nullptr, maxn, aux); }
    case TSFA_FAM_AR: { ArLds L; return L.carve(nullptr, maxn, aux); }
    case TSFA_FAM_CWT: {
        CwtPeaksLayout L;
        const size_t lds16 = L.carve(nullptr, maxn, aux, 8, 2);
        return lds16 > TSFA_LDS_LIMIT ? L.carve(nullptr, maxn, aux, 8, 4) : lds16;
    }
    default: return 0;
    }
}

int tsfa_launch_family(const TsfaLaunch &a) {
    if (a.dtype == 0) return launch_all_t<float>(a, (const float *)a.values);
    return launch_all_t<double>(a, (const double *)a.values);
}

template <typename T>
static int launch_order_stats_t(const TsfaLaunch &a, const T *values) {
    hipStream_t st = (hipStream_t)a.stream;
    const dim3 grid((unsigned)((a.n_series + 3) / 4));
    if (a.maxn <= 256)
        k_order_stats<T, 4><<<grid, 256, 0, st>>>(values, a.starts, a.ends, a.n_series, a.sel, a.specs, a.nspecs, a.out, a.ld);
    else if (a.maxn <= 1024)
        k_order_stats<T, 16><<<grid, 256, 0, st>>>(values, a.starts, a.ends, a.n_series, a.sel, a.specs, a.nspecs, a.out, a.ld);
    else if (a.maxn <= 2048)
        k_order_stats<T, 32><<<grid, 256, 0, st>>>(values, a.starts, a.ends, a.n_series, a.sel, a.specs, a.nspecs, a.out, a.ld);
    else
        return -1;
    TSFA_LAUNCH_CHECK();
    return 0;
}
template <typename T>
static int launch_stream_t(const TsfaLaunch &a, const T *values) {
    hipStream_t st = (hipStream_t)a.stream;
    const dim3 grid((unsigned)((a.n_series + 3) / 4));
    const int wm = a.nspecs > 0 ? 1 : 0;
#define TSFA_STREAM_CASE(EE) k_stream<T, EE><<<grid, 256, 0, st>>>(values, a.starts, a.ends, a.n_series, a.sel, a.bspecs, a.nbspecs, a.specs, a.nspecs, wm, a.out, a.ld)
    if (a.maxn <= 256) TSFA_STREAM_CASE(4);
    else if (a.maxn <= 512) TSFA_STREAM_CASE(8);
    else if (a.maxn <= 1024) TSFA_STREAM_CASE(16);
    else if (a.maxn <= 2048) TSFA_STREAM_CASE(32);
    else return -1;
#undef TSFA_STREAM_CASE
    TSFA_LAUNCH_CHECK();
    return 0;
}
int tsfa_launch_stream(const TsfaLaunch &a) {
    if (a.dtype == 0) return launch_stream_t<float>(a, (const float *)a.values);
    return launch_stream_t<double>(a, (const double *)a.values);
}
int tsfa_stream_calc_ok(int calc) {
    switch (calc) {
    case TSFA_C_SUM_VALUES: case TSFA_C_MEAN: case TSFA_C_LENGTH: case TSFA_C_STANDARD_DEVIATION: case TSFA_C_VARIANCE:
    case TSFA_C_ROOT_MEAN_SQUARE: case TSFA_C_MAXIMUM: case TSFA_C_ABSOLUTE_MAXIMUM: case TSFA_C_MINIMUM:
    case TSFA_C_ABS_ENERGY: case TSFA_C_VARIATION_COEFFICIENT: case TSFA_C_QUERY_SIMILARITY_COUNT: case TSFA_C_MEDIAN:
        return 1;
    default: return 0;
    }
}

size_t tsfa_perm_lds_bytes(int maxn, int nt, int elem_bytes) {
    PermLds L;
    return L.carve(nullptr, maxn, nt, elem_bytes, TSFA_PE_HIST_WORDS, TSFA_PE_LOGS + TSFA_PE_MAXD + 1);
}
template <typename T>
static int launch_perm_t(const TsfaLaunch &a, const T *values) {
    hipStream_t st = (hipStream_t)a.stream;
    const dim3 grid((unsigned)a.n_series);
    const int nt = a.nt;
    const size_t lds = tsfa_perm_lds_bytes(a.maxn, nt, (int)sizeof(T));
    int rc = 0;
    if ((rc = set_lds(k_perm<T>, lds))) return rc;
    k_perm<T><<<grid, nt, lds, st>>>(values, a.starts, a.ends, a.n_series, a.sel, a.specs, a.nspecs, a.out, a.ld, a.maxn, a.hint_d >> 8);
    TSFA_LAUNCH_CHECK();
    return 0;
}
int tsfa_launch_perm(const TsfaLaunch &a) {
    if (((unsigned)a.hint_d & 0xFFu) != TSFA_PE_MASK || (a.hint_d >> 8) < 1) return -1;
    if (a.dtype == 0) return launch_perm_t<float>(a, (const float *)a.values);
    return launch_perm_t<double>(a, (const double *)a.values);
}

int tsfa_launch_order_stats(const TsfaLaunch &a) {
    if (a.dtype == 0) return launch_order_stats_t<float>(a, (const float *)a.values);
    return launch_order_stats_t<double>(a, (const double *)a.values);
}

template <typename T>
static int launch_cwt_t(const TsfaCwtLaunch &a, const T *values) {
    hipStream_t st = (hipStream_t)a.stream;
    const int ct = (a.C + 15) / 16;
    const dim3 grid((unsigned)((a.n_series + 63) / 64));
#define TSFA_CWT_CASE(N)                                                                                         \
    case N:                                                                                                      \
        k_cwt_gemm<T, N><<<grid, 256, 0, st>>>(values, a.starts, a.ends, a.n_series, a.W, a.S4, a.C, a.cols, a.coeff_idx, \
                                               a.out, a.ld);                                                     \
        break;
    switch (ct) {
        TSFA_CWT_CASE(1)
        TSFA_CWT_CASE(2)
        TSFA_CWT_CASE(3)
        TSFA_CWT_CASE(4)
        TSFA_CWT_CASE(5)
        TSFA_CWT_CASE(6)
        TSFA_CWT_CASE(7)
        TSFA_CWT_CASE(8)
    default: return -1;
    }
#undef TSFA_CWT_CASE
    TSFA_LAUNCH_CHECK();
    return 0;
}

int tsfa_launch_cwt(const TsfaCwtLaunch &a) {
    if (a.dtype == 0) return launch_cwt_t<float>(a, (const float *)a.values);
    return launch_cwt_t<double>(a, (const double *)a.values);
}

int tsfa_launch_fill_nan(double *out, int64_t n_rows, int64_t n_cols, int64_t ld, void *stream, double value,
                         const int *cols, int n_fill) {
    if (cols == nullptr) k_fill_nan<<<2048, 256, 0, (hipStream_t)stream>>>(out, n_rows, n_cols, ld, value);
    else if (n_fill > 0) {
        const int64_t total = n_rows * (int64_t)n_fill;
        k_fill_cols<<<(unsigned)std::min<int64_t>((total + 255) / 256, 2048), 256, 0, (hipStream_t)stream>>>(out, n_rows, cols, n_fill, ld, value);
    }
    TSFA_LAUNCH_CHECK();
    return 0;
}

int tsfa_launch_len_stats(const int64_t *starts, const int64_t *ends, int64_t n_series, long long *stats, void *stream) {
    k_len_stats<<<256, 256, 0, (hipStream_t)stream>>>(starts, ends, n_series, stats);
    TSFA_LAUNCH_CHECK();
    return 0;
}

int tsfa_launch_class_fill(const int64_t *starts, const int64_t *ends, int64_t n_series, const TsfaClassMap &g, int *cursor,
                           int *sel, void *stream) {
    k_class_fill<<<256, 256, 0, (hipStream_t)stream>>>(starts, ends, n_series, g, cursor, sel);
    TSFA_LAUNCH_CHECK();
    return 0;
}

#ifdef TSFA_TICKS
extern "C" int tsfa_debug_ticks(unsigned long long *out, int n, int reset) {
    if (n > 256) n = 256;
    if (out && hipMemcpyFromSymbol(out, HIP_SYMBOL(tsfa_ticks), (size_t)n * sizeof(unsigned long long)) != hipSuccess) return -1;
    if (reset) {
        static unsigned long long zeros[256];
        if (hipMemcpyToSymbol(HIP_SYMBOL(tsfa_ticks), zeros, sizeof zeros) != hipSuccess) return -1;
    }
    return 0;
}
#endif
#endif
```

tsfresh_amd/csrc/tsfa_layout.h:

```cpp
#ifndef TSFA_LAYOUT_H
#define TSFA_LAYOUT_H

#include <stddef.h>
#include <stdint.h>

#include "tsfa_common.h"
#include "fam_cwt.h"
#include "fam_seq.h"
#include "tsfa_entb_params.h"

#if defined(__HIPCC__)
#define TSFA_HD __host__ __device__ inline
#else
#define TSFA_HD inline
#endif

#define TSFA_LDS_LIMIT (160 * 1024)

struct LdsCarve {
    unsigned char *base;
    size_t off;
    template <class U>
    TSFA_HD U *take(size_t count) {
        off = (off + 15) & ~(size_t)15;
        U *r = (U *)(base + off);
        off += count * sizeof(U);
        return r;
    }
};

TSFA_HD int tsfa_pow2_ceil(int n) {
    int p = 1;
    while (p < n) p <<= 1;
    return p;
}

struct BasicLds {
    double *red; NpScratch *np; void *xs; double *w; double *cum; double *altc; int *iw; TsfaSpec *stage; double *ctx;
    TSFA_HD size_t carve(unsigned char *base, int maxn, int nt, int xs_bytes = 8, int part = 3, int small_w = 0) {
        LdsCarve c{base, 0};
        red = c.take<double>(nt <= 64 ? 2 : TSFA_RED_DOUBLES);
        xs = c.take<unsigned char>((size_t)maxn * xs_bytes);
        size_t wb = (part & 2) ? (size_t)maxn * sizeof(double) : (size_t)maxn * xs_bytes;
        if ((part & 2) && small_w) wb = (size_t)(nt + 2 * 16 + 8) * sizeof(double);
        if (wb < sizeof(NpScratch)) wb = sizeof(NpScratch);
        unsigned char *u = c.take<unsigned char>(wb);
        w = (double *)u;
        cum = w;
        np = (NpScratch *)u;
        altc = (part & 2) ? c.take<double>(8 * 16) : nullptr;
        ctx = c.take<double>(32);
        iw = c.take<int>((4 * nt > 256) ? 4 * nt : 256);
#if defined(TSFA_SPEC_LDS)
        stage = c.take<TsfaSpec>(TSFA_SPEC_BATCH);
#else
        stage = nullptr;
#endif
        return c.off;
    }
};

#define TSFA_ROW_BINS 64
struct BasicRowLds {
    double *red; void *xs; double *w; double *cum; double *altc; int *iw; double *ctx;
    TSFA_HD static size_t row_bytes(int maxn, int xs_bytes, int part, int small_w) {
        BasicRowLds L;
        const size_t used = L.carve(nullptr, maxn, xs_bytes, part, small_w);
        return ((used + 127) & ~(size_t)127) + 64;
    }
    TSFA_HD size_t carve(unsigned char *base, int maxn, int xs_bytes, int part, int small_w) {
        LdsCarve c{base, 0};
        red = c.take<double>(2);
        xs = c.take<unsigned char>((size_t)maxn * xs_bytes);
        size_t wb = (part & 2) ? (size_t)maxn * sizeof(double) : (size_t)maxn * xs_bytes;
        if ((part & 2) && small_w) wb = (size_t)(TSFA_ROW_LANES + 2 * 16 + 8) * sizeof(double);
        if (wb < 64) wb = 64;
        w = (double *)c.take<unsigned char>(wb);
        cum = w;
        altc = (part & 2) ? c.take<double>(8 * 16) : nullptr;
        ctx = c.take<double>(32);
        iw = c.take<int>((part & 2) ? 16 * 6 * 2 : TSFA_ROW_BINS);
        return c.off;
    }
};

struct SortLds {
    double *red; NpScratch *np; void *xs; void *srt; double *w; int *iw; double *cq; TsfaSpec *stage; double *ctx;
    TSFA_HD size_t carve(unsigned char *base, int maxn, int nt, int xs_bytes = 8, int w_doubles = 1280) {
        (void)nt;
        LdsCarve c{base, 0};
        red = c.take<double>(TSFA_RED_DOUBLES);
        np = c.take<NpScratch>(1);
        xs = c.take<unsigned char>((size_t)maxn * xs_bytes);
        srt = c.take<unsigned char>((size_t)tsfa_pow2_ceil(maxn) * xs_bytes);
        w = c.take<double>(w_doubles);
        iw = (int *)w;
        cq = c.take<double>(5 * TSFA_CQ_MAX);
        ctx = c.take<double>(8);
#if defined(TSFA_SPEC_LDS)
        stage = c.take<TsfaSpec>(TSFA_SPEC_BATCH);
#else
        stage = nullptr;
#endif
        return c.off;
    }
};

struct SpectralLds {
    double *red; void *xs; double *Xr; double *Xi; double *tc; double *ts; double *win; double *pxx; int *iw;
    TSFA_HD size_t carve(unsigned char *base, int maxn, int dft_n, int xs_bytes = 8) {
        LdsCarve c{base, 0};
        red = c.take<double>(TSFA_RED_DOUBLES);
        xs = c.take<unsigned char>((size_t)maxn * xs_bytes);
        const int nx = (maxn / 2 + 2 > 260) ? maxn / 2 + 2 : 260;
        Xr = c.take<double>(nx);
        Xi = c.take<double>(nx);
        const int nd = (dft_n > 256) ? dft_n : (dft_n > 0 ? 256 : 2);
        tc = c.take<double>(nd);
        ts = c.take<double>(nd);
        win = c.take<double>(256);
        pxx = c.take<double>(dft_n > 0 ? 260 : 132);
        iw = (int *)(void *)win;
        has_chirp_tab = (nd == 256 && dft_n > 0);
        return c.off;
    }
    bool has_chirp_tab = false;
    TSFA_HD double *chirp_tab() const { return has_chirp_tab ? tc : nullptr; }
};

struct ArLds {
    double *red; NpScratch *np; double *xc; double *aw;
    TSFA_HD static int scratch_doubles(int P) { return 2 * P * P + 7 * P + 64 + 16 + 48 + 40 + 128; }
    TSFA_HD size_t carve(unsigned char *base, int maxn, int P, int xs_bytes = 8) {
        LdsCarve c{base, 0};
        red = c.take<double>(TSFA_RED_DOUBLES);
        xc = (double *)(void *)c.take<unsigned char>((size_t)(maxn + 64 + 16) * xs_bytes);
        const size_t ab = (size_t)scratch_doubles(P) * sizeof(double);
        unsigned char *u = c.take<unsigned char>(ab > sizeof(NpScratch) ? ab : sizeof(NpScratch));
        aw = (double *)u;
        np = (NpScratch *)u;
        return c.off;
    }
};

struct ArDdLds {
    double *red; double *scratch;
    TSFA_HD static int scratch_doubles(int P) { return 4 * P * P + 19 * (P + 1) + P + 10; }
    TSFA_HD size_t carve(unsigned char *base, int P) {
        LdsCarve c{base, 0};
        red = c.take<double>(TSFA_RED_DOUBLES);
        scratch = c.take<double>((size_t)scratch_doubles(P));
        return c.off;
    }
};

struct EntropyLds {
    double *red; NpScratch *np; double *xs; double *thr; unsigned short *perm; unsigned int *refs; unsigned int *cnt;
    TSFA_HD size_t carve(unsigned char *base, int maxn, int with_cnt, int idx_bytes = 2) {
        LdsCarve c{base, 0};
        red = c.take<double>(TSFA_RED_DOUBLES);
        thr = c.take<double>(56);
        xs = c.take<double>(maxn + 4);
        const int np2 = tsfa_pow2_ceil(maxn);
        const int nperm = ((np2 > 64) ? np2 : 64) + 32;
        perm = (unsigned short *)(void *)c.take<unsigned char>((size_t)nperm * (size_t)idx_bytes);
        if (with_cnt == 2 || with_cnt == 3) {
            refs = nullptr;
            const size_t cb = (with_cnt == 2 ? entb_work_words(maxn)
                                             : entb_work_words(maxn, TSFA_ENTB_QW_LONG + 1, entb_kround(maxn, TSFA_ENTB_MAXK, TSFA_ENTB_MAXWAVES))) * sizeof(unsigned int);
            unsigned char *u = c.take<unsigned char>(cb > sizeof(NpScratch) ? cb : sizeof(NpScratch));
            np = (NpScratch *)u;
            cnt = (unsigned int *)u;
        } else if (with_cnt) {
            refs = c.take<unsigned int>(nperm);
            const size_t cb = (size_t)(maxn + 16) * ((maxn <= 1024) ? 4 : 3) * sizeof(unsigned int);
            unsigned char *u = c.take<unsigned char>(cb > sizeof(NpScratch) ? cb : sizeof(NpScratch));
            np = (NpScratch *)u;
            cnt = (unsigned int *)u;
        } else {
            np = c.take<NpScratch>(1);
            refs = nullptr;
            cnt = nullptr;
        }
        return c.off;
    }
};

struct EntropyHugeSlot {
    double *thr; double *xs; double *xsrt; unsigned short *perm; unsigned int *rng; unsigned int *cnt; unsigned int *pre;
    TSFA_HD size_t carve(unsigned char *base, int maxn) {
        LdsCarve c{base, 0};
        thr = c.take<double>(64);
        xs = c.take<double>((size_t)maxn + 4);
        const int np2 = tsfa_pow2_ceil(maxn);
        xsrt = c.take<double>((size_t)np2);
        perm = c.take<unsigned short>((size_t)np2 + 32);
        rng = c.take<unsigned int>((size_t)TSFA_ENTB_MAXK * maxn);
        cnt = c.take<unsigned int>((size_t)TSFA_ENTB_MAXK * maxn + 8);
        pre = c.take<unsigned int>((size_t)((maxn + 32) >> 5) * 1024 * 2);
        return c.off;
    }
};
TSFA_HD size_t entropy_huge_lds_bytes(int maxn) {
    const size_t e = ((size_t)maxn + 1023) / 1024;
    size_t table = ((size_t)1024 * (e | 1) + 2) * TSFA_ENTH_S * sizeof(unsigned int);
    if (table < sizeof(NpScratch) + 64) table = sizeof(NpScratch) + 64;
    const size_t totals = (2 * TSFA_ENTB_MAXK * TSFA_ENTB_MAXWAVES * 4) * sizeof(double) + (2 * TSFA_ENTB_MAXK * TSFA_ENTB_MAXWAVES + 4) * sizeof(unsigned int);
    if (table < totals) table = totals;
    return TSFA_RED_DOUBLES * sizeof(double) + ((table + 15) & ~(size_t)15) + (size_t)2 * TSFA_ENTB_MAXWAVES * TSFA_ENTH_S * sizeof(unsigned int) + 64;
}


struct SeqLds {
    double *red; unsigned char *seq; uint32_t *tab; double *edges;
    TSFA_HD size_t carve(unsigned char *base, int group, int stride, int tab_words, int edge_doubles, int nwaves = 16) {
        LdsCarve c{base, 0};
        red = c.take<double>(nwaves < 2 ? 2 : (nwaves + 1) & ~1);
        edges = c.take<double>(edge_doubles + 2);
        tab = c.take<uint32_t>((size_t)tab_words);
        seq = c.take<unsigned char>((size_t)group * stride + 16);
        return c.off;
    }
};


struct PermLds {
    double *red; double *ltab; int *iw; void *xs;
    TSFA_HD size_t carve(unsigned char *base, int maxn, int nt, int elem_bytes, int hist_words, int log_doubles) {
        LdsCarve c{base, 0};
        const int nwaves = (nt + 63) >> 6;
        red = c.take<double>(nwaves * 8 < 16 ? 16 : nwaves * 8);
        ltab = c.take<double>((size_t)log_doubles);
        iw = c.take<int>((size_t)hist_words + 4);
        xs = (void *)c.take<unsigned char>((size_t)(maxn + 8) * elem_bytes);
        return c.off;
    }
};

struct CwtPeaksLayout {
    CwtPeaksLds p;
    TSFA_HD size_t carve(unsigned char *base, int maxn, int mode, int xs_bytes = 8, int idx_bytes = (int)sizeof(cwt_idx_t)) {
        LdsCarve c{base, 0};
        p.red = c.take<double>(TSFA_RED_DOUBLES);
        p.row0 = c.take<double>(maxn + 4);
        p.rowv = nullptr;
        p.xpad = mode ? (void *)c.take<unsigned char>((size_t)(maxn + 2 * TSFA_CWTP_HALO + 8) * xs_bytes) : nullptr;
        p.taps = c.take<double>(TSFA_CWTP_MAXTAPS + 16);
        p.mask = c.take<unsigned short>(maxn);
        p.lcol = (cwt_idx_t *)(void *)c.take<unsigned char>((2 * (size_t)maxn + 8) * idx_bytes);
        p.linf = p.lcol + maxn;
        p.colmap = (cwt_idx_t *)(void *)c.take<unsigned char>(2 * (size_t)maxn * idx_bytes);
        p.mline = p.colmap + maxn;
        p.misc = c.take<int>(8);
        return c.off;
    }
};

#endif
```

Before: 2.702 million.

## Pack AR Gram matrices triangularly, single-wave AR blocks with waitcnt-only sync

Stores the AR/ADF Cholesky Gram matrices in packed lower-triangular form, which shrinks the LDS scratch so more blocks can be resident. The lag-product recurrences are rebuilt with wave-level shuffles and readlanes instead of a serial thread-0 loop. The AR family now defaults to 64 threads per block. With a single wave, block barriers are replaced by an lgkmcnt wait, and a separate cross-wave partial-sum buffer is allocated only when there is more than one wave. This depends on intra-wave lockstep for correctness and adds index arithmetic to every matrix access.

Result: faster. 2.818 million, median of 6 (+4.3%).

```diff
diff --git a/tsfresh_amd/csrc/fam_ar.h b/tsfresh_amd/csrc/fam_ar.h
--- a/tsfresh_amd/csrc/fam_ar.h
+++ b/tsfresh_amd/csrc/fam_ar.h
@@ -10,107 +10,121 @@
     return maxlag;
 }
 
-TSFA_DEV bool chol_factor(double *G, int p, int ld) {
+TSFA_DEV int ar_tri(int i, int j) { return ((i * (i + 1)) >> 1) + j; }
+TSFA_DEV int ar_tri_doubles(int P) { return (P * (P - 1)) / 2; }
+
+TSFA_DEV void ar_sync(const Blk &b) {
+#if TSFA_GPU && !defined(TSFA_LONG)
+    if (b.nt <= 64) {
+        asm volatile("s_waitcnt lgkmcnt(0)" ::: "memory");
+        return;
+    }
+#endif
+    (void)b;
+    blk_sync();
+}
+
+TSFA_DEV bool chol_factor(double *G, int p) {
     for (int j = 0; j < p; ++j) {
-        double d = G[j + j * ld];
-        for (int k = 0; k < j; ++k) d -= G[j + k * ld] * G[j + k * ld];
+        double d = G[ar_tri(j, j)];
+        for (int k = 0; k < j; ++k) d -= G[ar_tri(j, k)] * G[ar_tri(j, k)];
         if (!(d > 0.0)) return false;
         d = sqrt(d);
-        G[j + j * ld] = d;
+        G[ar_tri(j, j)] = d;
         for (int i = j + 1; i < p; ++i) {
-            double s = G[i + j * ld];
-            for (int k = 0; k < j; ++k) s -= G[i + k * ld] * G[j + k * ld];
-            G[i + j * ld] = s / d;
+            double s = G[ar_tri(i, j)];
+            for (int k = 0; k < j; ++k) s -= G[ar_tri(i, k)] * G[ar_tri(j, k)];
+            G[ar_tri(i, j)] = s / d;
         }
     }
     return true;
 }
-TSFA_DEV void chol_solve(const double *L, int p, int ld, const double *rhs, double *x) {
+TSFA_DEV void chol_solve(const double *L, int p, const double *rhs, double *x) {
     for (int i = 0; i < p; ++i) {
         double s = rhs[i];
-        for (int k = 0; k < i; ++k) s -= L[i + k * ld] * x[k];
-        x[i] = s * (1.0 / L[i + i * ld]);
+        for (int k = 0; k < i; ++k) s -= L[ar_tri(i, k)] * x[k];
+        x[i] = s * (1.0 / L[ar_tri(i, i)]);
     }
     for (int i = p - 1; i >= 0; --i) {
         double s = x[i];
-        for (int k = i + 1; k < p; ++k) s -= L[k + i * ld] * x[k];
-        x[i] = s * (1.0 / L[i + i * ld]);
-    }
-}
-
-TSFA_DEV void blk_chol_solve(const Blk &b, const double *L, int p, int ld, const double *rhs, double *x) {
+        for (int k = i + 1; k < p; ++k) s -= L[ar_tri(k, i)] * x[k];
+        x[i] = s * (1.0 / L[ar_tri(i, i)]);
+    }
+}
+
+TSFA_DEV void blk_chol_solve(const Blk &b, const double *L, int p, const double *rhs, double *x) {
 #if TSFA_GPU
     const int lane = b.tid & 63;
     const bool live = lane < p;
     double s = live ? rhs[lane] : 0.0;
-    const double dg = live ? 1.0 / L[lane + lane * ld] : 1.0;
+    const double dg = live ? 1.0 / L[ar_tri(lane, lane)] : 1.0;
     for (int k = 0; k < p; ++k) {
         const double wk = readlane_f64(s, k) * readlane_f64(dg, k);
         if (lane == k) s = wk;
-        else if (live && lane > k) s -= L[lane + k * ld] * wk;
+        else if (live && lane > k) s -= L[ar_tri(lane, k)] * wk;
     }
     for (int k = p - 1; k >= 0; --k) {
         const double xk = readlane_f64(s, k) * readlane_f64(dg, k);
         if (lane == k) s = xk;
-        else if (live && lane < k) s -= L[k + lane * ld] * xk;
+        else if (live && lane < k) s -= L[ar_tri(k, lane)] * xk;
     }
     if (b.tid < p) x[b.tid] = s;
 #else
-    if (b.tid == 0) chol_solve(L, p, ld, rhs, x);
+    if (b.tid == 0) chol_solve(L, p, rhs, x);
 #endif
 }
 
 #define TSFA_AR_PIVOT_TOL 1e-6
-TSFA_DEV bool blk_chol_factor(const Blk &b, double *G, int p, int ld, double *diag0, double *dmin = nullptr) {
-    for (int a = b.tid; a < p; a += b.nt) diag0[a] = G[a + a * ld];
+TSFA_DEV bool blk_chol_factor(const Blk &b, double *G, int p, double *diag0, double *dmin = nullptr) {
+    for (int a = b.tid; a < p; a += b.nt) diag0[a] = G[ar_tri(a, a)];
     double dm = TSFA_INF;
     for (int j = 0; j < p; ++j) {
-        blk_sync();
-        const double d = G[j + j * ld];
+        ar_sync(b);
+        const double d = G[ar_tri(j, j)];
         if (!(d > TSFA_AR_PIVOT_TOL * diag0[j])) return false;
         dm = fmin(dm, d);
         if (dmin) *dmin = dm;
         const double sd = sqrt(d);
-        blk_sync();
+        ar_sync(b);
         const double rsd = 1.0 / sd;
-        for (int i = j + b.tid; i < p; i += b.nt) G[i + j * ld] = (i == j) ? sd : G[i + j * ld] * rsd;
-        blk_sync();
+        for (int i = j + b.tid; i < p; i += b.nt) G[ar_tri(i, j)] = (i == j) ? sd : G[ar_tri(i, j)] * rsd;
+        ar_sync(b);
         const int rsh = (b.nt >= 32) ? 5 : 0;
         for (int i = j + 1 + (b.tid & ((1 << rsh) - 1)); i < p; i += (1 << rsh)) {
-            const double lij = G[i + j * ld];
+            const double lij = G[ar_tri(i, j)];
             for (int k = j + 1 + (b.tid >> rsh); k <= i; k += (b.nt >> rsh))
-                G[i + k * ld] = G[i + k * ld] - lij * G[k + j * ld];
-        }
-    }
-    blk_sync();
+                G[ar_tri(i, k)] = G[ar_tri(i, k)] - lij * G[ar_tri(k, j)];
+        }
+    }
+    ar_sync(b);
     return true;
 }
-TSFA_DEV void blk_chol_forward(const Blk &b, const double *L, int p, int ld, double *w) {
+TSFA_DEV void blk_chol_forward(const Blk &b, const double *L, int p, double *w) {
 #if TSFA_GPU
     if (p <= 64) {
         const int lane = b.tid & 63;
         const bool live = lane < p;
         double s = live ? w[lane] : 0.0;
-        const double dg = live ? 1.0 / L[lane + lane * ld] : 1.0;
+        const double dg = live ? 1.0 / L[ar_tri(lane, lane)] : 1.0;
         for (int k = 0; k < p; ++k) {
             const double wk = readlane_f64(s, k) * readlane_f64(dg, k);
             if (lane == k) s = wk;
-            else if (live && lane > k) s = s - L[lane + k * ld] * wk;
-        }
-        blk_sync();
+            else if (live && lane > k) s = s - L[ar_tri(lane, k)] * wk;
+        }
+        ar_sync(b);
         if (b.tid < p) w[b.tid] = s;
-        blk_sync();
+        ar_sync(b);
         return;
     }
 #endif
     for (int i = 0; i < p; ++i) {
-        blk_sync();
-        const double wi = w[i] * (1.0 / L[i + i * ld]);
-        blk_sync();
+        ar_sync(b);
+        const double wi = w[i] * (1.0 / L[ar_tri(i, i)]);
+        ar_sync(b);
         if (b.tid == 0) w[i] = wi;
-        for (int k = i + 1 + b.tid; k < p; k += b.nt) w[k] = w[k] - L[k + i * ld] * wi;
-    }
-    blk_sync();
+        for (int k = i + 1 + b.tid; k < p; k += b.nt) w[k] = w[k] - L[ar_tri(k, i)] * wi;
+    }
+    ar_sync(b);
 }
 
 
@@ -176,7 +190,7 @@
 #else
     const int nwv = 1, wv = 0;
 #endif
-    const bool deferred = (part != nullptr) && (nwv * TSFA_AR_PART_STRIDE <= part_doubles) && (nlags <= 64);
+    const bool deferred = (part != nullptr) && (nwv > 1) && (nwv * TSFA_AR_PART_STRIDE <= part_doubles) && (nlags <= 64);
     if (deferred) blk_sync();
     double A[8], lo[8], hi[8];
     for (int j0 = 0; j0 < nlags; j0 += 8) {
@@ -245,20 +259,47 @@
 }
 
 template <class S>
-TSFA_DEV void blk_lag_products_rest(const Blk &b, S s, int Lg, int t0, int t1, double *T, int ld, double *C) {
-    if (b.tid == 0) {
+TSFA_DEV void ar_lag_products_into(const Blk &b, S s, int Lg, int t0, int t1, const double *Tc, double *G, int off,
+                                   double *C = nullptr, double c0 = 0.0) {
+#if TSFA_GPU
+    if (b.tid < 64) {
+        const int lane = b.tid;
+        const double sa = (lane < Lg) ? s(t0 - 1 - lane) : 0.0;
+        const double sb = (lane < Lg) ? s(t1 - 1 - lane) : 0.0;
+        if (C != nullptr) {
+            double c = c0, mine = c0;
+            for (int j = 0; j < Lg; ++j) {
+                c = c + readlane_f64(sa, j) - readlane_f64(sb, j);
+                if (lane == j + 1) mine = c;
+            }
+            if (lane <= Lg) C[lane] = mine;
+        }
+        const int dg = lane;
+        double v = (dg < Lg) ? Tc[dg] : 0.0;
+        for (int j = 0; j < Lg; ++j) {
+            const int i = dg + j;
+            const int src = (i < 64) ? i : 0;
+            const double ai = __shfl(sa, src), bi = __shfl(sb, src);
+            if (i + 1 <= Lg) {
+                v = v + ai * readlane_f64(sa, j) - bi * readlane_f64(sb, j);
+                G[ar_tri(i + 1 + off, j + 1 + off)] = v;
+            }
+        }
+    }
+#else
+    if (b.tid == 0 && C != nullptr) {
+        C[0] = c0;
         for (int j = 0; j < Lg; ++j) C[j + 1] = C[j] + s(t0 - 1 - j) - s(t1 - 1 - j);
     }
-    blk_sync();
     for (int dg = b.tid; dg <= Lg; dg += b.nt) {
-        double v = T[dg];
+        double v = Tc[dg];
         for (int j = 0; dg + j + 1 <= Lg; ++j) {
             const int i = dg + j;
             v = v + s(t0 - 1 - i) * s(t0 - 1 - j) - s(t1 - 1 - i) * s(t1 - 1 - j);
-            T[(i + 1) + (j + 1) * ld] = v;
-        }
-    }
-    blk_sync();
+            G[ar_tri(i + 1 + off, j + 1 + off)] = v;
+        }
+    }
+#endif
 }
 
 TSFA_DEV double mackinnon_p_c1(double t) {
@@ -270,7 +311,7 @@
     return tsfa_norm_cdf(z);
 }
 
-TSFA_DEV int ar_scratch_doubles(int P) { return 2 * P * P + 7 * P + 64 + 16 + 48 + 40 + 128; }
+TSFA_DEV int ar_scratch_doubles(int P) { return ar_tri_doubles(P) + 8 * P + 64 + 8 + 48 + 32; }
 
 #define TSFA_AR_REFINE_TOL 1e-8
 TSFA_DEV bool ar_refinement_suspect(const Blk &b, const double *beta, const double *corr, const double *diag0, int p) {
@@ -309,12 +350,12 @@
 template <class ST, class X>
 TSFA_DEV int fam_ar_series(const Blk &b, X xv, int n, const TsfaSpec *specs, int nspecs, double *out_row, void *xc_raw,
                             double *aw, int P, int hint_acf, int hint_pacf, int hint_adf, int n_loop = -1,
-                            const double *stats = nullptr) {
+                            const double *stats = nullptr, double *part = nullptr, int part_doubles = 0) {
     const int nloop = (n_loop >= 0) ? n_loop : nspecs;
     const double dn = (double)n;
     TSFA_TICKER(tk, 0);
     const double mean = stats ? stats[TSFA_STATS_MEAN] : np_sum(b, n, [=](int i) { return xv(i); }) / dn;
-    blk_sync();
+    ar_sync(b);
     ST *xs_lds = (ST *)xc_raw + TSFA_AR_PADL;
     for (int i = b.tid; i < n + TSFA_AR_PADL + TSFA_AR_PADR; i += b.nt) {
         const int j = i - TSFA_AR_PADL;
@@ -322,14 +363,14 @@
     }
     const ArCentred<ST> xc{xs_lds, mean};
     const ArBlocks<ST> blk{xs_lds, mean};
-    blk_sync();
+    ar_sync(b);
     double v0 = 0.0;
     for (int i = b.tid; i < n; i += b.nt) v0 += xc[i] * xc[i];
     const double var = blk_sum(b, v0) / dn;
 
-    double *T = aw;
-    double *G = T + P * P;
-    double *g = G + P * P;
+    double *G = aw;
+    double *Tc = G + ar_tri_doubles(P);
+    double *g = Tc + P;
     double *beta = g + P;
     double *tmp1 = beta + P;
     double *tmp2 = tmp1 + P;
@@ -338,11 +379,12 @@
     double *diag0 = V + P;
     double *acv = diag0 + P;
     double *res = acv + 64;
-    double *pac = res + 16;
+    double *pac = res + 8;
     double *arres = pac + 48;
-    double *pacw = arres + 40;
     const ArCentred<ST> xcc = xc;
     int degenerate = 0;
+    double *const pt = part ? part : G;
+    const int ptn = part ? part_doubles : ar_tri_doubles(P);
 
     TSFA_TICK(tk, b, 120);
     int max_acf_lag = hint_acf, max_pacf_lag = hint_pacf;
@@ -364,9 +406,9 @@
 #pragma unroll
                              for (int q = 0; q < 8; ++q) B[q] = (i0 >= 0) ? B[q] : 0.0;
                          },
-                         [=](int k, double v) { acv[k] = v / (double)(n - k); }, nullptr, G, P * P);
-    }
-    blk_sync();
+                         [=](int k, double v) { acv[k] = v / (double)(n - k); }, nullptr, pt, ptn);
+    }
+    ar_sync(b);
 
     TSFA_TICK(tk, b, 121);
     if (max_pacf_lag >= 0) {
@@ -374,7 +416,7 @@
         {
             const int lane = b.tid & 63;
             for (int k = b.tid; k <= max_pacf_lag; k += b.nt) pac[k] = TSFA_NAN;
-            blk_sync();
+            ar_sync(b);
             if (n > 1 && pacf_maxlag > 0) {
                 const int ord = pacf_maxlag;
                 const double a0 = acv[0], a1 = acv[1];
@@ -402,7 +444,7 @@
             for (int k = 0; k <= max_pacf_lag; ++k) pac[k] = TSFA_NAN;
             if (n > 1 && pacf_maxlag > 0) {
                 const int ord = pacf_maxlag;
-                double *prev = pacw, *cur = pacw + 42, *sig = pacw + 84;
+                double prev[42], cur[42], sig[42];
                 prev[1] = acv[1] / acv[0];
                 pac[1] = prev[1];
                 sig[1] = acv[0] - prev[1] * acv[1];
@@ -420,7 +462,7 @@
             }
         }
 #endif
-        blk_sync();
+        ar_sync(b);
     }
 
     TSFA_TICK(tk, b, 122);
@@ -436,35 +478,31 @@
             double sd[2], sl[2];
             blk_tile_lagdots(b, n, maxlag + 1,
                              [=](int tb, double (&A)[8]) { blk.d8(tb, A); tile_mask_rows(A, tb, t0, t1); }, d_blocks,
-                             [=](int j, double v) { T[j] = v; }, sd, G, P * P);
+                             [=](int j, double v) { Tc[j] = v; }, sd, pt, ptn);
             blk_tile_lagdots(b, n, maxlag + 1,
                              [=](int tb, double (&A)[8]) { blk.y8(tb, A); tile_mask_rows(A, tb, t0, t1); }, d_blocks,
-                             [=](int j, double v) { V[j] = v; }, sl, G, P * P);
-            if (b.tid == 0) C[0] = sd[0];
-            blk_lag_products_rest(b, dif, maxlag, t0, t1, T, P, C);
+                             [=](int j, double v) { V[j] = v; }, sl, pt, ptn);
+            ar_sync(b);
+            ar_lag_products_into(b, dif, maxlag, t0, t1, Tc, G, 1, C, sd[0]);
+            ar_sync(b);
             const double sx = sl[0], sxx = sl[1];
             const int p1 = maxlag + 2;
-            for (int e = b.tid; e < 64 * p1; e += b.nt) {
-                const int a = e & 63, c = e >> 6;
-                if (a >= p1 || c > a) continue;
+            for (int e = b.tid; e < 2 * p1; e += b.nt) {
+                const int c = (e >= p1) ? 1 : 0, a = e - c * p1;
+                if (c > a) continue;
                 double v;
                 if (a == 0) v = nobs;
                 else if (a == 1) v = (c == 0) ? sx : sxx;
-                else {
-                    const int la = a - 1;
-                    if (c == 0) v = C[la];
-                    else if (c == 1) v = V[la];
-                    else v = T[la + (c - 1) * P];
-                }
-                G[a + c * P] = v;
-            }
-            for (int a = b.tid; a < p1; a += b.nt) g[a] = (a == 0) ? C[0] : (a == 1 ? V[0] : T[a - 1]);
-            blk_sync();
-            const double yy = T[0];
+                else v = (c == 0) ? C[a - 1] : V[a - 1];
+                G[ar_tri(a, c)] = v;
+            }
+            for (int a = b.tid; a < p1; a += b.nt) g[a] = (a == 0) ? C[0] : (a == 1 ? V[0] : Tc[a - 1]);
+            ar_sync(b);
+            const double yy = Tc[0];
             TSFA_TICK(tk, b, 123);
             {
                 double dmin1 = 0.0;
-                const bool okf = blk_chol_factor(b, G, p1, P, diag0, &dmin1);
+                const bool okf = blk_chol_factor(b, G, p1, diag0, &dmin1);
                 if (!okf) degenerate |= 2;
                 else {
                     const double mu = xcc.mean;
@@ -473,12 +511,12 @@
                 }
                 if (okf) {
                     for (int a = b.tid; a < p1; a += b.nt) tmp1[a] = g[a];
-                    blk_chol_forward(b, G, p1, P, tmp1);
+                    blk_chol_forward(b, G, p1, tmp1);
                     if (b.tid == 0) {
                         double acc = 0.0;
                         for (int i = 0; i < p1; ++i) { acc += tmp1[i] * tmp1[i]; tmp2[i] = acc; }
                     }
-                    blk_sync();
+                    ar_sync(b);
                     for (int i = b.tid; i < p1; i += b.nt) {
                         const int pcols = i + 1;
                         const double ssr = yy - tmp2[i];
@@ -488,7 +526,7 @@
                         if (adf_mode == TSFA_AUTOLAG_TSTAT) ic = fabs(wi / sqrt(ssr / (nobs - (double)pcols)));
                         tmp1[i] = ic;
                     }
-                    blk_sync();
+                    ar_sync(b);
                 }
                 if (b.tid == 0) {
                     int best = -1;
@@ -508,9 +546,9 @@
                     res[0] = (double)best;
                 }
             }
-            blk_sync();
+            ar_sync(b);
             const int bestcols = (int)res[0];
-            blk_sync();
+            ar_sync(b);
             TSFA_TICK(tk, b, 124);
             if (bestcols >= 2) {
                 const int usedlag = bestcols - 2;
@@ -518,6 +556,8 @@
                 const int u0 = usedlag;
                 const double nobs2 = (double)(t1 - u0);
                 auto reg2 = [=](int a, int t) { return a == 0 ? xcc[t] : (a == p2 - 1 ? 1.0 : dif(t - a)); };
+                ar_lag_products_into(b, dif, usedlag, t0, t1, Tc, G, 0);
+                ar_sync(b);
                 for (int e = b.tid; e < p2 * p2 + p2; e += b.nt) {
                     const bool is_rhs = e >= p2 * p2;
                     const int a = is_rhs ? e - p2 * p2 : e % p2;
@@ -527,7 +567,7 @@
                     auto lagidx = [=](int q) { return q == 0 ? -2 : (q == p2 - 1 ? -1 : q); };
                     const int A = lagidx(a), Cc = is_rhs ? 0 : lagidx(c);
                     if (is_rhs) {
-                        v = (A == -2) ? V[0] : (A == -1 ? C[0] : T[A]);
+                        v = (A == -2) ? V[0] : (A == -1 ? C[0] : Tc[A]);
                     } else {
                         const int hi = a, lo = c;
                         (void)hi; (void)lo;
@@ -538,16 +578,16 @@
                         else if (Cc == -1) v = C[A];
                         else if (A == -2) v = V[Cc];
                         else if (Cc == -2) v = V[A];
-                        else v = (A >= Cc) ? T[A + Cc * P] : T[Cc + A * P];
+                        else v = G[ar_tri(a, c)];
                     }
                     for (int t = u0; t < t0; ++t) v += reg2(a, t) * (is_rhs ? dif(t) : reg2(c, t));
-                    if (is_rhs) g[a] = v; else G[a + c * P] = v;
-                }
-                blk_sync();
-                const bool ok2 = blk_chol_factor(b, G, p2, P, diag0);
+                    if (is_rhs) g[a] = v; else G[ar_tri(a, c)] = v;
+                }
+                ar_sync(b);
+                const bool ok2 = blk_chol_factor(b, G, p2, diag0);
                 if (!ok2) degenerate |= 2;
-                if (ok2) blk_chol_solve(b, G, p2, P, g, beta);
-                blk_sync();
+                if (ok2) blk_chol_solve(b, G, p2, g, beta);
+                ar_sync(b);
                 if (ok2) {
                     auto resid2 = [=](int t) {
                         double r = dif(t);
@@ -571,13 +611,13 @@
                                 if (a0 + j < p2) tmp1[a0 + j] = s8[j];
                         }
                     }
-                    blk_sync();
-                    blk_chol_solve(b, G, p2, P, tmp1, tmp2);
-                    blk_sync();
+                    ar_sync(b);
+                    blk_chol_solve(b, G, p2, tmp1, tmp2);
+                    ar_sync(b);
                     if (ar_refinement_suspect(b, beta, tmp2, diag0, p2)) degenerate |= 2;
-                    blk_sync();
+                    ar_sync(b);
                     for (int a = b.tid; a < p2; a += b.nt) beta[a] += tmp2[a];
-                    blk_sync();
+                    ar_sync(b);
                     double ssr = 0.0;
                     for (int t = u0 + b.tid; t < t1; t += b.nt) {
                         double r = dif(t);
@@ -586,9 +626,9 @@
                     }
                     ssr = blk_sum(b, ssr);
                     for (int i = b.tid; i < p2; i += b.nt) tmp1[i] = (i == 0) ? 1.0 : 0.0;
-                    blk_sync();
-                    blk_chol_solve(b, G, p2, P, tmp1, tmp2);
-                    blk_sync();
+                    ar_sync(b);
+                    blk_chol_solve(b, G, p2, tmp1, tmp2);
+                    ar_sync(b);
                     if (b.tid == 0) {
                         const double sigma2 = ssr / (nobs2 - (double)p2);
                         const double tstat = beta[0] / sqrt(sigma2 * tmp2[0]);
@@ -596,12 +636,12 @@
                         res[3] = mackinnon_p_c1(tstat);
                         res[4] = (double)usedlag;
                     }
-                    blk_sync();
+                    ar_sync(b);
                     adf_stat = res[2];
                     adf_p = res[3];
                     adf_lag = res[4];
                     if (adf_stat != adf_stat) adf_p = TSFA_NAN;
-                    blk_sync();
+                    ar_sync(b);
                 }
             }
         }
@@ -707,19 +747,16 @@
                 double sy[2];
                 blk_tile_lagdots(b, n, k + 1,
                                  [=](int tb, double (&A)[8]) { blk.y8(tb, A); tile_mask_rows(A, tb, k, n); }, y_blocks,
-                                 [=](int j, double v) { T[j] = v; }, sy, G, P * P);
-                if (b.tid == 0) C[0] = sy[0];
-                blk_lag_products_rest(b, sx, k, k, n, T, P, C);
+                                 [=](int j, double v) { Tc[j] = v; }, sy, pt, ptn);
+                ar_sync(b);
+                ar_lag_products_into(b, sx, k, k, n, Tc, G, 0, C, sy[0]);
+                ar_sync(b);
                 const int p = k + 1;
-                for (int e = b.tid; e < p * p; e += b.nt) {
-                    const int a = e % p, c = e / p;
-                    if (c > a) continue;
-                    G[a + c * P] = (a == 0) ? (double)(n - k) : (c == 0 ? C[a] : T[a + c * P]);
-                }
-                for (int a = b.tid; a < p; a += b.nt) g[a] = (a == 0) ? C[0] : T[a];
-                blk_sync();
+                for (int a = b.tid; a < p; a += b.nt) G[ar_tri(a, 0)] = (a == 0) ? (double)(n - k) : C[a];
+                for (int a = b.tid; a < p; a += b.nt) g[a] = (a == 0) ? C[0] : Tc[a];
+                ar_sync(b);
                 double dmin_ar = 0.0;
-                ar_ok = blk_chol_factor(b, G, p, P, diag0, &dmin_ar);
+                ar_ok = blk_chol_factor(b, G, p, diag0, &dmin_ar);
                 if (!ar_ok) degenerate |= 1;
                 else {
                     const double mu = xcc.mean, rows = (double)(n - k);
@@ -731,24 +768,24 @@
                     double tr0 = 0.0, s0 = 0.0;
                     for (int a = 0; a < p; ++a) { tr0 += diag0[a]; s0 += 1.0 / diag0[a]; }
                     for (int a = b.tid; a < p; a += b.nt) tmp1[a] = 1.0 / sqrt(diag0[a] * s0);
-                    blk_sync();
+                    ar_sync(b);
                     double lmin = tr0;
                     for (int it = 0; it < 2; ++it) {
-                        blk_chol_solve(b, G, p, P, tmp1, tmp2);
-                        blk_sync();
+                        blk_chol_solve(b, G, p, tmp1, tmp2);
+                        ar_sync(b);
                         double nrm2 = 0.0;
                         for (int a = 0; a < p; ++a) nrm2 += tmp2[a] * tmp2[a];
                         const double nrm = sqrt(nrm2);
                         if (!(nrm > 0.0) || isinf(nrm) || nrm != nrm) { lmin = 0.0; break; }
                         lmin = 1.0 / nrm;
-                        blk_sync();
+                        ar_sync(b);
                         for (int a = b.tid; a < p; a += b.nt) tmp1[a] = tmp2[a] / nrm;
-                        blk_sync();
+                        ar_sync(b);
                     }
                     if (!(lmin >= 1e-12 * tr0)) degenerate |= 1;
                 }
-                if (ar_ok) blk_chol_solve(b, G, p, P, g, beta);
-                blk_sync();
+                if (ar_ok) blk_chol_solve(b, G, p, g, beta);
+                ar_sync(b);
                 if (ar_ok) {
                     double sr[2];
                     blk_tile_lagdots(b, n, k + 1,
@@ -772,13 +809,13 @@
                                          }
                                          tile_mask_rows(A, tb, k, n);
                                      },
-                                     y_blocks, [=](int a, double v) { if (a > 0) tmp1[a] = v; }, sr, T, P * P);
+                                     y_blocks, [=](int a, double v) { if (a > 0) tmp1[a] = v; }, sr, part, part_doubles);
                     if (b.tid == 0) tmp1[0] = sr[0];
-                    blk_sync();
-                    blk_chol_solve(b, G, p, P, tmp1, tmp2);
-                    blk_sync();
+                    ar_sync(b);
+                    blk_chol_solve(b, G, p, tmp1, tmp2);
+                    ar_sync(b);
                     if (ar_refinement_suspect(b, beta, tmp2, diag0, p)) degenerate |= 1;
-                    blk_sync();
+                    ar_sync(b);
                     if (b.tid == 0) {
                         double sphi = 0.0;
                         for (int a = 0; a < p; ++a) {
@@ -788,7 +825,7 @@
                         arres[0] = beta[0] + mean * (1.0 - sphi);
                         for (int a = 1; a < p; ++a) arres[a] = beta[a];
                     }
-                    blk_sync();
+                    ar_sync(b);
                 }
                 ar_cached_k = k;
             }
@@ -800,7 +837,7 @@
         TSFA_TICK(tk, b, sp.calc);
     }
     if (nloop < nspecs) {
-        blk_sync();
+        ar_sync(b);
         for (int s = nloop + b.tid; s < nspecs; s += b.nt) {
             const TsfaSpec sp = specs[s];
             double v = TSFA_NAN;
diff --git a/tsfresh_amd/csrc/tsfa_api.cpp b/tsfresh_amd/csrc/tsfa_api.cpp
--- a/tsfresh_amd/csrc/tsfa_api.cpp
+++ b/tsfresh_amd/csrc/tsfa_api.cpp
@@ -594,7 +594,7 @@
                 a.nt = (maxn > 4096) ? nt_8k[f] : nt_4k[f];
             }
             if (maxn <= 2048) {
-                static const int pref[TSFA_N_FAMILIES] = {64, 128, 128, 128, 256, 256, 128, 64};
+                static const int pref[TSFA_N_FAMILIES] = {64, 128, 128, 64, 256, 256, 128, 64};
                 const int cap = std::max(64, ((maxn / 4 + 63) / 64) * 64);
                 a.nt = std::min(pref[f], cap);
             }
diff --git a/tsfresh_amd/csrc/tsfa_kernels.hip b/tsfresh_amd/csrc/tsfa_kernels.hip
--- a/tsfresh_amd/csrc/tsfa_kernels.hip
+++ b/tsfresh_amd/csrc/tsfa_kernels.hip
@@ -294,13 +294,13 @@
     const int64_t off = starts[sidx];
     const int n = (int)(ends[sidx] - off);
     ArLds L;
-    L.carve(tsfa_base, maxn, P, (int)sizeof(T));
+    L.carve(tsfa_base, maxn, P, (int)sizeof(T), (int)blockDim.x);
     TSFA_TICKS_BEGIN();
     Blk b{(int)threadIdx.x, (int)blockDim.x, L.red, L.np};
     const T *g = values + off;
     const int flags = fam_ar_series<T>(b, [=](int i) { return (double)g[i]; }, n, specs, nspecs, out + sidx * ld,
                                        (void *)L.xc, L.aw, P, hint_acf, hint_pacf, hint_adf, n_loop,
-                                       stats_in ? stats_in + sidx * TSFA_STATS_N : nullptr);
+                                       stats_in ? stats_in + sidx * TSFA_STATS_N : nullptr, L.part, L.part_doubles);
     if (flags && threadIdx.x == 0) deg_list[atomicAdd(deg_count, 1)] = ((long long)sidx << 2) | flags;
     TSFA_TICKS_END();
     TSFA_SERIES_END
@@ -983,7 +983,7 @@
         }
     } else if (a.fam == TSFA_FAM_AR) {
         ArLds L;
-        const size_t lds = L.carve(nullptr, a.maxn, a.ar_P, (int)sizeof(T));
+        const size_t lds = L.carve(nullptr, a.maxn, a.ar_P, (int)sizeof(T), nt);
         TSFA_KLAUNCH(k_ar<T>, lds, values, a.starts, a.ends, a.n_series, a.sel, a.specs, a.nspecs, a.out, a.ld, a.maxn, a.ar_P,
                      a.hint_a, a.hint_b, a.hint_c, a.hint_d, a.deg_list, a.deg_count, a.stats_in);
     } else if (a.fam == TSFA_FAM_ENTROPY) {
@@ -1200,7 +1200,7 @@
     case TSFA_FAM_TREND: { BasicLds L; return L.carve(nullptr, maxn, nt, 8, 2, aux); }
     case TSFA_FAM_SORT: { SortLds L; return L.carve(nullptr, maxn, nt); }
     case TSFA_FAM_SPECTRAL: { SpectralLds L; return L.carve(nullptr, maxn, aux); }
-    case TSFA_FAM_AR: { ArLds L; return L.carve(nullptr, maxn, aux); }
+    case TSFA_FAM_AR: { ArLds L; return L.carve(nullptr, maxn, aux, 8, nt); }
     case TSFA_FAM_CWT: {
         CwtPeaksLayout L;
         const size_t lds16 = L.carve(nullptr, maxn, aux, 8, 2);
diff --git a/tsfresh_amd/csrc/tsfa_layout.h b/tsfresh_amd/csrc/tsfa_layout.h
--- a/tsfresh_amd/csrc/tsfa_layout.h
+++ b/tsfresh_amd/csrc/tsfa_layout.h
@@ -129,9 +129,9 @@
 };
 
 struct ArLds {
-    double *red; NpScratch *np; double *xc; double *aw;
-    TSFA_HD static int scratch_doubles(int P) { return 2 * P * P + 7 * P + 64 + 16 + 48 + 40 + 128; }
-    TSFA_HD size_t carve(unsigned char *base, int maxn, int P, int xs_bytes = 8) {
+    double *red; NpScratch *np; double *xc; double *aw; double *part; int part_doubles;
+    TSFA_HD static int scratch_doubles(int P) { return (P * (P - 1)) / 2 + 8 * P + 64 + 8 + 48 + 32; }
+    TSFA_HD size_t carve(unsigned char *base, int maxn, int P, int xs_bytes = 8, int nt = 64) {
         LdsCarve c{base, 0};
         red = c.take<double>(TSFA_RED_DOUBLES);
         xc = (double *)(void *)c.take<unsigned char>((size_t)(maxn + 64 + 16) * xs_bytes);
@@ -139,6 +139,8 @@
         unsigned char *u = c.take<unsigned char>(ab > sizeof(NpScratch) ? ab : sizeof(NpScratch));
         aw = (double *)u;
         np = (NpScratch *)u;
+        part_doubles = (nt > 64) ? 72 * ((nt + 63) / 64) : 0;
+        part = part_doubles ? c.take<double>((size_t)part_doubles) : nullptr;
         return c.off;
     }
 };
```
